# cherubrock-seb/PrMers

Measured on AMD Instinct MI355X. Metric: PRP squaring throughput at p~136M (Marin IBDWT, one exponent per GPU), higher is better.
Workload: dtype u64 (GF(2^64-2^32+1)); 1 GPU; square_mul x<-x^2 mod 2^p-1, p=136279841, n=8388608 words; plan=marin-hip:n=8388608:m1=1024:m2=4096:c=4, parallelism=replicas: one exponent per GPU, no data-path collective

## Files before the change

### prmers_amd/csrc/engine.hip

```cpp
#include "engine.hpp"

#include <algorithm>
#include <cstdlib>
#include <cstring>

#include "host_digits.hpp"

namespace mi355 {

#define HIPCHK(expr)                                                                              \
  do {                                                                                            \
    hipError_t e_ = (expr);                                                                       \
    if (e_ != hipSuccess)                                                                         \
      throw std::runtime_error(std::string("HIP error: ") + hipGetErrorString(e_) + " in " #expr); \
  } while (0)

static ColSweeps col_sweeps(ColKernels k) {
  switch (k) {
    case ColKernels::kRadix8R1: return v2_cols(1);
    case ColKernels::kRadix8R2: return v2_cols(2);
    case ColKernels::kRadix8R4: return v2_cols(4);
    case ColKernels::kRadix4Pairs: return v3_cols(false);
    case ColKernels::kRadix4Planes: return v3_cols(true);
    case ColKernels::kRadix5: return v5_cols(false);
    case ColKernels::kRadix5J1: return v5_cols(true);
    case ColKernels::kSplit: return ColSweeps{};
    default: return ColSweeps{launch_front, launch_back, launch_back_ext, nullptr};
  }
}
static RowsFn row_sweep(RowKernels k) {
  switch (k) {
    case RowKernels::kRadix4Pairs: return v3_rows1024_pairs;
    case RowKernels::kRadix4Planes: return v3_rows1024_planes;
    case RowKernels::kRadix8: return v2_rows4096;
    case RowKernels::kRadix8Wide: return v2_rows8192;
    case RowKernels::kRows2048One: return v2_rows2048_one;
    case RowKernels::kRows2048Two: return v2_rows2048_two;
    default: return launch_middle;
  }
}

template <class T>
static const T* upload(unsigned char*& cursor, unsigned char* base, const std::vector<T>& v, std::vector<unsigned char>& host) {
  const size_t off = size_t(cursor - base);
  std::memcpy(host.data() + off, v.data(), v.size() * sizeof(T));
  const T* p = reinterpret_cast<const T*>(cursor);
  cursor += (v.size() * sizeof(T) + 255) & ~size_t(255);
  return p;
}

Engine::Engine(uint32_t p, size_t reg_count, int device, bool verbose, const char* spec)
    : pl_(make_plan(p, spec, true)), device_(device), verbose_(verbose), nregs_(reg_count) {
  if (reg_count == 0) throw std::runtime_error("register_count must be > 0");
  int ndev = 0;
  hipError_t e = hipGetDeviceCount(&ndev);
  if (e != hipSuccess || ndev == 0)
    throw std::runtime_error("no HIP device available: the MI355X engine has no CPU fallback");
  if (device < 0 || device >= ndev) throw std::runtime_error("HIP device index out of range");
  HIPCHK(hipSetDevice(device));
  HIPCHK(hipStreamCreateWithFlags(&stream_, hipStreamNonBlocking));

  reg_bytes_ = pl_.n * 8;
  HIPCHK(hipMalloc(reinterpret_cast<void**>(&regs_), (nregs_ + 1) * reg_bytes_));
  HIPCHK(hipMemsetAsync(regs_, 0, (nregs_ + 1) * reg_bytes_, stream_));
  slot_.resize(nregs_ + 1);
  for (size_t r = 0; r <= nregs_; ++r) slot_[r] = regs_ + r * reg_bytes_;
  HIPCHK(hipMalloc(reinterpret_cast<void**>(&cbuf_), (nregs_ + 4) * pl_.runs() * 8));
  HIPCHK(hipMemsetAsync(cbuf_, 0, (nregs_ + 4) * pl_.runs() * 8, stream_));
  cb_.resize(nregs_);
  for (size_t r = 0; r < nregs_; ++r) cb_[r] = cbuf_ + r * pl_.runs();
  for (size_t r = nregs_; r < nregs_ + 4; ++r) cb_spare_.push_back(cbuf_ + r * pl_.runs());
  kind_.assign(nregs_, kDigits);
  pending_carry_.assign(nregs_, 0);

  auto padded = [](size_t bytes) { return (bytes + 255) & ~size_t(255); };
  std::vector<uint64_t> tah(pl_.TA.size()), tai2(pl_.TAi.size());
  for (size_t i = 0; i < tah.size(); ++i) { tah[i] = gf::half(pl_.TA[i]); tai2[i] = gf::dbl(pl_.TAi[i]); }
  const size_t total = padded(pl_.SA.size() * 4) + padded(pl_.SB.size() * 4) + padded(pl_.TA.size() * 8) * 4 +
                       padded(pl_.TB.size() * 8) * 2 + padded(pl_.TWlo.size() * 8) + padded(pl_.TWhi.size() * 8) +
                       padded(pl_.UT1.size() * 8) + padded(pl_.UT2.size() * 8) + padded(pl_.S2r.size() * 8) * 2 +
                       padded(pl_.S1r.size() * 8) * 2 + 1024;
  HIPCHK(hipMalloc(&tables_, total));
  std::vector<unsigned char> host(total, 0);
  unsigned char* base = static_cast<unsigned char*>(tables_);
  unsigned char* cur = base;
  dp_.SA = upload(cur, base, pl_.SA, host);
  dp_.SB = upload(cur, base, pl_.SB, host);
  dp_.TA = upload(cur, base, pl_.TA, host);
  dp_.TAi = upload(cur, base, pl_.TAi, host);
  dp_.TAh = upload(cur, base, tah, host);
  dp_.TAi2 = upload(cur, base, tai2, host);
  dp_.TB = upload(cur, base, pl_.TB, host);
  dp_.TBi = upload(cur, base, pl_.TBi, host);
  dp_.TWlo = upload(cur, base, pl_.TWlo, host);
  dp_.TWhi = upload(cur, base, pl_.TWhi, host);
  dp_.UT1 = upload(cur, base, pl_.UT1, host);
  dp_.UT2 = upload(cur, base, pl_.UT2, host);
  dp_.S2r = pl_.S2r.empty() ? nullptr : upload(cur, base, pl_.S2r, host);
  dp_.S2ri = pl_.S2ri.empty() ? nullptr : upload(cur, base, pl_.S2ri, host);
  dp_.S1r = pl_.S1r.empty() ? nullptr : upload(cur, base, pl_.S1r, host);
  dp_.S1ri = pl_.S1ri.empty() ? nullptr : upload(cur, base, pl_.S1ri, host);
  HIPCHK(hipMemcpy(tables_, host.data(), total, hipMemcpyHostToDevice));

  dp_.n = uint32_t(pl_.n); dp_.m = uint32_t(pl_.m);
  dp_.M1 = pl_.M1; dp_.M2 = pl_.M2; dp_.L1 = pl_.L1; dp_.logL1 = pl_.logL1; dp_.logM2 = pl_.logM2;
  dp_.r5 = pl_.r5; dp_.C = pl_.C; dp_.logC = 0; while ((1u << dp_.logC) < pl_.C) ++dp_.logC; dp_.q = pl_.q; dp_.t = pl_.t; dp_.twh = pl_.twh;
  dp_.I4 = pl_.I4; dp_.I4inv = pl_.I4inv;
  dp_.DI = nullptr;
  dp_.F0f = dp_.F0i = dp_.FBf = dp_.FBi = nullptr;
  if (!pl_.DI.empty()) {
    HIPCHK(hipMalloc(reinterpret_cast<void**>(&di_), pl_.DI.size() * 4));
    HIPCHK(hipMemcpy(di_, pl_.DI.data(), pl_.DI.size() * 4, hipMemcpyHostToDevice));
    dp_.DI = di_;
  }
  for (int i = 0; i < 4; ++i) dp_.W5c[i] = pl_.W5c[i];
  { const char* tn = std::getenv("MI355_TUNE"); dp_.tune = tn ? uint32_t(std::atoi(tn)) : 0u; }
  {
    hipDeviceProp_t prop;
    HIPCHK(hipGetDeviceProperties(&prop, device_));
    const uint32_t slots = 2u * uint32_t(prop.multiProcessorCount);
    auto from = [&](size_t grid) { return grid > slots ? uint32_t(grid - size_t(slots) * 50 / 100) : ~0u; };
    dp_.boost_rows = from(pl_.M2 == 2048 ? pl_.M1 / 2 : pl_.M1);
    dp_.boost_tiles = from(pl_.tiles());
  }
  HIPCHK(configure_kernels(pl_.lds_front, pl_.lds_mid));
  if (pl_.split5) {
    HIPCHK(configure_split(dp_));
    HIPCHK(hipMalloc(reinterpret_cast<void**>(&split_), reg_bytes_));
  }
  kc_ = choose_kernels(pl_, std::getenv("MI355_KERNELS"));
  cols_ = col_sweeps(kc_.cols);
  rows_ = row_sweep(kc_.rows);
  dp_.lab_u = 1; dp_.lab_v = pl_.r5; dp_.lab_red = 0;
  if (kc_.cols == ColKernels::kRadix5 || kc_.cols == ColKernels::kRadix5J1) {
    v5_pfa(kc_.cols == ColKernels::kRadix5J1, &dp_.lab_u, &dp_.lab_v);
  } else if (kc_.cols == ColKernels::kGeneric && pl_.r5 == 5 && pl_.L1 > 1) {
    uint32_t u = 1; while ((pl_.L1 * u) % 5 != 1) ++u;
    dp_.lab_u = pl_.L1 * u;
    dp_.lab_red = pl_.M1;
  }
  {
    const uint64_t max_label = dp_.lab_red ? uint64_t(pl_.M1) - 1 : uint64_t(dp_.lab_u) * (pl_.r5 - 1) + uint64_t(dp_.lab_v) * (pl_.L1 - 1);
    if (max_label + uint64_t(pl_.M1) * (pl_.M2 - 1) >= (uint64_t(pl_.TWhi.size()) << pl_.twh))
      throw std::runtime_error("internal: column frequency labels beyond the root table");
  }
  if (kc_.resident_cols() || kc_.rows != RowKernels::kGeneric) HIPCHK(v2_configure());
  if (kc_.resident_cols()) {
    const size_t nt = pl_.tiles() * threads_per_tile(kc_.cols);
    HIPCHK(hipMalloc(reinterpret_cast<void**>(&f0_), (2 * nt + 2 * size_t(pl_.M2)) * 8));
    HIPCHK(cols_.build_fourstep(dp_, f0_, f0_ + nt, f0_ + 2 * nt, f0_ + 2 * nt + pl_.M2, stream_));
    HIPCHK(hipStreamSynchronize(stream_));
    dp_.F0f = f0_; dp_.F0i = f0_ + nt; dp_.FBf = f0_ + 2 * nt; dp_.FBi = f0_ + 2 * nt + pl_.M2;
  }

  width_ = host_digits::digit_widths(p, pl_.n);
  cg_ = CanonGeom::tile_major(dp_, p);
  { const char* hc = std::getenv("MI355_HOST_CARRY"); host_carry_ = hc && hc[0] == '1'; }
  HIPCHK(hipStreamSynchronize(stream_));
  if (verbose_) std::fprintf(stderr, "[mi355] p=%u %s regs=%zu device=%d\n", p, pl_.describe().c_str(), nregs_, device_);
}

Engine::~Engine() {
  (void)hipSetDevice(device_);
  if (stream_) (void)hipStreamSynchronize(stream_);
  if (regs_) (void)hipFree(regs_);
  if (cbuf_) (void)hipFree(cbuf_);
  if (tables_) (void)hipFree(tables_);
  if (di_) (void)hipFree(di_);
  if (f0_) (void)hipFree(f0_);
  if (split_) (void)hipFree(split_);
  if (canon_) (void)hipFree(canon_);
  if (stream_) (void)hipStreamDestroy(stream_);
}

void Engine::sync() {
  HIPCHK(hipSetDevice(device_));
  HIPCHK(hipStreamSynchronize(stream_));
}

void Engine::normalize(size_t r) {
  if (kind_[r] != kDigits) return;
  if (pending_carry_[r]) {
    HIPCHK(launch_carry_fix(dp_, digits(r), cbuf(r), stream_));
    pending_carry_[r] = 0;
  }
}

void Engine::carry_fix_now(size_t r, int excess) {
  HIPCHK(launch_carry_fix(dp_, digits(r), cbuf(r), stream_));
  pending_carry_[r] = 0;
  if (pl_.C >= 2) return;
  if (excess < 0) excess = ilog2(pl_.n) + 1 + 4 - 2;
  const int w = int(pl_.q);
  while (excess > w - 2) {
    HIPCHK(canon_relax(dp_, pl_.p, digits(r), reinterpret_cast<uint32_t*>(work()), stream_));
    swap_with_work(r);
    excess -= w;
  }
}

void Engine::run_front(size_t r) {
  if (kc_.cols == ColKernels::kSplit) HIPCHK(launch_front_split(dp_, digits(r), split_, work(), stream_));
  else HIPCHK(cols_.front(dp_, digits(r), pending_carry_[r] ? cbuf(r) : nullptr, work(), stream_));
}

void Engine::run_middle(const uint64_t* in, const uint64_t* y, uint64_t* out, int mode, const uint64_t* y2, uint64_t* img) {
  HIPCHK(rows_(dp_, in, y, y2, img, out, mode, stream_));
}

void Engine::run_back(size_t r, uint32_t a, hipEvent_t* ev) {
  if (kc_.cols == ColKernels::kSplit) HIPCHK(launch_back_split(dp_, work(), split_, digits(r), cbuf(r), a, stream_));
  else HIPCHK(cols_.back(dp_, work(), digits(r), cbuf(r), a, stream_));
  if (ev) HIPCHK(hipEventRecord(ev[0], stream_));
  if (pl_.C >= 2) pending_carry_[r] = 1;
  else carry_fix_now(r);
  if (ev) HIPCHK(hipEventRecord(ev[1], stream_));
}


void Engine::write_values(size_t dst, const std::vector<uint32_t>& natural) {
  HIPCHK(hipSetDevice(device_));
  HIPCHK(hipStreamSynchronize(stream_));
  uint32_t* nat = reinterpret_cast<uint32_t*>(work());
  HIPCHK(hipMemcpy(nat, natural.data(), pl_.n * 4, hipMemcpyHostToDevice));
  HIPCHK(canon_scatter(dp_, pl_.p, nat, digits(dst), stream_));
  HIPCHK(hipStreamSynchronize(stream_));
  kind_[dst] = kDigits;
  pending_carry_[dst] = 0;
}

uint32_t* Engine::canon_digits(size_t r, int slot) {
  need_residue(r, "get");
  HIPCHK(hipSetDevice(device_));
  const size_t sw = canon_scratch_bytes<uint32_t>(cg_) / 4;
  if (!canon_) {
    HIPCHK(hipMalloc(reinterpret_cast<void**>(&canon_), (sw + 2 * pl_.n) * 4));
    HIPCHK(hipMemsetAsync(canon_flags<uint32_t>(cg_, canon_), 0, 16 * 4, stream_));
  }
  normalize(r);
  uint32_t* out = canon_ + sw + size_t(slot) * pl_.n;
  HIPCHK(canon_launch(cg_, digits(r), out, canon_, stream_));
  return out;
}

bool Engine::canon_flags_ok(uint32_t (&flags)[4]) {
  uint32_t* df = canon_flags<uint32_t>(cg_, canon_);
  HIPCHK(hipMemcpyAsync(flags, df, 16, hipMemcpyDeviceToHost, stream_));
  HIPCHK(hipMemsetAsync(df, 0, 16 * 4, stream_));
  HIPCHK(hipStreamSynchronize(stream_));
  return flags[1] == 0;
}

void Engine::read_values(size_t src, std::vector<uint64_t>& v) {
  if (host_carry_) { read_values_host(src, v); return; }
  uint32_t* d = canon_digits(src, 0);
  uint32_t flags[4];
  stage_.resize(pl_.n);
  HIPCHK(hipMemcpyAsync(stage_.data(), d, pl_.n * 4, hipMemcpyDeviceToHost, stream_));
  if (!canon_flags_ok(flags)) { read_values_host(src, v); return; }
  v.resize(pl_.n);
  if (flags[0]) {
    for (size_t k = 0; k < pl_.n; ++k) v[k] = host_digits::ones(width_[k]);
  } else {
    for (size_t k = 0; k < pl_.n; ++k) v[k] = stage_[k];
  }
}

void Engine::read_values_host(size_t src, std::vector<uint64_t>& v) {
  need_residue(src, "get");
  stage_.resize(pl_.n);
  HIPCHK(hipSetDevice(device_));
  normalize(src);
  HIPCHK(hipStreamSynchronize(stream_));
  HIPCHK(hipMemcpy(stage_.data(), digits(src), pl_.n * 4, hipMemcpyDeviceToHost));
  v.resize(pl_.n);
  const size_t M2 = pl_.M2, C = pl_.C, M1 = pl_.M1;
  for (size_t i = 0; i < pl_.m; ++i) {
    const size_t i1 = i / M2, i2 = i % M2, T = i2 / C, c = i2 % C;
    const size_t s = ((T * M1 + i1) * C + c) * 2;
    v[2 * i] = stage_[s];
    v[2 * i + 1] = stage_[s + 1];
  }
  host_digits::strong_carry(v.data(), width_);
}

void Engine::set_u32(size_t dst, uint32_t value) {
  need_register(dst, "set");
  HIPCHK(hipSetDevice(device_));
  HIPCHK(hipMemsetAsync(digits(dst), 0, pl_.n * 4, stream_));
  if (value) HIPCHK(canon_set_small(dp_, pl_.p, digits(dst), value, stream_));
  kind_[dst] = kDigits;
  pending_carry_[dst] = 0;
}

void Engine::set_digits(size_t dst, const uint64_t* d, size_t count) {
  need_register(dst, "set_digits");
  if (count != pl_.n) throw std::runtime_error("set_digits: count must equal the transform size");
  std::vector<uint32_t> nat(pl_.n);
  for (size_t k = 0; k < pl_.n; ++k) nat[k] = uint32_t(d[k]);
  write_values(dst, nat);
}

void Engine::get_digits(size_t src, uint64_t* d, size_t count) {
  if (count != pl_.n) throw std::runtime_error("get_digits: count must equal the transform size");
  std::vector<uint64_t> v;
  read_values(src, v);
  for (size_t k = 0; k < pl_.n; ++k) d[k] = uint32_t(v[k]) | (uint64_t(width_[k]) << 32);
}

uint64_t Engine::res64(size_t src) {
  std::vector<uint64_t> v;
  size_t have = pl_.n;
  if (host_carry_) {
    read_values_host(src, v);
  } else {
    uint32_t* d = canon_digits(src, 0);
    have = std::min<size_t>(pl_.n, 16);
    uint32_t head[16], flags[4];
    HIPCHK(hipMemcpyAsync(head, d, have * 4, hipMemcpyDeviceToHost, stream_));
    if (!canon_flags_ok(flags)) { read_values_host(src, v); have = pl_.n; }
    else { v.resize(have); for (size_t k = 0; k < have; ++k) v[k] = flags[0] ? host_digits::ones(width_[k]) : head[k]; }
  }
  return host_digits::res64_of_head(v.data(), width_, have);
}

void Engine::get_words(size_t src, uint32_t* w, size_t count) {
  if (count != word_count()) throw std::runtime_error("get_words: count must equal word_count()");
  if (!host_carry_) {
    uint32_t* d = canon_digits(src, 0);
    uint32_t* dw = canon_;
    HIPCHK(canon_pack_words(cg_, d, dw, stream_));
    HIPCHK(hipMemcpyAsync(w, dw, count * 4, hipMemcpyDeviceToHost, stream_));
    uint32_t flags[4];
    if (canon_flags_ok(flags)) return;
  }
  std::vector<uint64_t> v;
  read_values_host(src, v);
  host_digits::pack_words(v.data(), width_, w, count);
}

void Engine::set_words(size_t dst, const uint32_t* w, size_t count) {
  need_register(dst, "set_words");
  if (count != word_count()) throw std::runtime_error("set_words: count must equal word_count()");
  std::vector<uint32_t> src;
  if (host_carry_ || ((pl_.p % 32) && (w[count - 1] >> (pl_.p % 32)))) {
    src.assign(w, w + count);
    host_digits::fold_words_mod_mp(src.data(), count, pl_.p);
    w = src.data();
  }
  if (!host_carry_) {
    HIPCHK(hipSetDevice(device_));
    uint32_t* dw = reinterpret_cast<uint32_t*>(work());
    HIPCHK(hipMemcpyAsync(dw, w, count * 4, hipMemcpyHostToDevice, stream_));
    HIPCHK(canon_unpack_words(cg_, dw, digits(dst), stream_));
    HIPCHK(hipStreamSynchronize(stream_));
    kind_[dst] = kDigits;
    pending_carry_[dst] = 0;
    return;
  }
  std::vector<uint64_t> v(pl_.n);
  host_digits::unpack_words(w, count, width_, v.data());
  write_values(dst, std::vector<uint32_t>(v.begin(), v.end()));
}

bool Engine::equal(size_t lhs, size_t rhs) {
  if (!host_carry_) {
    uint32_t* a = canon_digits(lhs, 0);
    uint32_t* b = canon_digits(rhs, 1);
    HIPCHK(canon_compare(a, b, uint32_t(pl_.n), canon_flags<uint32_t>(cg_, canon_) + 2, stream_));
    uint32_t flags[4];
    if (canon_flags_ok(flags)) return flags[2] == 0;
  }
  return equal_words(lhs, rhs);
}


void Engine::copy(size_t dst, size_t src) {
  need_register(dst, "copy"); need_register(src, "copy");
  if (dst == src) return;
  HIPCHK(hipSetDevice(device_));
  const size_t bytes = (kind_[src] == kDigits) ? pl_.n * 4 : reg_bytes_;
  HIPCHK(hipMemcpyAsync(slot_[dst], slot_[src], bytes, hipMemcpyDeviceToDevice, stream_));
  if (kind_[src] == kDigits && pending_carry_[src])
    HIPCHK(hipMemcpyAsync(cbuf(dst), cbuf(src), pl_.runs() * 8, hipMemcpyDeviceToDevice, stream_));
  pending_carry_[dst] = (kind_[src] == kDigits) ? pending_carry_[src] : 0;
  kind_[dst] = kind_[src];
}

void Engine::square_chain(size_t r, uint32_t a, hipEvent_t* ev) {
  if (a > pl_.a_fast) { square_chain(r, 1, ev); scale(r, a); return; }
  if (ev) HIPCHK(hipEventRecord(ev[0], stream_));
  run_front(r);
  if (ev) HIPCHK(hipEventRecord(ev[1], stream_));
  run_middle(work(), nullptr, work(), 0);
  if (ev) HIPCHK(hipEventRecord(ev[2], stream_));
  run_back(r, a, ev ? ev + 3 : nullptr);
}

void Engine::square_mul(size_t r, uint32_t a) {
  need_residue(r, "square_mul"); need_factor(a, "square_mul");
  HIPCHK(hipSetDevice(device_));
  square_chain(r, a, nullptr);
}

void Engine::square_mul_n(size_t r, uint32_t a, size_t count, uint32_t sub) {
  need_residue(r, "square_mul_n"); need_factor(a, "square_mul_n");
  if (count == 0) return;
  HIPCHK(hipSetDevice(device_));
  for (size_t i = 0; i < count; ++i) { square_chain(r, a, nullptr); if (sub) sub_u32(r, sub); }
}

void Engine::set_multiplicand(size_t dst, size_t src) {
  need_residue(src, "set_multiplicand"); need_register(dst, "set_multiplicand");
  HIPCHK(hipSetDevice(device_));
  run_front(src);
  run_middle(work(), nullptr, image(dst), 2);
  kind_[dst] = kImage;
  pending_carry_[dst] = 0;
}

void Engine::mul(size_t dst, size_t src, uint32_t a) {
  need_residue(dst, "mul"); need_image(src, "mul"); need_factor(a, "mul");
  HIPCHK(hipSetDevice(device_));
  run_front(dst);
  run_middle(work(), image(src), work(), 1);
  run_back(dst, a > pl_.a_fast ? 1u : a);
  if (a > pl_.a_fast) scale(dst, a);
}

void Engine::scale(size_t r, uint32_t a) {
  need_residue(r, "scale");
  uint64_t* fresh = take_spare_cbuf();
  HIPCHK(launch_scale(dp_, digits(r), pending_carry_[r] ? cbuf(r) : nullptr, digits(r), fresh, a, stream_));
  adopt_cbuf(r, fresh);
  pending_carry_[r] = 1;
  if (pl_.C < 2) carry_fix_now(r, 34 - int(pl_.q));
}

uint64_t* Engine::take_spare_cbuf() {
  if (cb_spare_.empty()) throw std::runtime_error("internal: no spare carry buffer");
  uint64_t* b = cb_spare_.back();
  cb_spare_.pop_back();
  return b;
}
void Engine::adopt_cbuf(size_t r, uint64_t* fresh) {
  cb_spare_.push_back(cb_[r]);
  cb_[r] = fresh;
}

void Engine::addsub(long s1, long s2, long d1, long d2, size_t a, size_t b) {
  HIPCHK(hipSetDevice(device_));
  need_residue(a, "addsub"); need_residue(b, "addsub");
  const long outs[4] = {s1, s2, d1, d2};
  for (int i = 0; i < 4; ++i)
    if (outs[i] >= 0) { need_register(size_t(outs[i]), "addsub"); for (int j = 0; j < i; ++j) if (outs[j] == outs[i]) throw std::runtime_error("addsub: output registers must differ"); }
  LinArgs la;
  la.a = digits(a); la.ca = pending_carry_[a] ? cbuf(a) : nullptr;
  la.b = digits(b); la.cb = pending_carry_[b] ? cbuf(b) : nullptr;
  uint64_t* fresh[4] = {nullptr, nullptr, nullptr, nullptr};
  for (int i = 0; i < 4; ++i) if (outs[i] >= 0) fresh[i] = take_spare_cbuf();
  if (s1 >= 0) { la.s1 = digits(size_t(s1)); la.cs1 = fresh[0]; }
  if (s2 >= 0) { la.s2 = digits(size_t(s2)); la.cs2 = fresh[1]; }
  if (d1 >= 0) { la.d1 = digits(size_t(d1)); la.cd1 = fresh[2]; }
  if (d2 >= 0) { la.d2 = digits(size_t(d2)); la.cd2 = fresh[3]; }
  if ((s2 >= 0 && s1 < 0) || (d2 >= 0 && d1 < 0)) throw std::runtime_error("internal: copy output without a primary output");
  HIPCHK(launch_linear(dp_, la, stream_));
  for (int i = 0; i < 4; ++i)
    if (outs[i] >= 0) {
      const size_t r = size_t(outs[i]);
      adopt_cbuf(r, fresh[i]);
      kind_[r] = kDigits; pending_carry_[r] = 1;
      if (pl_.C < 2) carry_fix_now(r);
    }
}

void Engine::add(size_t dst, size_t src) { addsub(long(dst), -1, -1, -1, dst, src); }
void Engine::sub_reg(size_t dst, size_t src) { addsub(-1, -1, long(dst), -1, dst, src); }

void Engine::back_ext(size_t dst, uint32_t a, long copy_to, long add_src) {
  BackExt x;
  if (copy_to >= 0 && size_t(copy_to) != dst) { x.digits2 = digits(size_t(copy_to)); x.cbuf2 = cbuf(size_t(copy_to)); }
  if (add_src >= 0) { x.add_digits = digits(size_t(add_src)); x.add_cbuf = pending_carry_[size_t(add_src)] ? cbuf(size_t(add_src)) : nullptr; }
  uint64_t* fresh = take_spare_cbuf();
  HIPCHK(cols_.back_ext(dp_, work(), digits(dst), fresh, a, x, stream_));
  adopt_cbuf(dst, fresh);
  const size_t outs[2] = {dst, x.digits2 ? size_t(copy_to) : dst};
  for (int i = 0; i < (x.digits2 ? 2 : 1); ++i) {
    const size_t r = outs[i];
    kind_[r] = kDigits; pending_carry_[r] = 1;
    if (pl_.C < 2) carry_fix_now(r);
  }
}

void Engine::square_mul_copy(size_t src, size_t dst_copy, uint32_t a) {
  need_residue(src, "square_mul_copy"); need_register(dst_copy, "square_mul_copy"); need_factor(a, "square_mul_copy");
  HIPCHK(hipSetDevice(device_));
  if (dst_copy == src || !kc_.fused_back() || a > pl_.a_fast) { RegisterMachine::square_mul_copy(src, dst_copy, a); return; }
  run_front(src);
  run_middle(work(), nullptr, work(), 0);
  back_ext(src, a, long(dst_copy), -1);
}

void Engine::mul_copy(size_t dst, size_t src, size_t dst_copy, uint32_t a) {
  need_residue(dst, "mul_copy"); need_image(src, "mul_copy"); need_register(dst_copy, "mul_copy"); need_factor(a, "mul_copy");
  if (dst_copy == src) throw std::runtime_error("mul_copy: the multiplicand must differ from the outputs");
  HIPCHK(hipSetDevice(device_));
  if (dst_copy == dst || !kc_.fused_back() || a > pl_.a_fast) { RegisterMachine::mul_copy(dst, src, dst_copy, a); return; }
  run_front(dst);
  run_middle(work(), image(src), work(), 1);
  back_ext(dst, a, long(dst_copy), -1);
}

void Engine::mul_add(size_t dst, size_t mul_src, size_t add_src, uint32_t a) {
  need_residue(dst, "mul_add"); need_image(mul_src, "mul_add"); need_residue(add_src, "mul_add"); need_factor(a, "mul_add");
  HIPCHK(hipSetDevice(device_));
  if (!kc_.fused_back() || a > pl_.a_fast) {
    if (add_src == dst)
      throw std::runtime_error(!kc_.fused_back() ? "mul_add: add_src == dst needs the fused sweep, which this transform size does not have"
                                          : "mul_add: add_src == dst needs the fused sweep, which takes factors up to the plan's fused bound only (mi355_engine.h)");
    RegisterMachine::mul_add(dst, mul_src, add_src, a); return;
  }
  run_front(dst);
  run_middle(work(), image(mul_src), work(), 1);
  back_ext(dst, a, -1, long(add_src));
}

void Engine::mul_sum(size_t dst, size_t src_a, size_t src_b, size_t tmp) {
  if (!pl_.sum_fast) { RegisterMachine::mul_sum(dst, src_a, src_b, tmp); return; }
  check_mul_sum(dst, src_a, src_b, tmp);
  HIPCHK(hipSetDevice(device_));
  run_front(dst);
  run_middle(work(), image(src_a), work(), 3, image(src_b));
  run_back(dst, 1);
}

void Engine::square_mul_prepare(size_t src, size_t img_out, uint32_t a) {
  check_square_mul_prepare(src, img_out, a);
  HIPCHK(hipSetDevice(device_));
  run_front(src);
  run_middle(work(), nullptr, work(), 4, nullptr, image(img_out));
  kind_[img_out] = kImage;
  pending_carry_[img_out] = 0;
  run_back(src, a > pl_.a_fast ? 1u : a);
  if (a > pl_.a_fast) scale(src, a);
}

void Engine::square_mul_bits(size_t r, uint32_t factor, const uint8_t* bits, size_t nbits) {
  if (!check_square_mul_bits(r, factor, bits, nbits)) return;
  HIPCHK(hipSetDevice(device_));
  for (size_t i = 0; i < nbits; ++i) square_chain(r, bit_of(bits, i) ? factor : 1u, nullptr);
}

void Engine::sub_u32(size_t r, uint32_t v) {
  need_residue(r, "sub");
  if (v == 0) return;
  HIPCHK(hipSetDevice(device_));
  HIPCHK(launch_sub_small(dp_, digits(r), v, stream_));
}


void Engine::get_data(size_t src, void* data, size_t size) {
  need_register(src, "get_data");
  if (size != register_data_size()) throw std::runtime_error("get_data: size mismatch");
  HIPCHK(hipSetDevice(device_));
  normalize(src);
  HIPCHK(hipStreamSynchronize(stream_));
  HIPCHK(hipMemcpy(data, slot_[src], reg_bytes_, hipMemcpyDeviceToHost));
  const uint64_t tag = kind_[src];
  std::memcpy(static_cast<unsigned char*>(data) + reg_bytes_, &tag, 8);
}

void Engine::set_data(size_t dst, const void* data, size_t size) {
  need_register(dst, "set_data");
  if (size != register_data_size()) throw std::runtime_error("set_data: size mismatch");
  uint64_t tag = 0;
  std::memcpy(&tag, static_cast<const unsigned char*>(data) + reg_bytes_, 8);
  if (tag > 1) throw std::runtime_error("set_data: not an image written by this engine");
  HIPCHK(hipSetDevice(device_));
  HIPCHK(hipStreamSynchronize(stream_));
  HIPCHK(hipMemcpy(slot_[dst], data, reg_bytes_, hipMemcpyHostToDevice));
  kind_[dst] = uint8_t(tag);
  pending_carry_[dst] = 0;
}


namespace {
struct EventPool {
  std::vector<hipEvent_t> evs;
  hipEvent_t make() {
    hipEvent_t e = nullptr;
    HIPCHK(hipEventCreate(&e));
    evs.push_back(e);
    return e;
  }
  ~EventPool() { for (hipEvent_t e : evs) (void)hipEventDestroy(e); }
};
}

const char* Engine::stage_name(size_t k) {
  static const char* names[kKernels] = {"k_front", "k_middle", "k_back", "k_carry_fix", "k_sub_small", "event_overhead"};
  return k < kKernels ? names[k] : "";
}

void Engine::time_square_mul(size_t r, uint32_t a, uint32_t sub, size_t iters, double* total_ms, double* kernel_ms, size_t kcount) {
  need_residue(r, "time_square_mul");
  if (a == 0 || iters == 0) throw std::runtime_error("time_square_mul: factor and iters must be >= 1");
  HIPCHK(hipSetDevice(device_));
  EventPool pool;
  const hipEvent_t e0 = pool.make(), e1 = pool.make();
  HIPCHK(hipStreamSynchronize(stream_));
  HIPCHK(hipEventRecord(e0, stream_));
  square_mul_n(r, a, iters, sub);
  HIPCHK(hipEventRecord(e1, stream_));
  HIPCHK(hipEventSynchronize(e1));
  float ms = 0;
  HIPCHK(hipEventElapsedTime(&ms, e0, e1));
  if (total_ms) *total_ms = ms;

  if (kernel_ms && kcount) {
    for (size_t k = 0; k < kcount; ++k) kernel_ms[k] = 0;
    const size_t reps = std::min<size_t>(iters, 64);
    const size_t per = 6;
    std::vector<hipEvent_t> ev(reps * per);
    for (auto& x : ev) x = pool.make();
    double overhead = 0;
    {
      constexpr size_t kBatch = 64, kSkip = 8;
      std::vector<hipEvent_t> oe(kBatch);
      for (auto& x : oe) x = pool.make();
      for (size_t i = 0; i < kBatch; ++i) HIPCHK(hipEventRecord(oe[i], stream_));
      HIPCHK(hipStreamSynchronize(stream_));
      float t = 0;
      HIPCHK(hipEventElapsedTime(&t, oe[kSkip], oe[kBatch - 1]));
      overhead = double(t) / double(kBatch - 1 - kSkip);
    }
    for (size_t i = 0; i < reps; ++i) {
      square_chain(r, a, &ev[i * per]);
// ... 71 lines not shown
```

### prmers_amd/csrc/engine.hpp

```cpp
#pragma once
#include <hip/hip_runtime.h>

#include <algorithm>
#include <cstdint>
#include <stdexcept>
#include <string>
#include <vector>

#include "canon.hpp"
#include "kernels.hpp"
#include "plan.hpp"
#include "register_machine.hpp"

namespace mi355 {

class Engine final : public RegisterMachine {
 public:
  Engine(uint32_t p, size_t reg_count, int device, bool verbose, const char* spec);
  ~Engine() override;
  Engine(const Engine&) = delete;
  Engine& operator=(const Engine&) = delete;

  uint32_t exponent() const override { return pl_.p; }
  std::string describe() const override { return pl_.describe(); }
  size_t size() const override { return pl_.n; }
  size_t reg_count() const override { return nregs_; }

  void sync() override;
  void set_u32(size_t dst, uint32_t v) override;
  void set_digits(size_t dst, const uint64_t* d, size_t count) override;
  void get_digits(size_t src, uint64_t* d, size_t count) override;
  void set_words(size_t dst, const uint32_t* w, size_t count) override;
  void get_words(size_t src, uint32_t* w, size_t count) override;
  uint64_t res64(size_t src) override;
  void copy(size_t dst, size_t src) override;
  void set_multiplicand(size_t dst, size_t src) override;
  void square_mul(size_t r, uint32_t a) override;
  void mul(size_t dst, size_t src, uint32_t a) override;
  void add(size_t dst, size_t src) override;
  void sub_reg(size_t dst, size_t src) override;
  void sub_u32(size_t r, uint32_t v) override;
  bool equal(size_t lhs, size_t rhs) override;
  void addsub(long sum, long sum_copy, long diff, long diff_copy, size_t a, size_t b) override;
  void mul_add(size_t dst, size_t mul_src, size_t add_src, uint32_t a) override;
  void square_mul_copy(size_t src, size_t dst_copy, uint32_t a) override;
  void mul_copy(size_t dst, size_t src, size_t dst_copy, uint32_t a) override;
  void square_mul_n(size_t r, uint32_t a, size_t count, uint32_t sub) override;
  void square_mul_bits(size_t r, uint32_t factor, const uint8_t* bits, size_t nbits) override;
  void mul_sum(size_t dst, size_t src_a, size_t src_b, size_t tmp) override;
  bool mul_sum_is_fused() const override { return pl_.sum_fast; }
  void square_mul_prepare(size_t src, size_t img_out, uint32_t a) override;
  bool square_mul_prepare_is_fused() const override { return true; }

  size_t register_data_size() const override { return reg_bytes_ + 8; }
  void get_data(size_t src, void* data, size_t size) override;
  void set_data(size_t dst, const void* data, size_t size) override;

  static constexpr size_t kKernels = 6;
  static const char* stage_name(size_t k);
  size_t kernel_count() const override { return kKernels; }
  const char* kernel_name(size_t k) const override { return stage_name(k); }
  void time_square_mul(size_t r, uint32_t a, uint32_t sub, size_t iters, double* total_ms, double* kernel_ms, size_t kcount) override;
  size_t algorithmic_bytes() const override { return 48 * pl_.n; }
#if defined(MI355_PROBE)
  void probe(int kind, int grid_mult, int extra_lds, int boost_pct, size_t iters, double* avg_ms, uint64_t* tl, size_t tl_words);
#endif

 private:
  enum Kind : uint8_t { kDigits = 0, kImage = 1 };
  bool holds_image(size_t r) const override { return kind_[r] == kImage; }
  uint32_t* digits(size_t r) { return reinterpret_cast<uint32_t*>(slot_[r]); }
  uint64_t* image(size_t r) { return reinterpret_cast<uint64_t*>(slot_[r]); }
  uint64_t* work() { return reinterpret_cast<uint64_t*>(slot_[nregs_]); }
  void swap_with_work(size_t r) { std::swap(slot_[r], slot_[nregs_]); }
  void read_values(size_t src, std::vector<uint64_t>& v);
  void read_values_host(size_t src, std::vector<uint64_t>& v);
  uint32_t* canon_digits(size_t r, int slot);
  bool canon_flags_ok(uint32_t (&flags)[4]);
  void write_values(size_t dst, const std::vector<uint32_t>& natural);
  void square_chain(size_t r, uint32_t a, hipEvent_t* ev);
  uint64_t* cbuf(size_t r) { return cb_[r]; }
  uint64_t* take_spare_cbuf();
  void adopt_cbuf(size_t r, uint64_t* fresh);
  void back_ext(size_t dst, uint32_t a, long copy_to, long add_src);
  void normalize(size_t r);
  void carry_fix_now(size_t r, int excess = -1);
  void scale(size_t r, uint32_t a);
  void run_front(size_t r);
  void run_middle(const uint64_t* in, const uint64_t* y, uint64_t* out, int mode, const uint64_t* y2 = nullptr, uint64_t* img = nullptr);
  void run_back(size_t r, uint32_t a, hipEvent_t* ev = nullptr);

  Plan pl_;
  DevPlan dp_{};
  CanonGeom cg_{};
  int device_ = 0;
  bool verbose_ = false;
  hipStream_t stream_ = nullptr;
  size_t nregs_ = 0, reg_bytes_ = 0;
  unsigned char* regs_ = nullptr;
  std::vector<unsigned char*> slot_;
  uint64_t* cbuf_ = nullptr;
  std::vector<uint64_t*> cb_, cb_spare_;
  void* tables_ = nullptr;
  uint64_t* split_ = nullptr;
  uint64_t* f0_ = nullptr;
  uint32_t* di_ = nullptr;
  std::vector<uint8_t> kind_;
  std::vector<uint8_t> pending_carry_;
  KernelChoice kc_;
  ColSweeps cols_{};
  RowsFn rows_ = nullptr;
  std::vector<uint8_t> width_;
  std::vector<uint32_t> stage_;
  uint32_t* canon_ = nullptr;
  bool host_carry_ = false;
};

}
```

### prmers_amd/csrc/gfdft.hpp

```cpp
#pragma once
#include "gf.hpp"

namespace gf {

constexpr unsigned LOG2_W64 = 39;
constexpr unsigned shift64(unsigned e) { return (LOG2_W64 * e) % 192; }

template <bool INV, int LAZY = 0>
GF_HD void dft8(uint64_t (&x)[8]) {
  constexpr bool LZ_A0 = (LAZY >= 2), LZ_E0 = (LAZY >= 1);
  const uint64_t a0 = LZ_A0 ? add_lazy(x[0], x[4]) : add(x[0], x[4]);
  const uint64_t a1 = add(x[1], x[5]), a2 = add(x[2], x[6]), a3 = add(x[3], x[7]);
  uint64_t b0 = sub(x[0], x[4]), b1, b2, b3;
  if (!INV) {
    b1 = mul_pow2(sub(x[5], x[1]), 24);
    b2 = mul_pow2(sub(x[2], x[6]), 48);
    b3 = mul_pow2(sub(x[7], x[3]), 72);
  } else {
    b1 = mul_pow2(sub(x[1], x[5]), 72);
    b2 = mul_pow2(sub(x[6], x[2]), 48);
    b3 = mul_pow2(sub(x[3], x[7]), 24);
  }
  const uint64_t c0 = LZ_A0 ? add_lazy(a0, a2) : add(a0, a2);
  const uint64_t c1 = add(a1, a3), d0 = sub(a0, a2);
  const uint64_t d1 = mul_pow2(INV ? sub(a3, a1) : sub(a1, a3), 48);
  const uint64_t e0 = LZ_E0 ? add_lazy(b0, b2) : add(b0, b2);
  const uint64_t e1 = add(b1, b3), f0 = sub(b0, b2);
  const uint64_t f1 = mul_pow2(INV ? sub(b3, b1) : sub(b1, b3), 48);
  x[0] = (LAZY >= 2) ? add_lazy(c0, c1) : add(c0, c1); x[4] = sub(c0, c1);
  x[2] = (LAZY >= 1) ? add_lazy(d0, d1) : add(d0, d1); x[6] = sub(d0, d1);
  x[1] = (LAZY >= 1) ? add_lazy(e0, e1) : add(e0, e1); x[5] = sub(e0, e1);
  x[3] = (LAZY >= 1) ? add_lazy(f0, f1) : add(f0, f1); x[7] = sub(f0, f1);
}

}
```

### prmers_amd/csrc/kernels.hip

```cpp
#include <hip/hip_runtime.h>
#include <stdint.h>
#include <stdlib.h>

#include "gf.hpp"
#include "kernels.hpp"

namespace mi355 {

struct alignas(16) P2 { uint64_t a, b; };

__device__ __forceinline__ P2 p2_add(P2 x, P2 y) { return {gf::add(x.a, y.a), gf::add(x.b, y.b)}; }
__device__ __forceinline__ P2 p2_sub(P2 x, P2 y) { return {gf::sub(x.a, y.a), gf::sub(x.b, y.b)}; }
__device__ __forceinline__ P2 p2_mul(P2 x, uint64_t w) { return {gf::mul(x.a, w), gf::mul(x.b, w)}; }
__device__ __forceinline__ P2 p2_shift48(P2 x) { return {gf::mul_pow2(x.a, 48), gf::mul_pow2(x.b, 48)}; }

__device__ __forceinline__ uint64_t tw_lookup(const DevPlan& pl, uint64_t e) {
  const uint64_t lo = pl.TWlo[e & ((1u << pl.twh) - 1)], hi = pl.TWhi[e >> pl.twh];
  return gf::mul(lo, hi);
}

__device__ __forceinline__ uint32_t freq1(const DevPlan& pl, uint32_t pos) {
  const uint32_t blk = pos >> pl.logL1, q = pos & (pl.L1 - 1);
  const uint32_t rq = pl.logL1 ? (__brev(q) >> (32 - pl.logL1)) : 0u;
  return col_label(pl, blk, rq);
}

__device__ __forceinline__ void digit_info(const DevPlan& pl, uint32_t sa, uint32_t sb, uint32_t& width, bool& wrap) {
  uint64_t s = uint64_t(sa) + sb;
  wrap = (sa > 0) && (sb > 0) && (s <= pl.n);
  if (s >= pl.n) s -= pl.n;
  width = pl.q + ((s + pl.t > 0) ? 1u : 0u) + ((s + pl.t > pl.n) ? 1u : 0u) - ((s > 0) ? 1u : 0u);
}

template <bool INVERSE>
__device__ __forceinline__ void lds_pow2_dft_planes(P2* X, uint32_t L, uint32_t logL, uint32_t nblocks, uint32_t ncols, uint32_t logcols,
                                                    const uint64_t* __restrict__ root, uint32_t rootN, uint32_t rstep, uint32_t tid, uint32_t nthr) {
  uint64_t* Xw = reinterpret_cast<uint64_t*>(X);
  const uint32_t n4 = logL / 2, has2 = logL & 1;
  const uint32_t npass = n4 + has2;
  for (uint32_t ps = 0; ps < npass; ++ps) {
    const uint32_t pf = INVERSE ? (npass - 1 - ps) : ps;
    if (pf < n4) {
      const uint32_t loglen = logL - 2 * pf, len = 1u << loglen, q = len >> 2;
      const uint32_t per = L >> 2;
      const uint32_t total = per * nblocks * ncols * 2;
      const uint32_t tstep = (L >> loglen) * rstep;
      for (uint32_t idx2 = tid; idx2 < total; idx2 += nthr) {
        const uint32_t plane = idx2 & 1, idx = idx2 >> 1;
        const uint32_t col = idx & (ncols - 1), bi = idx >> logcols;
        const uint32_t blk = bi >> (logL - 2), bj = bi & (per - 1);
        const uint32_t sub = bj >> (loglen - 2), t = bj & (q - 1);
        const uint32_t e0 = 2 * ((blk * L + sub * len + t) * ncols + col) + plane, es = 2 * q * ncols;
        const uint32_t r1 = t * tstep;
        const uint64_t x0 = Xw[e0], x1 = Xw[e0 + es], x2 = Xw[e0 + 2 * es], x3 = Xw[e0 + 3 * es];
        if (!INVERSE) {
          const uint64_t w1 = root[r1], w2 = root[2 * r1], w3 = root[3 * r1];
          const uint64_t a = gf::add(x0, x2), b = gf::add(x1, x3), c = gf::sub(x0, x2), d = gf::mul_pow2(gf::sub(x1, x3), 48);
          Xw[e0] = gf::add(a, b);
          Xw[e0 + es] = gf::mul(gf::sub(a, b), w2);
          Xw[e0 + 2 * es] = gf::mul(gf::add(c, d), w1);
          Xw[e0 + 3 * es] = gf::mul(gf::sub(c, d), w3);
        } else {
          const uint64_t w1 = root[r1 ? rootN - r1 : 0], w2 = root[r1 ? rootN - 2 * r1 : 0], w3 = root[r1 ? rootN - 3 * r1 : 0];
          const uint64_t y1 = gf::mul(x1, w2);
          const uint64_t A = gf::add(x0, y1), B = gf::sub(x0, y1);
          const uint64_t y2 = gf::mul(x2, w1), y3 = gf::mul(x3, w3);
          const uint64_t Cc = gf::add(y2, y3), D = gf::mul_pow2(gf::sub(y3, y2), 48);
          Xw[e0] = gf::add(A, Cc);
          Xw[e0 + 2 * es] = gf::sub(A, Cc);
          Xw[e0 + es] = gf::add(B, D);
          Xw[e0 + 3 * es] = gf::sub(B, D);
        }
      }
    } else {
      const uint32_t per = L >> 1, total = per * nblocks * ncols * 2;
      for (uint32_t idx2 = tid; idx2 < total; idx2 += nthr) {
        const uint32_t plane = idx2 & 1, idx = idx2 >> 1;
        const uint32_t col = idx & (ncols - 1), bi = idx >> logcols;
        const uint32_t blk = bi >> (logL - 1), bj = bi & (per - 1);
        const uint32_t e0 = 2 * ((blk * L + 2 * bj) * ncols + col) + plane;
        const uint64_t u = Xw[e0], v = Xw[e0 + 2 * ncols];
        Xw[e0] = gf::add(u, v);
        Xw[e0 + 2 * ncols] = gf::sub(u, v);
      }
    }
    __syncthreads();
  }
}

template <bool INVERSE>
__device__ __forceinline__ void lds_pow2_dft(P2* X, uint32_t L, uint32_t logL, uint32_t nblocks, uint32_t ncols, uint32_t logcols,
                                             const uint64_t* __restrict__ root, uint32_t rootN, uint32_t rstep,
                                             uint64_t I4, uint32_t tid, uint32_t nthr) {
  if (nthr * 2 >= (L >> 2) * nblocks * ncols * 2 && nthr > (L >> 2) * nblocks * ncols) {
    lds_pow2_dft_planes<INVERSE>(X, L, logL, nblocks, ncols, logcols, root, rootN, rstep, tid, nthr);
    return;
  }
  const uint32_t n4 = logL / 2, has2 = logL & 1;
  const uint32_t npass = n4 + has2;
  for (uint32_t ps = 0; ps < npass; ++ps) {
    const uint32_t pf = INVERSE ? (npass - 1 - ps) : ps;
    if (pf < n4) {
      const uint32_t loglen = logL - 2 * pf, len = 1u << loglen, q = len >> 2;
      const uint32_t per = L >> 2;
      const uint32_t total = per * nblocks * ncols;
      const uint32_t tstep = (L >> loglen) * rstep;
      for (uint32_t idx = tid; idx < total; idx += nthr) {
        const uint32_t col = idx & (ncols - 1), bi = idx >> logcols;
        const uint32_t blk = bi >> (logL - 2), bj = bi & (per - 1);
        const uint32_t sub = bj >> (loglen - 2), t = bj & (q - 1);
        const uint32_t e0 = (blk * L + sub * len + t) * ncols + col, es = q * ncols;
        const uint32_t r1 = t * tstep;
        P2 x0 = X[e0], x1 = X[e0 + es], x2 = X[e0 + 2 * es], x3 = X[e0 + 3 * es];
        if (!INVERSE) {
          const uint64_t w1 = root[r1], w2 = root[2 * r1], w3 = root[3 * r1];
          const P2 a = p2_add(x0, x2), b = p2_add(x1, x3), c = p2_sub(x0, x2), d = p2_shift48(p2_sub(x1, x3));
          X[e0] = p2_add(a, b);
          X[e0 + es] = p2_mul(p2_sub(a, b), w2);
          X[e0 + 2 * es] = p2_mul(p2_add(c, d), w1);
          X[e0 + 3 * es] = p2_mul(p2_sub(c, d), w3);
        } else {
          const uint64_t w1 = root[r1 ? rootN - r1 : 0], w2 = root[r1 ? rootN - 2 * r1 : 0], w3 = root[r1 ? rootN - 3 * r1 : 0];
          const P2 y1 = p2_mul(x1, w2);
          const P2 A = p2_add(x0, y1), B = p2_sub(x0, y1);
          const P2 y2 = p2_mul(x2, w1), y3 = p2_mul(x3, w3);
          const P2 Cc = p2_add(y2, y3), D = p2_shift48(p2_sub(y3, y2));
          X[e0] = p2_add(A, Cc);
          X[e0 + 2 * es] = p2_sub(A, Cc);
          X[e0 + es] = p2_add(B, D);
          X[e0 + 3 * es] = p2_sub(B, D);
        }
      }
    } else {
      const uint32_t per = L >> 1, total = per * nblocks * ncols;
      for (uint32_t idx = tid; idx < total; idx += nthr) {
        const uint32_t col = idx & (ncols - 1), bi = idx >> logcols;
        const uint32_t blk = bi >> (logL - 1), bj = bi & (per - 1);
        const uint32_t e0 = (blk * L + 2 * bj) * ncols + col;
        const P2 u = X[e0], v = X[e0 + ncols];
        X[e0] = p2_add(u, v);
        X[e0 + ncols] = p2_sub(u, v);
      }
    }
    __syncthreads();
  }
}

template <bool INVERSE>
__device__ __forceinline__ void dft5(P2 (&x)[5], const uint64_t (&c5)[4]) {
  const P2 t1 = p2_add(x[1], x[4]), t2 = p2_add(x[2], x[3]), t3 = p2_sub(x[1], x[4]), t4 = p2_sub(x[2], x[3]);
  const P2 t5 = p2_add(t1, t2);
  const P2 A = p2_add(x[0], P2{gf::mul_pow2(t5.a, 94), gf::mul_pow2(t5.b, 94)});
  const P2 m2 = p2_mul(p2_sub(t1, t2), c5[0]);
  const P2 B1 = p2_add(A, m2), B2 = p2_sub(A, m2);
  const P2 m3 = p2_mul(p2_add(t3, t4), c5[1]), m4 = p2_mul(t4, c5[2]), m5 = p2_mul(t3, c5[3]);
  const P2 Pp = p2_add(m3, m4), Q = p2_sub(m5, m3);
  x[0] = p2_add(x[0], t5);
  if (!INVERSE) { x[1] = p2_add(B1, Pp); x[4] = p2_sub(B1, Pp); x[2] = p2_add(B2, Q); x[3] = p2_sub(B2, Q); }
  else          { x[1] = p2_sub(B1, Pp); x[4] = p2_add(B1, Pp); x[2] = p2_sub(B2, Q); x[3] = p2_add(B2, Q); }
}

template <bool INVERSE>
__device__ __forceinline__ void lds_radix5(const DevPlan& pl, P2* X, uint32_t ncols, uint32_t tid, uint32_t nthr) {
  const uint32_t L1 = pl.L1, total = L1 * ncols;
  const bool pfa = pl.lab_u != 1;
  for (uint32_t idx = tid; idx < total; idx += nthr) {
    const uint32_t col = idx & (ncols - 1), t = idx >> pl.logC;
    const uint32_t t5 = 5 * t, rho = pfa ? (t5 & (L1 - 1)) : t, w0 = pfa ? (t5 >> pl.logL1) : 0u;
    P2 x[5];
    if (!INVERSE) {
#pragma unroll
      for (uint32_t r = 0; r < 5; ++r) { const uint32_t b = r + w0; x[r] = X[(L1 * (b >= 5 ? b - 5 : b) + rho) * ncols + col]; }
      dft5<false>(x, pl.W5c);
      if (!pfa) {
#pragma unroll
        for (int k = 1; k < 5; ++k) x[k] = p2_mul(x[k], pl.UT1[t * k]);
      }
#pragma unroll
      for (int r = 0; r < 5; ++r) X[(L1 * r + rho) * ncols + col] = x[r];
    } else {
#pragma unroll
      for (int r = 0; r < 5; ++r) x[r] = X[(L1 * r + rho) * ncols + col];
      if (!pfa) {
#pragma unroll
        for (int k = 1; k < 5; ++k) x[k] = p2_mul(x[k], pl.UT1[(t * k) ? pl.M1 - t * k : 0]);
      }
      dft5<true>(x, pl.W5c);
#pragma unroll
      for (uint32_t r = 0; r < 5; ++r) { const uint32_t b = r + w0; X[(L1 * (b >= 5 ? b - 5 : b) + rho) * ncols + col] = x[r]; }
    }
  }
  __syncthreads();
}

extern __shared__ __attribute__((aligned(16))) unsigned char smem_raw[];

__device__ __forceinline__ uint64_t carry_in_of(const DevPlan& pl, const uint64_t* cbuf, uint32_t T, uint32_t i1) {
  const uint32_t NT = pl.M2 / pl.C;
  if (T > 0) return *(cbuf + size_t(T - 1) * pl.M1 + i1);
  return *(cbuf + size_t(NT - 1) * pl.M1 + (i1 ? i1 - 1 : pl.M1 - 1));
}

__device__ __forceinline__ void front_body(const DevPlan& pl, const uint32_t* digits, const uint64_t* cbuf_in, uint64_t* Wout, uint32_t T,
                                           P2* X, uint32_t tid, uint32_t nthr) {
  const uint32_t C = pl.C, M1 = pl.M1, tile = M1 * C;
  const uint2* dg = reinterpret_cast<const uint2*>(digits) + size_t(T) * tile;

  for (uint32_t e = tid; e < tile; e += nthr) {
    const uint32_t i1 = e >> pl.logC, c = e & (C - 1), i2 = T * C + c;
    uint2 d = dg[e];
    const uint32_t sa = pl.SA[i1];
    if (cbuf_in && c < 2) {
      uint64_t cin = carry_in_of(pl, cbuf_in, T, i1);
      if (cin) {
        const uint2* run = dg + i1 * C;
        const uint2 p0 = run[0], p1 = run[1];
        uint32_t dd[4] = {p0.x, p0.y, p1.x, p1.y};
#pragma unroll
        for (int k = 0; k < 3; ++k) {
          uint32_t width; bool wr;
          digit_info(pl, sa, pl.SB[2 * (T * C) + k], width, wr);
          const uint64_t v = uint64_t(dd[k]) + cin;
          dd[k] = uint32_t(v & ((uint64_t(1) << width) - 1));
          cin = v >> width;
        }
        dd[3] += uint32_t(cin);
        d = c ? make_uint2(dd[2], dd[3]) : make_uint2(dd[0], dd[1]);
      }
    }
    uint32_t w0, w1; bool wr0, wr1;
    const uint32_t sb = pl.SB[2 * i2];
    digit_info(pl, sa, sb, w0, wr0);
    digit_info(pl, pl.SA[M1 + i1], sb, w1, wr1);
    const uint64_t a0 = gf::mul_u32(pl.TAh[i1], d.x << (wr0 ? 0 : 1));
    const uint64_t a1 = gf::mul_u32(pl.TAh[M1 + i1], d.y << (wr1 ? 0 : 1));
    X[e] = {a0, a1};
  }
  __syncthreads();

  const bool one = tile <= nthr;
  uint64_t pre_lo = 0, pre_hi = 0, pre_tb = 0;
  if (one && tid < tile) {
    const uint32_t pos = tid >> pl.logC, i2 = T * C + (tid & (C - 1));
    const uint64_t ex = uint64_t(i2) * freq1(pl, pos);
    pre_lo = pl.TWlo[ex & ((1u << pl.twh) - 1)]; pre_hi = pl.TWhi[ex >> pl.twh]; pre_tb = pl.TB[2 * i2];
  }
  if (pl.r5 == 5) lds_radix5<false>(pl, X, C, tid, nthr);
  if (pl.logL1) lds_pow2_dft<false>(X, pl.L1, pl.logL1, pl.r5, C, pl.logC, pl.UT1, M1, pl.r5, pl.I4, tid, nthr);

  P2* W = reinterpret_cast<P2*>(Wout);
  for (uint32_t e = tid; e < tile; e += nthr) {
    const uint32_t pos = e >> pl.logC, c = e & (C - 1), i2 = T * C + c;
    const uint32_t k1 = freq1(pl, pos);
    const uint32_t ex = i2 * k1;
    const uint64_t tw = one ? gf::mul(pre_lo, pre_hi) : tw_lookup(pl, ex);
    const P2 x = X[e];
    const uint64_t twb = gf::mul(tw, one ? pre_tb : pl.TB[2 * i2]);
    P2* out = W + size_t(pos) * pl.M2 + i2;
    *out = {gf::mul(x.a, twb), gf::mul(x.b, twb)};
  }
}
__global__ void __launch_bounds__(1024) k_front(DevPlan pl, const uint32_t* __restrict__ digits, const uint64_t* __restrict__ cbuf_in,
                                                uint64_t* __restrict__ Wout) {
  if (blockIdx.x >= pl.boost_tiles) __builtin_amdgcn_s_setprio(3);
  front_body(pl, digits, cbuf_in, Wout, blockIdx.x, reinterpret_cast<P2*>(smem_raw), threadIdx.x, blockDim.x);
}

template <bool KEEP = false>
__device__ __forceinline__ void middle_body(const DevPlan& pl, const uint64_t* Win, const uint64_t* Yimg, const uint64_t* Yimg2, uint64_t* Wout, int mode, uint32_t sub, uint32_t row,
                                            P2* X, uint32_t tid, uint32_t nthr, uint64_t* Wimg = nullptr) {
  const uint32_t M2 = pl.M2;
  const P2* in = reinterpret_cast<const P2*>(Win) + size_t(row) * M2;
  P2* out = reinterpret_cast<P2*>(Wout) + size_t(row) * M2;

  for (uint32_t e = tid; e < M2; e += nthr) X[e] = in[e];
  __syncthreads();
  if (sub != 0 && tid == 0) X[0].a = gf::sub(X[0].a, uint64_t(sub));
  __syncthreads();
  const uint32_t k1 = freq1(pl, row);
  const bool one = M2 <= nthr;
  uint64_t pre_lo = 0, pre_hi = 0;
  if (one && tid < M2 && mode != 2) {
    const uint64_t ex = rho_exponent(pl, k1, __brev(tid) >> (32 - pl.logM2));
    pre_lo = pl.TWlo[ex & ((1u << pl.twh) - 1)]; pre_hi = pl.TWhi[ex >> pl.twh];
  }
  lds_pow2_dft<false>(X, M2, pl.logM2, 1, 1, 0, pl.UT2, M2, 1, pl.I4, tid, nthr);
  if (mode == 2) {
    for (uint32_t e = tid; e < M2; e += nthr) out[e] = X[e];
    return;
  }
  if constexpr (KEEP) {
    P2* img = reinterpret_cast<P2*>(Wimg) + size_t(row) * M2;
    for (uint32_t e = tid; e < M2; e += nthr) img[e] = X[e];
  }
  const P2* Y = reinterpret_cast<const P2*>(Yimg) + size_t(row) * M2;
  for (uint32_t e = tid; e < M2; e += nthr) {
    const uint32_t k2 = __brev(e) >> (32 - pl.logM2);
    const uint64_t rho = one ? gf::mul(pre_lo, pre_hi) : tw_lookup(pl, rho_exponent(pl, k1, k2));
    const P2 u = X[e];
    P2 r;
    if (mode == 0) {
      r.a = gf::add(gf::sqr(u.a), gf::mul(gf::sqr(u.b), rho));
      r.b = gf::mul(u.b, gf::dbl(u.a));
    } else {
      P2 y = Y[e];
      if (mode == 3) {
        const P2 z = reinterpret_cast<const P2*>(Yimg2)[size_t(row) * M2 + e];
        y = {gf::add_lazy_any(y.a, z.a), gf::add_lazy_any(y.b, z.b)};
      }
      r.a = gf::add(gf::mul(u.a, y.a), gf::mul(gf::mul(u.b, y.b), rho));
      r.b = gf::add(gf::mul(u.a, y.b), gf::mul(u.b, y.a));
    }
    X[e] = r;
  }
  __syncthreads();
  lds_pow2_dft<true>(X, M2, pl.logM2, 1, 1, 0, pl.UT2, M2, 1, pl.I4inv, tid, nthr);
  for (uint32_t e = tid; e < M2; e += nthr) out[e] = X[e];
}
__global__ void __launch_bounds__(1024) k_middle(DevPlan pl, const uint64_t* __restrict__ Win, const uint64_t* __restrict__ Yimg,
                                                const uint64_t* __restrict__ Yimg2, uint64_t* __restrict__ Wout, int mode, uint32_t sub) {
  middle_body(pl, Win, Yimg, Yimg2, Wout, mode, sub, blockIdx.x, reinterpret_cast<P2*>(smem_raw), threadIdx.x, blockDim.x);
}
__global__ void __launch_bounds__(1024) k_middle_keep(DevPlan pl, const uint64_t* __restrict__ Win, uint64_t* __restrict__ Wimg, uint64_t* __restrict__ Wout, uint32_t sub) {
  middle_body<true>(pl, Win, nullptr, nullptr, Wout, 0, sub, blockIdx.x, reinterpret_cast<P2*>(smem_raw), threadIdx.x, blockDim.x, Wimg);
}

__device__ __forceinline__ void run_carry_in(const DevPlan& pl, uint32_t sa, uint32_t T, uint64_t cin, uint32_t (&dd)[4]) {
#pragma unroll
  for (int k = 0; k < 3; ++k) {
    uint32_t width; bool wr;
    digit_info(pl, sa, pl.SB[2 * (T * pl.C) + k], width, wr);
    const uint64_t v = uint64_t(dd[k]) + cin;
    dd[k] = uint32_t(v & ((uint64_t(1) << width) - 1));
    cin = v >> width;
  }
  dd[3] += uint32_t(cin);
}

__device__ __forceinline__ uint32_t xcd_tile(const DevPlan& pl, uint32_t b, uint32_t groups) {
  return (!(pl.tune & 1) && groups % 8 == 0) ? (b & 7) * (groups >> 3) + (b >> 3) : b;
}
template <bool EXT>
__device__ __forceinline__ void back_body(const DevPlan& pl, const uint64_t* Win, uint32_t* digits, uint64_t* cbuf, uint32_t a, const BackExt& ext, uint32_t T,
                                          P2* X, uint32_t tid, uint32_t nthr) {
  const uint32_t C = pl.C, M1 = pl.M1, tile = M1 * C;
  const P2* W = reinterpret_cast<const P2*>(Win);

  for (uint32_t e = tid; e < tile; e += nthr) {
    const uint32_t pos = e >> pl.logC, c = e & (C - 1), i2 = T * C + c;
    const uint32_t k1 = freq1(pl, pos);
    const uint32_t ex = i2 * k1;
    const uint64_t tw = tw_lookup(pl, ex ? pl.m - ex : 0);
    const P2 x = *(W + size_t(pos) * pl.M2 + i2);
    const uint64_t twb = gf::mul(tw, pl.TBi[2 * i2]);
    X[e] = {gf::mul(x.a, twb), gf::mul(x.b, twb)};
  }
  __syncthreads();

  if (pl.logL1) lds_pow2_dft<true>(X, pl.L1, pl.logL1, pl.r5, C, pl.logC, pl.UT1, M1, pl.r5, pl.I4inv, tid, nthr);
  if (pl.r5 == 5) lds_radix5<true>(pl, X, C, tid, nthr);

  uint2* dg = reinterpret_cast<uint2*>(digits) + size_t(T) * tile;
  for (uint32_t i1 = tid; i1 < M1; i1 += nthr) {
    const uint32_t sa[2] = {pl.SA[i1], pl.SA[M1 + i1]};
    const uint64_t tai[2] = {pl.TAi[i1], pl.TAi[M1 + i1]};
    const uint64_t tai2[2] = {pl.TAi2[i1], pl.TAi2[M1 + i1]};
    uint64_t carry = 0;
    uint32_t addh[4] = {0, 0, 0, 0};
    const uint2* ad = nullptr;
    if (EXT && ext.add_digits) {
      ad = reinterpret_cast<const uint2*>(ext.add_digits) + size_t(T) * tile + size_t(i1) * C;
      if (ext.add_cbuf) {
        const uint2 p0 = ad[0], p1 = ad[1];
        addh[0] = p0.x; addh[1] = p0.y; addh[2] = p1.x; addh[3] = p1.y;
        run_carry_in(pl, pl.SA[i1], T, carry_in_of(pl, ext.add_cbuf, T, i1), addh);
      }
    }
    for (uint32_t c = 0; c < C; ++c) {
      const uint32_t i2 = T * C + c;
      const P2 x = X[i1 * C + c];
      const uint32_t sb = pl.SB[2 * i2];
      uint32_t out[2];
      uint32_t av[2] = {0, 0};
      if (EXT && ad) {
        if (ext.add_cbuf && c < 2) { av[0] = addh[2 * c]; av[1] = addh[2 * c + 1]; }
        else { const uint2 q = ad[c]; av[0] = q.x; av[1] = q.y; }
      }
#pragma unroll
      for (int b = 0; b < 2; ++b) {
        uint32_t width; bool wrap;
        digit_info(pl, sa[b], sb, width, wrap);
        const uint64_t u = gf::mul(b ? x.b : x.a, wrap ? tai2[b] : tai[b]);
        const uint64_t mask = (uint64_t(1) << width) - 1;
        if (a == 1) {
          const uint64_t r = u + carry + (EXT ? av[b] : 0u);
          out[b] = uint32_t(r & mask);
          carry = r >> width;
        } else {
          const uint64_t dlo = u & mask, chi = u >> width;
          const uint64_t r = dlo * a + carry + (EXT ? av[b] : 0u);
          out[b] = uint32_t(r & mask);
          carry = (r >> width) + chi * a;
        }
      }
      *(dg + i1 * C + c) = make_uint2(out[0], out[1]);
      if (EXT && ext.digits2) reinterpret_cast<uint2*>(ext.digits2)[size_t(T) * tile + size_t(i1) * C + c] = make_uint2(out[0], out[1]);
    }
    *(cbuf + size_t(T) * M1 + i1) = carry;
    if (EXT && ext.digits2) ext.cbuf2[size_t(T) * M1 + i1] = carry;
  }
}
template <bool EXT>
__global__ void __launch_bounds__(1024) k_back(DevPlan pl, const uint64_t* __restrict__ Win, uint32_t* __restrict__ digits,
                                              uint64_t* __restrict__ cbuf, uint32_t a, BackExt ext) {
  if (blockIdx.x >= pl.boost_tiles) __builtin_amdgcn_s_setprio(3);
  back_body<EXT>(pl, Win, digits, cbuf, a, ext, xcd_tile(pl, blockIdx.x, gridDim.x), reinterpret_cast<P2*>(smem_raw), threadIdx.x, blockDim.x);
}

__global__ void __launch_bounds__(256) k_front_split_a(DevPlan pl, const uint32_t* __restrict__ digits, uint64_t* __restrict__ Uout) {
  const size_t e = size_t(blockIdx.x) * 256 + threadIdx.x;
  const uint32_t t = uint32_t(e & (pl.L1 - 1)), i2 = uint32_t(e >> pl.logL1), M1 = pl.M1;
  if (i2 >= pl.M2) return;
  const uint2* dg = reinterpret_cast<const uint2*>(digits) + size_t(i2) * M1;
  const uint32_t sb = pl.SB[2 * i2];
  P2 x[5];
#pragma unroll
  for (int r = 0; r < 5; ++r) {
    const uint32_t i1 = pl.L1 * r + t;
    const uint2 d = dg[i1];
    uint32_t w0, w1; bool wr0, wr1;
    digit_info(pl, pl.SA[i1], sb, w0, wr0);
    digit_info(pl, pl.SA[M1 + i1], sb, w1, wr1);
    x[r] = {gf::mul_u32(pl.TAh[i1], d.x << (wr0 ? 0 : 1)), gf::mul_u32(pl.TAh[M1 + i1], d.y << (wr1 ? 0 : 1))};
  }
  dft5<false>(x, pl.W5c);
#pragma unroll
  for (int k = 1; k < 5; ++k) x[k] = p2_mul(x[k], pl.UT1[t * k]);
  P2* U = reinterpret_cast<P2*>(Uout);
#pragma unroll
  for (int k0 = 0; k0 < 5; ++k0) U[(size_t(k0) * pl.M2 + i2) * pl.L1 + t] = x[k0];
}
__global__ void __launch_bounds__(1024) k_front_split_b(DevPlan pl, const uint64_t* __restrict__ Uin, uint64_t* __restrict__ Wout, uint32_t logCb) {
  P2* X = reinterpret_cast<P2*>(smem_raw);
  const uint32_t tid = threadIdx.x, nthr = blockDim.x, Cb = 1u << logCb, per = pl.M2 >> logCb;
  const uint32_t k0 = blockIdx.x / per, T = blockIdx.x - k0 * per, tile = pl.L1 << logCb;
  const P2* U = reinterpret_cast<const P2*>(Uin);
  for (uint32_t e = tid; e < tile; e += nthr) {
    const uint32_t c = e >> pl.logL1, pp = e & (pl.L1 - 1);
    X[(pp << logCb) + c] = U[(size_t(k0) * pl.M2 + (T << logCb) + c) * pl.L1 + pp];
  }
  __syncthreads();
  if (pl.logL1) lds_pow2_dft<false>(X, pl.L1, pl.logL1, 1, Cb, logCb, pl.UT1, pl.M1, pl.r5, pl.I4, tid, nthr);
  P2* W = reinterpret_cast<P2*>(Wout);
  for (uint32_t e = tid; e < tile; e += nthr) {
    const uint32_t pp = e >> logCb, c = e & (Cb - 1), i2 = (T << logCb) + c, pos = k0 * pl.L1 + pp;
    const uint64_t ex = uint64_t(i2) * freq1(pl, pos);
// ... 271 lines not shown
```

### prmers_amd/csrc/kernels.hpp

```cpp
#pragma once
#include <hip/hip_runtime.h>
#include <stdint.h>

namespace mi355 {

struct DevPlan {
  uint32_t n, m, M1, M2, L1, logL1, logM2, r5, C, logC, q, t, twh;
  const uint32_t *SA, *SB;
  const uint64_t *TA, *TAi, *TB, *TBi;
  const uint64_t *TAh, *TAi2;
  const uint64_t *TWlo, *TWhi, *UT1, *UT2;
  const uint64_t *S2r, *S2ri, *S1r, *S1ri;
  uint64_t I4, I4inv;
  uint64_t W5c[4];
  const uint64_t *F0f, *F0i, *FBf, *FBi;
  const uint32_t* DI;
  uint32_t boost_rows, boost_tiles;
  uint32_t lab_u, lab_v;
  uint32_t lab_red;
#if defined(MI355_PROBE)
  uint64_t* probe;
  uint32_t probe_mod;
#endif
  uint32_t tune;
};

#if defined(__HIPCC__)
__device__ __forceinline__ uint32_t col_label(const DevPlan& pl, uint32_t blk, uint32_t rq) {
  uint32_t l = pl.lab_u * blk + pl.lab_v * rq;
  if (pl.lab_red) {
#pragma unroll
    for (int i = 0; i < 4; ++i) l = (l >= pl.lab_red) ? l - pl.lab_red : l;
  }
  return l;
}
__device__ __forceinline__ uint64_t rho_exponent(const DevPlan& pl, uint32_t label, uint64_t k) { return uint64_t(label) + uint64_t(pl.M1) * k; }
#endif

struct BackExt {
  uint32_t* digits2 = nullptr; uint64_t* cbuf2 = nullptr;
  const uint32_t* add_digits = nullptr; const uint64_t* add_cbuf = nullptr;
  bool any() const { return digits2 || add_digits; }
};
struct LinArgs {
  const uint32_t* a = nullptr; const uint64_t* ca = nullptr; const uint32_t* b = nullptr; const uint64_t* cb = nullptr;
  uint32_t* s1 = nullptr; uint64_t* cs1 = nullptr; uint32_t* s2 = nullptr; uint64_t* cs2 = nullptr;
  uint32_t* d1 = nullptr; uint64_t* cd1 = nullptr; uint32_t* d2 = nullptr; uint64_t* cd2 = nullptr;
};
hipError_t launch_linear(const DevPlan& pl, const LinArgs& la, hipStream_t s);
hipError_t launch_scale(const DevPlan& pl, const uint32_t* in, const uint64_t* cin, uint32_t* out, uint64_t* cout, uint32_t a, hipStream_t s);
hipError_t launch_carry_fix(const DevPlan& pl, uint32_t* digits, const uint64_t* cbuf, hipStream_t s);
hipError_t launch_sub_small(const DevPlan& pl, uint32_t* digits, uint32_t a, hipStream_t s);

typedef hipError_t (*FrontFn)(const DevPlan& pl, const uint32_t* digits, const uint64_t* cbuf_in, uint64_t* W, hipStream_t s);
typedef hipError_t (*BackFn)(const DevPlan& pl, const uint64_t* W, uint32_t* digits, uint64_t* cbuf, uint32_t a, hipStream_t s);
typedef hipError_t (*BackExtFn)(const DevPlan& pl, const uint64_t* W, uint32_t* digits, uint64_t* cbuf, uint32_t a, const BackExt& x, hipStream_t s);
typedef hipError_t (*FourStepFn)(const DevPlan& pl, uint64_t* f0f, uint64_t* f0i, uint64_t* fbf, uint64_t* fbi, hipStream_t s);
typedef hipError_t (*RowsFn)(const DevPlan& pl, const uint64_t* Win, const uint64_t* Y, const uint64_t* Y2, uint64_t* Wimg, uint64_t* Wout, int mode, hipStream_t s);
struct ColSweeps { FrontFn front; BackFn back; BackExtFn back_ext; FourStepFn build_fourstep; };

hipError_t configure_kernels(size_t lds_front, size_t lds_mid);
hipError_t launch_front(const DevPlan& pl, const uint32_t* digits, const uint64_t* cbuf_in, uint64_t* W, hipStream_t s);
hipError_t launch_middle(const DevPlan& pl, const uint64_t* Win, const uint64_t* Y, const uint64_t* Y2, uint64_t* Wimg, uint64_t* Wout, int mode, hipStream_t s);
hipError_t launch_back(const DevPlan& pl, const uint64_t* W, uint32_t* digits, uint64_t* cbuf, uint32_t a, hipStream_t s);
hipError_t launch_back_ext(const DevPlan& pl, const uint64_t* W, uint32_t* digits, uint64_t* cbuf, uint32_t a, const BackExt& x, hipStream_t s);
hipError_t configure_split(const DevPlan& pl);
hipError_t launch_front_split(const DevPlan& pl, const uint32_t* digits, uint64_t* U, uint64_t* W, hipStream_t s);
hipError_t launch_back_split(const DevPlan& pl, const uint64_t* W, uint64_t* U, uint32_t* digits, uint64_t* cbuf, uint32_t a, hipStream_t s);

hipError_t v2_configure();
ColSweeps v2_cols(uint32_t R);
ColSweeps v3_cols(bool planes);
ColSweeps v5_cols(bool j1);
void v5_pfa(bool j1, uint32_t* u, uint32_t* v);
hipError_t v2_rows4096(const DevPlan& pl, const uint64_t* Win, const uint64_t* Y, const uint64_t* Y2, uint64_t* Wimg, uint64_t* Wout, int mode, hipStream_t s);
hipError_t v2_rows8192(const DevPlan& pl, const uint64_t* Win, const uint64_t* Y, const uint64_t* Y2, uint64_t* Wimg, uint64_t* Wout, int mode, hipStream_t s);
hipError_t v2_rows2048_one(const DevPlan& pl, const uint64_t* Win, const uint64_t* Y, const uint64_t* Y2, uint64_t* Wimg, uint64_t* Wout, int mode, hipStream_t s);
hipError_t v2_rows2048_two(const DevPlan& pl, const uint64_t* Win, const uint64_t* Y, const uint64_t* Y2, uint64_t* Wimg, uint64_t* Wout, int mode, hipStream_t s);
hipError_t v3_rows1024_pairs(const DevPlan& pl, const uint64_t* Win, const uint64_t* Y, const uint64_t* Y2, uint64_t* Wimg, uint64_t* Wout, int mode, hipStream_t s);
hipError_t v3_rows1024_planes(const DevPlan& pl, const uint64_t* Win, const uint64_t* Y, const uint64_t* Y2, uint64_t* Wimg, uint64_t* Wout, int mode, hipStream_t s);
#if defined(MI355_PROBE)
hipError_t v2_probe_launch(const DevPlan& pl, int kind, int grid_mult, int extra_lds, const uint32_t* digits, uint64_t* cbuf, uint64_t* W, uint32_t* dout, hipStream_t s);
hipError_t v5_probe_launch(const DevPlan& pl, int kind, int grid_mult, int extra_lds, const uint32_t* digits, uint64_t* cbuf, uint64_t* W, uint32_t* dout, hipStream_t s);
#endif

}
```

### prmers_amd/csrc/kernels_v2.hip

```cpp
#include "kernels_v2_common.hpp"

namespace mi355 {
namespace v2 {
template <int RL, int W, bool INV>
__device__ __forceinline__ void seam_rows_const(P2 (&x)[8]) {
#pragma unroll
  for (int k = 1; k < 8; ++k) {
    constexpr int R1 = 8 >> RL;
    if ((k & (R1 - 1)) == 0) continue;
    const unsigned f = ((1u << RL) * gf::LOG2_W64 * unsigned(k & (R1 - 1)) * unsigned(W)) % 192u;
    const unsigned sh = INV ? (192u - f) % 192u : f;
    x[k] = {gf::mul_pow2(x[k].a, sh), gf::mul_pow2(x[k].b, sh)};
  }
}
template <int RL, bool INV>
__device__ __forceinline__ void seam_rows(P2 (&x)[8], uint32_t wave) {
  switch (wave) {
    case 0: break;
    case 1: seam_rows_const<RL, 1, INV>(x); break;
    case 2: seam_rows_const<RL, 2, INV>(x); break;
    case 3: seam_rows_const<RL, 3, INV>(x); break;
    case 4: seam_rows_const<RL, 4, INV>(x); break;
    case 5: seam_rows_const<RL, 5, INV>(x); break;
    case 6: seam_rows_const<RL, 6, INV>(x); break;
    default: seam_rows_const<RL, 7, INV>(x); break;
  }
}
template <int RL, bool INV>
__device__ __forceinline__ void dft_rows_first(P2 (&x)[8]) {
  static_assert(RL == 1, "two rows to a tile");
  dft4<INV>(x[0].a, x[1].a, x[2].a, x[3].a); dft4<INV>(x[0].b, x[1].b, x[2].b, x[3].b);
  dft4<INV>(x[4].a, x[5].a, x[6].a, x[7].a); dft4<INV>(x[4].b, x[5].b, x[6].b, x[7].b);
}

template <int mode, int H, int RL = 0>
__global__ void __launch_bounds__(512 * H, 4) k2_rows4096(DevPlan pl, const uint64_t* __restrict__ Win, const uint64_t* __restrict__ Yimg,
                                                          const uint64_t* __restrict__ Yimg2, uint64_t* __restrict__ Wimg, uint64_t* __restrict__ Wout, uint32_t sub) {
  static_assert(RL == 0 || (RL == 1 && H == 1), "two rows to a tile only with one tile per work-group");
  constexpr bool HALF = (RL > 0);
  constexpr int HH = H;
  constexpr int R1 = 8 >> RL;
  const uint32_t h = (H == 2) ? __builtin_amdgcn_readfirstlane(threadIdx.x >> 9) : 0u;
  if (H == 1) boost_if_late(pl.boost_rows);
  P2* X = reinterpret_cast<P2*>(smem_v2) + h * kLdsSlots;
  const uint32_t t = threadIdx.x & 511, lane = t & 63, wave = __builtin_amdgcn_readfirstlane((threadIdx.x >> 6) & 7);
  const uint32_t tile = PROBE_BLOCK(pl);
  const uint32_t row = HALF ? (tile << RL) + (lane >> (6 - RL)) : tile;
  PROBE_BEGIN(pl)
  const P2* in = reinterpret_cast<const P2*>(Win) + size_t(tile) * (4096 * HH);
  P2* out = reinterpret_cast<P2*>(Wout) + size_t(tile) * (4096 * HH) + h * 4096;
  P2 x[8];
  const uint32_t kb = ((lane >> 3) & uint32_t(R1 - 1)) + R1 * (lane & 7) + 8 * R1 * wave;
  const uint32_t blk = row / pl.L1, qq = row - blk * pl.L1;
  const uint32_t k1row = col_label(pl, blk, pl.logL1 ? (__brev(qq) >> (32 - pl.logL1)) : 0u);
  const uint64_t erho = rho_exponent(pl, k1row, HH * kb + h);
  const uint64_t rho_lo = pl.TWlo[erho & ((1u << pl.twh) - 1)], rho_hi = pl.TWhi[erho >> pl.twh];

  if (H == 1) {
#pragma unroll
    for (int j = 0; j < 8; ++j) x[j] = w_load(&in[512 * j + t]);
    if (sub != 0 && t == 0) {
#pragma unroll
      for (int r = 0; r < (1 << RL); ++r) x[R1 * r].a = gf::sub(x[R1 * r].a, uint64_t(sub));
    }
  } else {
#pragma unroll
    for (int j = 0; j < 8; ++j) {
      P2 lo = in[512 * j + t];
      const P2 hi = in[4096 + 512 * j + t];
      if (j == 0 && sub != 0 && t == 0) lo.a = gf::sub(lo.a, uint64_t(sub));
      if (h == 0) x[j] = {gf::add(lo.a, hi.a), gf::add(lo.b, hi.b)};
      else x[j] = p2_mul(P2{gf::sub(lo.a, hi.a), gf::sub(lo.b, hi.b)}, pl.UT2[512 * j + t]);
    }
  }
  if constexpr (HALF) { dft_rows_first<RL, false>(x); seam_rows<RL, false>(x, wave); }
  else {
    dft8p<false, 1>(x);
    seam64<false, true>(x, wave);
  }
  uint64_t sw[8];
  {
    const uint32_t k1 = t & 7, b = t >> 3;
    const uint64_t* __restrict__ tw = pl.S2r + b * 64 + k1 * 8;
#pragma unroll
    for (int k2 = 0; k2 < 8; ++k2) sw[k2] = tw[k2];
  }
  EXCH_THREAD_MAJOR_TO_STRIDED(X, x, t)
  dft8p<false, 2>(x);
#pragma unroll
  for (int k2 = 0; k2 < 8; ++k2) x[k2] = p2_mul(x[k2], sw[k2]);
  EXCH_THREAD_MAJOR_TO_STRIDED(X, x, t)
  dft8p<false, 1>(x);
  seam64<false, true>(x, wave);
  lds_barrier();
#pragma unroll
  for (int k = 0; k < 8; ++k) X[phys(wave * 512 + k * 64 + lane)] = x[k];
  lds_barrier();
#pragma unroll
  for (int j = 0; j < 8; ++j) x[j] = X[phys(j * 512 + t)];
  dft8p<false, 2>(x);

  if (mode == 2) {
#pragma unroll
    for (int j = 0; j < 8; ++j) out[512 * j + t] = x[j];
    return;
  }
  if (mode == 4) {
    P2* img = reinterpret_cast<P2*>(Wimg) + size_t(tile) * (4096 * HH) + h * 4096;
#pragma unroll
    for (int j = 0; j < 8; ++j) img[512 * j + t] = x[j];
  }

  PROBE_MID(pl)
  {
    const uint64_t rho0 = gf::mul(rho_lo, rho_hi);
    const P2* Y = reinterpret_cast<const P2*>(Yimg) + size_t(tile) * (4096 * HH) + h * 4096;
#pragma unroll
    for (int k4 = 0; k4 < 8; ++k4) {
      const unsigned sh = 24u * (k4 & 3);
      const bool neg = (k4 == 1) || (k4 == 3) || (k4 == 4) || (k4 == 6);
      const P2 u = x[k4];
      P2 r;
      if (mode == 0 || mode == 4) {
        const uint64_t q = gf::mul_pow2(gf::mul(gf::sqr(u.b), rho0), sh);
        const uint64_t s0 = gf::sqr(u.a);
        r.a = neg ? gf::sub(s0, q) : gf::add(s0, q);
        r.b = gf::dbl(gf::mul(u.b, u.a));
      } else {
        P2 y = Y[512 * k4 + t];
        if (mode == 3) {
          const P2 z = (reinterpret_cast<const P2*>(Yimg2) + size_t(tile) * (4096 * HH) + h * 4096)[512 * k4 + t];
          y = {gf::add_lazy_any(y.a, z.a), gf::add_lazy_any(y.b, z.b)};
        }
        const uint64_t q = gf::mul_pow2(gf::mul(gf::mul(u.b, y.b), rho0), sh);
        const uint64_t s0 = gf::mul(u.a, y.a);
        r.a = neg ? gf::sub(s0, q) : gf::add(s0, q);
        r.b = gf::add(gf::mul(u.a, y.b), gf::mul(u.b, y.a));
      }
      x[k4] = r;
    }
  }

  dft8p<true>(x);
  lds_barrier();
#pragma unroll
  for (int j = 0; j < 8; ++j) X[phys(j * 512 + t)] = x[j];
  lds_barrier();
#pragma unroll
  for (int k = 0; k < 8; ++k) x[k] = X[phys(wave * 512 + k * 64 + lane)];
  seam64<true>(x, wave);
  dft8p<true, 2>(x);
  {
    const uint32_t k1 = t & 7, b = t >> 3;
    const uint64_t* __restrict__ tw = pl.S2ri + b * 64 + k1 * 8;
#pragma unroll
    for (int k2 = 0; k2 < 8; ++k2) sw[k2] = tw[k2];
  }
  EXCH_STRIDED_TO_THREAD_MAJOR(X, x, t)
  if (H == 1) __builtin_amdgcn_s_setprio(0);
#pragma unroll
  for (int k2 = 0; k2 < 8; ++k2) x[k2] = p2_mul(x[k2], sw[k2]);
  dft8p<true>(x);
  EXCH_STRIDED_TO_THREAD_MAJOR(X, x, t)
  if constexpr (HALF) { seam_rows<RL, true>(x, wave); dft_rows_first<RL, true>(x); }
  else {
    seam64<true>(x, wave);
    if (H == 1) dft8p<true, 2>(x);
    else dft8p<true>(x);
  }
  if (H == 2) {
    if (h == 1) {
#pragma unroll
      for (int j = 0; j < 8; ++j) { const uint32_t i = 512 * j + t; x[j] = p2_mul(x[j], pl.UT2[i ? 8192 - i : 0]); }
    }
    __syncthreads();
#pragma unroll
    for (int j = 0; j < 8; ++j) X[phys(j * 512 + t)] = x[j];
    __syncthreads();
    const P2* Xo = reinterpret_cast<const P2*>(smem_v2) + (1 - h) * kLdsSlots;
#pragma unroll
    for (int j = 0; j < 8; ++j) {
      const P2 o = Xo[phys(j * 512 + t)];
      x[j] = (h == 0) ? P2{gf::add(x[j].a, o.a), gf::add(x[j].b, o.b)} : P2{gf::sub(o.a, x[j].a), gf::sub(o.b, x[j].b)};
    }
  }
#pragma unroll
  for (int j = 0; j < 8; ++j) w_store(&out[512 * j + t], x[j]);
  PROBE_END(pl)
}

__device__ __forceinline__ uint32_t phys8(uint32_t i) { return i ^ ((i >> 3) & 31u); }
__device__ __forceinline__ uint64_t swap32(uint64_t v, uint32_t partner_byte) {
  const uint32_t lo = uint32_t(__builtin_amdgcn_ds_bpermute(int(partner_byte), int(uint32_t(v))));
  const uint32_t hi = uint32_t(__builtin_amdgcn_ds_bpermute(int(partner_byte), int(uint32_t(v >> 32))));
  return (uint64_t(hi) << 32) | lo;
}
template <int W, bool INV>
__device__ __forceinline__ void seam64w_const(uint64_t (&x)[8]) {
#pragma unroll
  for (int k = 1; k < 8; ++k) {
    const unsigned f = (gf::LOG2_W64 * unsigned(k) * unsigned(W)) % 192u;
    x[k] = gf::mul_pow2(x[k], INV ? (192u - f) % 192u : f);
  }
}
template <bool INV, bool FOLD0 = false>
__device__ __forceinline__ void seam64w(uint64_t (&x)[8], uint32_t wave) {
  switch (wave) {
    case 0:
      if (FOLD0) { x[1] = gf::fold(x[1]); x[2] = gf::fold(x[2]); x[3] = gf::fold(x[3]); x[5] = gf::fold(x[5]); }
      break;
    case 1: seam64w_const<1, INV>(x); break;
    case 2: seam64w_const<2, INV>(x); break;
    case 3: seam64w_const<3, INV>(x); break;
    case 4: seam64w_const<4, INV>(x); break;
    case 5: seam64w_const<5, INV>(x); break;
    case 6: seam64w_const<6, INV>(x); break;
    default: seam64w_const<7, INV>(x); break;
  }
}
template <int W, bool INV>
__device__ __forceinline__ void seam32w_const(uint64_t (&x)[8]) {
#pragma unroll
  for (int k = 1; k < 8; ++k) {
    if ((k & 3) == 0) continue;
    const unsigned f = (2u * gf::LOG2_W64 * unsigned(k & 3) * unsigned(W)) % 192u;
    x[k] = gf::mul_pow2(x[k], INV ? (192u - f) % 192u : f);
  }
}
template <bool INV>
__device__ __forceinline__ void seam32w(uint64_t (&x)[8], uint32_t wave) {
  switch (wave) {
    case 0: break;
    case 1: seam32w_const<1, INV>(x); break;
    case 2: seam32w_const<2, INV>(x); break;
    case 3: seam32w_const<3, INV>(x); break;
    case 4: seam32w_const<4, INV>(x); break;
    case 5: seam32w_const<5, INV>(x); break;
    case 6: seam32w_const<6, INV>(x); break;
    default: seam32w_const<7, INV>(x); break;
  }
}
#define EXCHW_THREAD_MAJOR_TO_STRIDED(X, x, t)                      \
  lds_barrier();                                                    \
  _Pragma("unroll") for (int r_ = 0; r_ < 8; ++r_) X[phys8((t) * 8 + r_)] = x[r_]; \
  lds_barrier();                                                    \
  _Pragma("unroll") for (int j_ = 0; j_ < 8; ++j_) x[j_] = X[phys8(j_ * 512 + (t))];
#define EXCHW_STRIDED_TO_THREAD_MAJOR(X, x, t)                      \
  lds_barrier();                                                    \
  _Pragma("unroll") for (int j_ = 0; j_ < 8; ++j_) X[phys8(j_ * 512 + (t))] = x[j_]; \
  lds_barrier();                                                    \
  _Pragma("unroll") for (int r_ = 0; r_ < 8; ++r_) x[r_] = X[phys8((t) * 8 + r_)];

constexpr uint32_t kLdsBytesPlanes = 4096 * 8;

template <int mode>
__global__ void __launch_bounds__(512, 4) k2_rows2048_planes(DevPlan pl, const uint64_t* __restrict__ Win, const uint64_t* __restrict__ Yimg,
                                                             const uint64_t* __restrict__ Yimg2, uint64_t* __restrict__ Wimg, uint64_t* __restrict__ Wout, uint32_t sub) {
  uint64_t* X = reinterpret_cast<uint64_t*>(smem_v2);
  const uint32_t t = threadIdx.x, lane = t & 63, wave = __builtin_amdgcn_readfirstlane(threadIdx.x >> 6);
  const uint32_t row = blockIdx.x;
  const P2* in = reinterpret_cast<const P2*>(Win) + size_t(row) * 2048;
  P2* out = reinterpret_cast<P2*>(Wout) + size_t(row) * 2048;
  uint64_t x[8];
  const uint32_t pln = lane >> 5, partner = ((lane ^ 32u) << 2);
  const uint32_t kb = ((lane >> 3) & 3u) + 4 * (lane & 7) + 32 * wave;
  const uint32_t blk = row / pl.L1, qq = row - blk * pl.L1;
  const uint32_t k1row = col_label(pl, blk, pl.logL1 ? (__brev(qq) >> (32 - pl.logL1)) : 0u);
  const uint64_t erho = rho_exponent(pl, k1row, kb);
  const uint64_t rho_lo = pl.TWlo[erho & ((1u << pl.twh) - 1)], rho_hi = pl.TWhi[erho >> pl.twh];

#pragma unroll
  for (int d = 0; d < 4; ++d) { const P2 v = in[512 * d + t]; x[d] = v.a; x[4 + d] = v.b; }
  if (sub != 0 && t == 0) x[0] = gf::sub(x[0], uint64_t(sub));
  dft4<false>(x[0], x[1], x[2], x[3]); dft4<false>(x[4], x[5], x[6], x[7]);
  seam32w<false>(x, wave);
  uint64_t sw[8];
  {
    const uint32_t k1 = t & 7, b = t >> 3;
    const uint64_t* __restrict__ tw = pl.S2r + b * 64 + k1 * 8;
#pragma unroll
    for (int k2 = 0; k2 < 8; ++k2) sw[k2] = tw[k2];
  }
  EXCHW_THREAD_MAJOR_TO_STRIDED(X, x, t)
  gf::dft8<false, 2>(x);
#pragma unroll
  for (int k2 = 0; k2 < 8; ++k2) x[k2] = gf::mul(x[k2], sw[k2]);
  EXCHW_THREAD_MAJOR_TO_STRIDED(X, x, t)
  gf::dft8<false, 1>(x);
  seam64w<false, true>(x, wave);
  lds_barrier();
#pragma unroll
  for (int k = 0; k < 8; ++k) X[phys8(wave * 512 + k * 64 + lane)] = x[k];
  lds_barrier();
#pragma unroll
  for (int j = 0; j < 8; ++j) x[j] = X[phys8(j * 512 + t)];
  gf::dft8<false, 2>(x);

  if (mode == 2) {
    uint64_t* img = Wout + size_t(row) * 4096;
#pragma unroll
    for (int j = 0; j < 8; ++j) img[512 * j + t] = x[j];
    return;
  }
  if (mode == 4) {
    uint64_t* img = Wimg + size_t(row) * 4096;
#pragma unroll
    for (int j = 0; j < 8; ++j) img[512 * j + t] = x[j];
  }

  {
    const uint64_t rho0 = gf::mul(rho_lo, rho_hi);
    const uint64_t* Y = Yimg + size_t(row) * 4096;
#pragma unroll
    for (int k4 = 0; k4 < 8; ++k4) {
      const unsigned sh = 24u * (k4 & 3);
      const bool neg = (k4 == 1) || (k4 == 3) || (k4 == 4) || (k4 == 6);
      const uint64_t w = x[k4];
      uint64_t keep, send;
      if (mode == 0 || mode == 4) {
        const uint64_t o = swap32(w, partner);
        keep = gf::sqr(w);
        send = gf::mul(pln ? keep : w, pln ? rho0 : o);
        if (pln) send = gf::mul_pow2(send, sh);
      } else {
        uint64_t y = Y[512 * k4 + t], yo = Y[512 * k4 + (t ^ 32u)];
        if (mode == 3) {
          const uint64_t* Z = Yimg2 + size_t(row) * 4096;
          y = gf::add_lazy_any(y, Z[512 * k4 + t]); yo = gf::add_lazy_any(yo, Z[512 * k4 + (t ^ 32u)]);
        }
        keep = gf::mul(w, y);
        send = gf::mul(w, yo);
        if (pln) { const uint64_t q = gf::mul_pow2(gf::mul(keep, rho0), sh); keep = send; send = q; }
      }
      const uint64_t recv = swap32(send, partner);
      if (mode == 0 || mode == 4) x[k4] = pln ? gf::dbl(recv) : (neg ? gf::sub(keep, recv) : gf::add(keep, recv));
      else x[k4] = pln ? gf::add(keep, recv) : (neg ? gf::sub(keep, recv) : gf::add(keep, recv));
    }
  }

  gf::dft8<true>(x);
  lds_barrier();
#pragma unroll
  for (int j = 0; j < 8; ++j) X[phys8(j * 512 + t)] = x[j];
  lds_barrier();
#pragma unroll
  for (int k = 0; k < 8; ++k) x[k] = X[phys8(wave * 512 + k * 64 + lane)];
  seam64w<true>(x, wave);
  gf::dft8<true, 2>(x);
  {
    const uint32_t k1 = t & 7, b = t >> 3;
    const uint64_t* __restrict__ tw = pl.S2ri + b * 64 + k1 * 8;
#pragma unroll
    for (int k2 = 0; k2 < 8; ++k2) sw[k2] = tw[k2];
  }
  EXCHW_STRIDED_TO_THREAD_MAJOR(X, x, t)
#pragma unroll
  for (int k2 = 0; k2 < 8; ++k2) x[k2] = gf::mul(x[k2], sw[k2]);
  gf::dft8<true>(x);
  EXCHW_STRIDED_TO_THREAD_MAJOR(X, x, t)
  seam32w<true>(x, wave);
  dft4<true>(x[0], x[1], x[2], x[3]); dft4<true>(x[4], x[5], x[6], x[7]);
#pragma unroll
  for (int d = 0; d < 4; ++d) out[512 * d + t] = P2{x[d], x[4 + d]};
}


template <int R> struct ColShape {
  static constexpr int C = 8 / R;
  static constexpr int LC = (C == 8) ? 3 : (C == 4) ? 2 : 1;
  static constexpr int LR = 3 - LC;
  static constexpr int M1 = 512 * R, LM = 9 + LR, ND = 2 * C;
};

template <int R, int W>
__device__ __forceinline__ void stage_r_fwd_const(P2 (&x)[8]) {
  constexpr int C = 8 / R;
  if (R == 2) {
#pragma unroll
    for (int c = 0; c < C; ++c) {
      const P2 u = x[c], v = x[C + c];
      x[c] = {gf::add(u.a, v.a), gf::add(u.b, v.b)};
      x[C + c] = {gf::sub(u.a, v.a), gf::sub(u.b, v.b)};
    }
  } else if (R == 4) {
#pragma unroll
    for (int c = 0; c < C; ++c) {
      dft4<false>(x[c].a, x[C + c].a, x[2 * C + c].a, x[3 * C + c].a);
      dft4<false>(x[c].b, x[C + c].b, x[2 * C + c].b, x[3 * C + c].b);
    }
  }
#pragma unroll
  for (int k1 = 1; k1 < R; ++k1) {
    const unsigned s = ((8u / unsigned(R)) * gf::LOG2_W64 * unsigned(k1) * unsigned(W)) % 192u;
#pragma unroll
    for (int c = 0; c < C; ++c) x[k1 * C + c] = {gf::mul_pow2(x[k1 * C + c].a, s), gf::mul_pow2(x[k1 * C + c].b, s)};
  }
}
template <int R, int W>
__device__ __forceinline__ void stage_r_inv_const(P2 (&x)[8]) {
  constexpr int C = 8 / R;
  if (R == 2) {
    const unsigned f = (192u - (4u * gf::LOG2_W64 * unsigned(W)) % 192u) % 192u;
    const bool neg = f >= 96u;
    const unsigned s = neg ? f - 96u : f;
#pragma unroll
    for (int c = 0; c < C; ++c) {
      const P2 u = x[c];
      const P2 v = {gf::mul_pow2(x[C + c].a, s), gf::mul_pow2(x[C + c].b, s)};
      const P2 sum = {gf::add(u.a, v.a), gf::add(u.b, v.b)}, dif = {gf::sub(u.a, v.a), gf::sub(u.b, v.b)};
      x[c] = neg ? dif : sum;
      x[C + c] = neg ? sum : dif;
    }
  } else if (R == 4) {
#pragma unroll
    for (int k1 = 1; k1 < R; ++k1) {
      const unsigned s = (192u - ((8u / unsigned(R)) * gf::LOG2_W64 * unsigned(k1) * unsigned(W)) % 192u) % 192u;
#pragma unroll
      for (int c = 0; c < C; ++c) x[k1 * C + c] = {gf::mul_pow2(x[k1 * C + c].a, s), gf::mul_pow2(x[k1 * C + c].b, s)};
    }
#pragma unroll
    for (int c = 0; c < C; ++c) {
      dft4<true>(x[c].a, x[C + c].a, x[2 * C + c].a, x[3 * C + c].a);
      dft4<true>(x[c].b, x[C + c].b, x[2 * C + c].b, x[3 * C + c].b);
    }
  }
}

template <int R>
__device__ __forceinline__ void front_tile(const DevPlan& pl, P2* X, uint32_t T, uint32_t t, uint32_t lane, uint32_t wave,
                                           const uint32_t (&dg)[R][16 / R], uint32_t di, uint32_t sub, uint64_t* __restrict__ Wout) {
  using S = ColShape<R>;
  constexpr int C = S::C, LC = S::LC;
  P2 x[8];
  const uint32_t nowrap = ~di;
#pragma unroll
  for (int d1 = 0; d1 < R; ++d1) {
    const uint32_t i1 = 512 * d1 + t;
    const uint64_t tah = pl.TAh[i1], tah1 = pl.TAh[S::M1 + i1];
#pragma unroll
    for (int c = 0; c < C; ++c) {
      const int idx = d1 * S::ND + 2 * c;
      const uint64_t a0 = gf::mul_u32(tah, dg[d1][2 * c] << ((nowrap >> (2 * idx + 1)) & 1u));
      const uint64_t a1 = gf::mul_u32(tah1, dg[d1][2 * c + 1] << ((nowrap >> (2 * idx + 3)) & 1u));
      x[C * d1 + c] = {a0, a1};
    }
    if (sub != 0 && T == 0 && i1 == 0) x[0].a = gf::sub(x[0].a, uint64_t(sub));
  }
#define MI355_CALL(W) stage_r_fwd_const<R, W>(x)
  MI355_SWITCH8(wave, MI355_CALL)
#undef MI355_CALL
  uint64_t sw[8];
  {
    const uint32_t k1 = (t & 7) >> LC, b = t >> 3;
    const uint64_t* __restrict__ tw = pl.S1r + b * (8 * R) + k1 * 8;
#pragma unroll
    for (int k2 = 0; k2 < 8; ++k2) sw[k2] = tw[k2];
  }
  EXCH_THREAD_MAJOR_TO_STRIDED(X, x, t)
  dft8p<false, 2>(x);
#pragma unroll
  for (int k2 = 0; k2 < 8; ++k2) x[k2] = p2_mul(x[k2], sw[k2]);
  const uint32_t fc = t & (C - 1), fkb = ((t >> (3 + LC)) & (R - 1)) + R * ((t >> LC) & 7) + 8 * R * (t >> 6), fi2 = C * T + fc;
  const uint64_t fca0 = pl.F0f[size_t(T) * 512 + t], fB = pl.FBf[fi2];
  EXCH_THREAD_MAJOR_TO_STRIDED(X, x, t)
  dft8p<false, 1>(x);
  seam64<false, true>(x, wave);
  {
    const uint32_t off = ((lane >> (3 + LC)) << (3 + LC)) | ((lane & 7) << LC) | ((lane >> 3) & (C - 1));
    lds_barrier();
#pragma unroll
    for (int k = 0; k < 8; ++k) X[phys(wave * 512 + k * 64 + off)] = x[k];
    lds_barrier();
#pragma unroll
    for (int j = 0; j < 8; ++j) x[j] = X[phys(j * 512 + t)];
  }
  dft8p<false, 2>(x);
  {
    const uint32_t kb = fkb, i2 = fi2;
    const uint64_t B = fB;
    uint64_t ca = fca0;
    const uint32_t row0 = __brev(kb) >> (32 - S::LM);
    P2* W = reinterpret_cast<P2*>(Wout);
#pragma unroll
    for (int j = 0; j < 8; ++j) {
      const uint32_t rj = ((j & 1) << 2) | (j & 2) | (j >> 2);
      w_store(&W[size_t(row0 + rj) * pl.M2 + i2], P2{gf::mul(x[j].a, ca), gf::mul(x[j].b, ca)});
      if (j < 7) ca = gf::mul(ca, B);
    }
// ... 293 lines not shown
```

### prmers_amd/csrc/kernels_v2_common.hpp

```cpp
#pragma once
#include <hip/hip_runtime.h>
#include <stdint.h>

#include "gfdft.hpp"
#include "kernels.hpp"

namespace mi355 {
namespace v2 {

struct alignas(16) P2 { uint64_t a, b; };

__device__ __forceinline__ uint32_t phys(uint32_t i) { return i ^ ((i >> 3) & 15u); }
constexpr uint32_t kLdsSlots = 4096;
constexpr uint32_t kLdsBytes = kLdsSlots * 16;

__device__ __forceinline__ void w_store(P2* p, P2 v) { *p = v; }
__device__ __forceinline__ P2 w_load(const P2* p) { return *p; }

__device__ __forceinline__ P2 p2_mul(P2 x, uint64_t w) { return {gf::mul(x.a, w), gf::mul(x.b, w)}; }

template <bool INV, int LAZY = 0>
__device__ __forceinline__ void dft8p(P2 (&x)[8]) {
  uint64_t u[8], v[8];
#pragma unroll
  for (int j = 0; j < 8; ++j) { u[j] = x[j].a; v[j] = x[j].b; }
  gf::dft8<INV, LAZY>(u);
  gf::dft8<INV, LAZY>(v);
#pragma unroll
  for (int j = 0; j < 8; ++j) x[j] = {u[j], v[j]};
}

template <int W, bool INV>
__device__ __forceinline__ void seam64_const(P2 (&x)[8]) {
#pragma unroll
  for (int k = 1; k < 8; ++k) {
    const unsigned f = (gf::LOG2_W64 * unsigned(k) * unsigned(W)) % 192u;
    const unsigned s = INV ? (192u - f) % 192u : f;
    x[k] = {gf::mul_pow2(x[k].a, s), gf::mul_pow2(x[k].b, s)};
  }
}
template <bool INV, bool FOLD0 = false>
__device__ __forceinline__ void seam64(P2 (&x)[8], uint32_t wave) {
  switch (wave) {
    case 0:
      if (FOLD0) {
#pragma unroll
        for (int k = 1; k < 4; ++k) x[k] = {gf::fold(x[k].a), gf::fold(x[k].b)};
        x[5] = {gf::fold(x[5].a), gf::fold(x[5].b)};
      }
      break;
    case 1: seam64_const<1, INV>(x); break;
    case 2: seam64_const<2, INV>(x); break;
    case 3: seam64_const<3, INV>(x); break;
    case 4: seam64_const<4, INV>(x); break;
    case 5: seam64_const<5, INV>(x); break;
    case 6: seam64_const<6, INV>(x); break;
    default: seam64_const<7, INV>(x); break;
  }
}

#define MI355_SWITCH8(w, CALL) \
  switch (w) {                 \
    case 0: CALL(0); break;    \
    case 1: CALL(1); break;    \
    case 2: CALL(2); break;    \
    case 3: CALL(3); break;    \
    case 4: CALL(4); break;    \
    case 5: CALL(5); break;    \
    case 6: CALL(6); break;    \
    default: CALL(7); break;   \
  }

__device__ __forceinline__ uint64_t tw_lookup(const DevPlan& pl, uint64_t e) {
  const uint64_t lo = pl.TWlo[e & ((1u << pl.twh) - 1)], hi = pl.TWhi[e >> pl.twh];
  return gf::mul(lo, hi);
}

extern __shared__ __attribute__((aligned(16))) unsigned char smem_v2[];

__device__ __forceinline__ uint32_t tile_of_block(const DevPlan& pl, uint32_t b, uint32_t nblocks) {
  if (!(pl.tune & 1) && (nblocks % 8 == 0)) return (b & 7) * (nblocks >> 3) + (b >> 3);
  return b;
}
__device__ __forceinline__ void boost_if_late(uint32_t boost_from) {
  if (blockIdx.x >= boost_from) __builtin_amdgcn_s_setprio(3);
}

__device__ __forceinline__ void lds_barrier() {
  asm volatile("s_waitcnt lgkmcnt(0)\n\ts_barrier" ::: "memory");
}

#if defined(MI355_PROBE)
#define PROBE_BEGIN(pl)                                                                             \
  uint64_t pb_r0_ = 0, pb_c0_ = 0, pb_rm_ = 0;                                                      \
  if (pl.probe) { pb_r0_ = __builtin_amdgcn_s_memrealtime(); pb_c0_ = __builtin_amdgcn_s_memtime(); }
#define PROBE_MID(pl) if (pl.probe) pb_rm_ = __builtin_amdgcn_s_memrealtime();
#define PROBE_END(pl)                                                                               \
  if (pl.probe && threadIdx.x == 0) {                                                               \
    uint64_t* o_ = pl.probe + size_t(blockIdx.x) * 8;                                               \
    o_[0] = pb_r0_; o_[1] = __builtin_amdgcn_s_memrealtime(); o_[2] = pb_c0_; o_[3] = __builtin_amdgcn_s_memtime(); \
    o_[4] = __builtin_amdgcn_s_getreg((31 << 11) | 4); o_[5] = __builtin_amdgcn_s_getreg((31 << 11) | 20); o_[6] = pb_rm_; \
  }
#define PROBE_BLOCK(pl) (pl.probe_mod ? blockIdx.x % pl.probe_mod : blockIdx.x)
#define PROBE_GRID(pl) (pl.probe_mod ? pl.probe_mod : gridDim.x)
#else
#define PROBE_BEGIN(pl)
#define PROBE_MID(pl)
#define PROBE_END(pl)
#define PROBE_BLOCK(pl) blockIdx.x
#define PROBE_GRID(pl) gridDim.x
#endif

#define EXCH_THREAD_MAJOR_TO_STRIDED(X, x, t)                      \
  lds_barrier();                                                   \
  _Pragma("unroll") for (int r_ = 0; r_ < 8; ++r_) X[phys((t) * 8 + r_)] = x[r_]; \
  lds_barrier();                                                   \
  _Pragma("unroll") for (int j_ = 0; j_ < 8; ++j_) x[j_] = X[phys(j_ * 512 + (t))];

#define EXCH_STRIDED_TO_THREAD_MAJOR(X, x, t)                      \
  lds_barrier();                                                   \
  _Pragma("unroll") for (int j_ = 0; j_ < 8; ++j_) X[phys(j_ * 512 + (t))] = x[j_]; \
  lds_barrier();                                                   \
  _Pragma("unroll") for (int r_ = 0; r_ < 8; ++r_) x[r_] = X[phys((t) * 8 + r_)];

__device__ __forceinline__ uint64_t carry_in_of(const DevPlan& pl, const uint64_t* cbuf, uint32_t T, uint32_t i1) {
  const uint32_t NT = pl.M2 / pl.C;
  if (T > 0) return cbuf[size_t(T - 1) * pl.M1 + i1];
  return cbuf[size_t(NT - 1) * pl.M1 + (i1 ? i1 - 1 : pl.M1 - 1)];
}

template <bool INV>
__device__ __forceinline__ void dft4(uint64_t& x0, uint64_t& x1, uint64_t& x2, uint64_t& x3) {
  const uint64_t a0 = gf::add(x0, x2), a1 = gf::add(x1, x3), b0 = gf::sub(x0, x2);
  const uint64_t b1 = gf::mul_pow2(INV ? gf::sub(x3, x1) : gf::sub(x1, x3), 48);
  x0 = gf::add(a0, a1); x2 = gf::sub(a0, a1); x1 = gf::add(b0, b1); x3 = gf::sub(b0, b1);
}

template <int ND>
__device__ __forceinline__ void apply_carry_in(const DevPlan& pl, uint32_t di, int run, uint64_t cin, uint32_t (&d)[ND]) {
#pragma unroll
  for (int k = 0; k < 3; ++k) {
    const uint32_t width = pl.q + ((di >> (2 * (run * ND + k))) & 1u);
    const uint64_t v = uint64_t(d[k]) + cin;
    d[k] = __builtin_amdgcn_ubfe(uint32_t(v), 0u, width);
    cin = v >> width;
  }
  d[3] += uint32_t(cin);
}

}

hipError_t v5_configure();

}
```

### prmers_amd/csrc/kernels_v3.hip

```cpp
#include "kernels_v2_common.hpp"

namespace mi355 {
namespace v3 {
using v2::P2;
using v2::lds_barrier;

constexpr uint32_t kThreads = 256;
constexpr uint32_t kLdsBytes = 1024 * 16;

__device__ __forceinline__ uint32_t m0(uint32_t i) { return i; }
__device__ __forceinline__ uint32_t m2(uint32_t i) { return i ^ ((i >> 2) & 15u); }
__device__ __forceinline__ uint32_t m3(uint32_t i) { return i ^ ((i >> 3) & 15u); }

struct Pairs {
  using E = P2;
  static constexpr uint32_t kBlock = kThreads, pln = 0;
  const uint32_t t = threadIdx.x;
  template <class I> __device__ __forceinline__ I at(I i) const { return i; }
  __device__ __forceinline__ P2 halves(const uint64_t* __restrict__ tab) const { return {tab[t], tab[256 + t]}; }
  static __device__ __forceinline__ uint32_t edge(uint32_t i) { return m3(i); }
};
struct Planes {
  using E = uint64_t;
  static constexpr uint32_t kBlock = 2 * kThreads;
  const uint32_t t = threadIdx.x >> 1, pln = threadIdx.x & 1u;
  template <class I> __device__ __forceinline__ I at(I i) const { return 2 * i + pln; }
  __device__ __forceinline__ uint64_t halves(const uint64_t* __restrict__ tab) const { return tab[256 * pln + t]; }
  static __device__ __forceinline__ uint32_t edge(uint32_t i) { return m2(i); }
};
__device__ __forceinline__ uint64_t swap_planes(uint64_t v) {
  const uint32_t lo = uint32_t(__builtin_amdgcn_update_dpp(0, int(uint32_t(v)), 0xB1, 0xF, 0xF, false));
  const uint32_t hi = uint32_t(__builtin_amdgcn_update_dpp(0, int(uint32_t(v >> 32)), 0xB1, 0xF, 0xF, false));
  return (uint64_t(hi) << 32) | lo;
}

template <bool INV>
__device__ __forceinline__ void dft4(P2 (&x)[4]) {
  v2::dft4<INV>(x[0].a, x[1].a, x[2].a, x[3].a);
  v2::dft4<INV>(x[0].b, x[1].b, x[2].b, x[3].b);
}
template <bool INV>
__device__ __forceinline__ void dft4(uint64_t (&x)[4]) { v2::dft4<INV>(x[0], x[1], x[2], x[3]); }
__device__ __forceinline__ P2 mulw(P2 x, uint64_t w) { return v2::p2_mul(x, w); }
__device__ __forceinline__ uint64_t mulw(uint64_t x, uint64_t w) { return gf::mul(x, w); }
template <class E>
__device__ __forceinline__ void twiddle3(E (&x)[4], const uint64_t (&w)[3]) {
#pragma unroll
  for (int k = 1; k < 4; ++k) x[k] = mulw(x[k], w[k - 1]);
}

__device__ __forceinline__ uint32_t hi2(uint32_t t) { return t >> 6; }
__device__ __forceinline__ uint32_t d2nd(uint32_t t) { return (t >> 4) & 3u; }
__device__ __forceinline__ uint32_t d3rd(uint32_t t) { return (t >> 2) & 3u; }
__device__ __forceinline__ uint32_t idx_a(uint32_t t, uint32_t j) { return 256u * j + t; }
__device__ __forceinline__ uint32_t idx_b(uint32_t t, uint32_t j) { return 256u * hi2(t) + 64u * j + (t & 63u); }
__device__ __forceinline__ uint32_t idx_c(uint32_t t, uint32_t j) { return 256u * hi2(t) + 64u * d2nd(t) + 16u * j + (t & 15u); }
__device__ __forceinline__ uint32_t idx_d(uint32_t t, uint32_t j) { return (t & ~3u) * 4u + 4u * j + (t & 3u); }
__device__ __forceinline__ uint32_t idx_e(uint32_t t, uint32_t j) { return 4u * t + j; }

using Idx = uint32_t (*)(uint32_t, uint32_t);
using Map = uint32_t (*)(uint32_t);
template <Idx WI, Idx RI, Map MAP, class Form>
__device__ __forceinline__ void exchange(const Form& f, typename Form::E (&x)[4]) {
  typename Form::E* X = reinterpret_cast<typename Form::E*>(v2::smem_v2);
  lds_barrier();
#pragma unroll
  for (int k = 0; k < 4; ++k) X[f.at(MAP(WI(f.t, k)))] = x[k];
  lds_barrier();
#pragma unroll
  for (int j = 0; j < 4; ++j) x[j] = X[f.at(MAP(RI(f.t, j)))];
}

template <class Form, int NS>
__device__ __forceinline__ void forward3(const Form& f, typename Form::E (&x)[4], const uint64_t (&w)[NS][3]) {
  dft4<false>(x); twiddle3(x, w[0]); exchange<idx_a, idx_b, m0>(f, x);
  dft4<false>(x); twiddle3(x, w[1]); exchange<idx_b, idx_c, m0>(f, x);
  dft4<false>(x); twiddle3(x, w[2]); exchange<idx_c, idx_d, m2>(f, x);
}
template <class Form, int NS>
__device__ __forceinline__ void inverse3(const Form& f, typename Form::E (&x)[4], const uint64_t (&v)[NS][3]) {
  exchange<idx_d, idx_c, m2>(f, x); twiddle3(x, v[2]); dft4<true>(x);
  exchange<idx_c, idx_b, m0>(f, x); twiddle3(x, v[1]); dft4<true>(x);
  exchange<idx_b, idx_a, m0>(f, x); twiddle3(x, v[0]); dft4<true>(x);
}

struct RowWords { uint64_t w[4][3], v[4][3]; };
template <bool INVERSE_TOO>
__device__ __forceinline__ void rows_prefetch(const uint64_t* __restrict__ UT, uint32_t t, RowWords& tw) {
#pragma unroll
  for (uint32_t k = 1; k < 4; ++k) {
    const uint32_t e[4] = {k * t, 4 * k * (t & 63u), 16 * k * (t & 15u), 64 * k * (t & 3u)};
#pragma unroll
    for (int s = 0; s < 4; ++s) tw.w[s][k - 1] = UT[e[s]];
    if (INVERSE_TOO) {
#pragma unroll
      for (int s = 0; s < 4; ++s) tw.v[s][k - 1] = UT[(1024 - e[s]) & 1023];
    }
  }
}
template <class Form>
__device__ __forceinline__ void rows_forward(const Form& f, typename Form::E (&x)[4], const RowWords& tw) {
  forward3(f, x, tw.w);
  dft4<false>(x); twiddle3(x, tw.w[3]); exchange<idx_d, idx_e, m2>(f, x);
  dft4<false>(x);
}
template <class Form>
__device__ __forceinline__ void rows_inverse(const Form& f, typename Form::E (&x)[4], const RowWords& tw) {
  dft4<true>(x);
  exchange<idx_e, idx_d, m2>(f, x); twiddle3(x, tw.v[3]); dft4<true>(x);
  inverse3(f, x, tw.v);
}

template <int mode>
__device__ __forceinline__ void pointwise(const Pairs& f, P2 (&x)[4], uint64_t rho0, const uint64_t* __restrict__ Y, const uint64_t* __restrict__ Y2, size_t base) {
#pragma unroll
  for (int k5 = 0; k5 < 4; ++k5) {
    const P2 u = x[k5];
    P2 r;
    uint64_t q, s0;
    if (mode == 0) {
      q = gf::mul(gf::sqr(u.b), rho0);
      s0 = gf::sqr(u.a);
      r.b = gf::dbl(gf::mul(u.b, u.a));
    } else {
      P2 y = reinterpret_cast<const P2*>(Y + base)[256 * k5 + f.t];
      if (mode == 3) {
        const P2 z = reinterpret_cast<const P2*>(Y2 + base)[256 * k5 + f.t];
        y = {gf::add_lazy_any(y.a, z.a), gf::add_lazy_any(y.b, z.b)};
      }
      q = gf::mul(gf::mul(u.b, y.b), rho0);
      s0 = gf::mul(u.a, y.a);
      r.b = gf::add(gf::mul(u.a, y.b), gf::mul(u.b, y.a));
    }
    if (k5 & 1) q = gf::mul_pow2(q, 48);
    r.a = (k5 & 2) ? gf::sub(s0, q) : gf::add(s0, q);
    x[k5] = r;
  }
}
template <int mode>
__device__ __forceinline__ void pointwise(const Planes& f, uint64_t (&x)[4], uint64_t rho0, const uint64_t* __restrict__ Y, const uint64_t* __restrict__ Y2, size_t base) {
#pragma unroll
  for (int k5 = 0; k5 < 4; ++k5) {
    const uint64_t u = x[k5], uo = swap_planes(u);
    uint64_t m1, cross;
    if (mode == 0) {
      m1 = gf::sqr(u);
      cross = gf::dbl(gf::mul(u, uo));
    } else {
      uint64_t y = (Y + base)[f.at(256 * k5 + f.t)];
      if (mode == 3) y = gf::add_lazy_any(y, (Y2 + base)[f.at(256 * k5 + f.t)]);
      const uint64_t yo = swap_planes(y);
      m1 = gf::mul(u, y);
      const uint64_t mx = gf::mul(u, yo);
      cross = gf::add(mx, swap_planes(mx));
    }
    uint64_t q = swap_planes(gf::mul(m1, rho0));
    if (k5 & 1) q = gf::mul_pow2(q, 48);
    const uint64_t ra = (k5 & 2) ? gf::sub(m1, q) : gf::add(m1, q);
    x[k5] = f.pln ? cross : ra;
  }
}

template <class Form, int mode>
__global__ void __launch_bounds__(Form::kBlock) k2_rows1024(DevPlan pl, const uint64_t* __restrict__ Win, const uint64_t* __restrict__ Yimg,
                                                            const uint64_t* __restrict__ Yimg2, uint64_t* __restrict__ Wimg, uint64_t* __restrict__ Wout) {
  using E = typename Form::E;
  const Form f;
  const uint32_t t = f.t, row = blockIdx.x;
  const size_t base = size_t(row) * 2048;
  const E* in = reinterpret_cast<const E*>(Win + base);
  E* out = reinterpret_cast<E*>(Wout + base);
  E x[4];
#pragma unroll
  for (int j = 0; j < 4; ++j) x[j] = in[f.at(256 * j + t)];
  RowWords tw;
  rows_prefetch<mode != 2>(pl.UT2, t, tw);
  const uint32_t kb = hi2(t) + 4 * d2nd(t) + 16 * d3rd(t) + 64 * (t & 3u);
  const uint32_t blk = row / pl.L1, qq = row - blk * pl.L1;
  const uint32_t k1row = col_label(pl, blk, pl.logL1 ? (__brev(qq) >> (32 - pl.logL1)) : 0u);
  const uint64_t erho = rho_exponent(pl, k1row, kb);
  uint64_t rho_lo = 0, rho_hi = 0;
  if (mode != 2) { rho_lo = pl.TWlo[erho & ((1u << pl.twh) - 1)]; rho_hi = pl.TWhi[erho >> pl.twh]; }

  rows_forward(f, x, tw);
  if (mode == 4) {
    E* img = reinterpret_cast<E*>(Wimg + base);
#pragma unroll
    for (int j = 0; j < 4; ++j) img[f.at(256 * j + t)] = x[j];
  }
  if (mode != 2) {
    pointwise<(mode == 4 ? 0 : mode)>(f, x, gf::mul(rho_lo, rho_hi), Yimg, Yimg2, base);
    rows_inverse(f, x, tw);
  }
#pragma unroll
  for (int j = 0; j < 4; ++j) out[f.at(256 * j + t)] = x[j];
}

__device__ __forceinline__ uint32_t rev2(uint32_t k) { return ((k & 1u) << 1) | (k >> 1); }

template <bool INV>
__device__ __forceinline__ void cols_prefetch(const uint64_t* __restrict__ UT, uint32_t t, uint64_t (&w)[3][3]) {
#pragma unroll
  for (uint32_t k = 1; k < 4; ++k) {
    const uint32_t e[3] = {k * (t >> 2), 4 * k * ((t >> 2) & 15u), 16 * k * ((t >> 2) & 3u)};
#pragma unroll
    for (int s = 0; s < 3; ++s) w[s][k - 1] = UT[INV ? (256 - e[s]) & 255 : e[s]];
  }
}
template <class Form>
__device__ __forceinline__ void cols_forward(const Form& f, typename Form::E (&x)[4], const uint64_t (&w)[3][3]) {
  exchange<idx_e, idx_a, Form::edge>(f, x);
  forward3(f, x, w);
  dft4<false>(x);
}
template <class Form>
__device__ __forceinline__ void cols_inverse(const Form& f, typename Form::E (&x)[4], const uint64_t (&v)[3][3]) {
  dft4<true>(x);
  inverse3(f, x, v);
  exchange<idx_a, idx_e, Form::edge>(f, x);
}
__device__ __forceinline__ void load_run(const uint32_t* __restrict__ digits, uint32_t T, uint32_t t, uint32_t (&dg)[8]) {
  const uint4* src = reinterpret_cast<const uint4*>(digits) + (size_t(T) * 256 + t) * 2;
  const uint4 a = src[0], b = src[1];
  dg[0] = a.x; dg[1] = a.y; dg[2] = a.z; dg[3] = a.w; dg[4] = b.x; dg[5] = b.y; dg[6] = b.z; dg[7] = b.w;
}
template <class E>
__device__ __forceinline__ void chain4(E (&x)[4], uint64_t ca, uint64_t ratio) {
#pragma unroll
  for (int j = 0; j < 4; ++j) {
    x[j] = mulw(x[j], ca);
    if (j < 3) ca = gf::mul(ca, ratio);
  }
}

__device__ __forceinline__ void weigh(const Pairs&, P2 tah, uint32_t nowrap, const uint32_t (&dg)[8], P2 (&x)[4]) {
#pragma unroll
  for (int c = 0; c < 4; ++c)
    x[c] = {gf::mul_u32(tah.a, dg[2 * c] << ((nowrap >> (4 * c + 1)) & 1u)), gf::mul_u32(tah.b, dg[2 * c + 1] << ((nowrap >> (4 * c + 3)) & 1u))};
}
__device__ __forceinline__ void weigh(const Planes& f, uint64_t tah, uint32_t nowrap, const uint32_t (&dg)[8], uint64_t (&x)[4]) {
#pragma unroll
  for (int c = 0; c < 4; ++c) {
    const uint32_t d = dg[2 * c] ^ ((dg[2 * c] ^ dg[2 * c + 1]) & (0u - f.pln));
    const uint32_t sh = nowrap >> (4 * c + 1 + 2 * f.pln);
    x[c] = gf::mul_u32(tah, d << (sh & 1u));
  }
}

template <class Form>
__global__ void __launch_bounds__(Form::kBlock) k1_cols256(DevPlan pl, const uint32_t* __restrict__ digits, const uint64_t* __restrict__ cbuf_in,
                                                           uint64_t* __restrict__ Wout) {
  using E = typename Form::E;
  const Form f;
  const uint32_t t = f.t, T = blockIdx.x;
  uint64_t w[3][3];
  cols_prefetch<false>(pl.UT1, t, w);
  const uint32_t c4 = t & 3u, kb = hi2(t) + 4 * d2nd(t) + 16 * d3rd(t), i2 = 4 * T + c4;
  const uint64_t fca0 = pl.F0f[size_t(T) * kThreads + t], fB = pl.FBf[i2];
  const uint32_t di = pl.DI[size_t(T) * kThreads + t];
  const E tah = f.halves(pl.TAh);
  uint32_t dg[8];
  load_run(digits, T, t, dg);
  asm volatile("" ::: "memory");
  if (cbuf_in) v2::apply_carry_in<8>(pl, di, 0, v2::carry_in_of(pl, cbuf_in, T, t), dg);
  E x[4];
  weigh(f, tah, ~di, dg, x);
  cols_forward(f, x, w);
  chain4(x, fca0, fB);
  const uint32_t row0 = __brev(kb) >> 24;
  E* W = reinterpret_cast<E*>(Wout);
#pragma unroll
  for (int j = 0; j < 4; ++j) W[f.at(size_t(row0 + rev2(j)) * pl.M2 + i2)] = x[j];
}

__device__ __forceinline__ void unweigh(const Pairs&, uint32_t di, P2 tai, P2 tai2, const P2 (&x)[4], uint64_t (&u)[8]) {
#pragma unroll
  for (int k = 0; k < 8; ++k) {
    const bool wrap = ((di >> (2 * k)) & 2u) != 0;
    u[k] = (k & 1) ? gf::mul(x[k >> 1].b, wrap ? tai2.b : tai.b) : gf::mul(x[k >> 1].a, wrap ? tai2.a : tai.a);
  }
}
__device__ __forceinline__ void unweigh(const Planes& f, uint32_t di, uint64_t tai, uint64_t tai2, const uint64_t (&x)[4], uint64_t (&u)[8]) {
  uint64_t own[4], oth[4];
#pragma unroll
  for (int c = 0; c < 4; ++c) {
    const bool wrap = ((di >> (2 * (2 * c + int(f.pln)))) & 2u) != 0;
    own[c] = gf::mul(x[c], wrap ? tai2 : tai);
  }
#pragma unroll
  for (int c = 0; c < 4; ++c) oth[c] = swap_planes(own[c]);
#pragma unroll
  for (int k = 0; k < 8; ++k) u[k] = ((k & 1) == int(f.pln)) ? own[k >> 1] : oth[k >> 1];
}
__device__ __forceinline__ uint32_t adc_mul(uint64_t u, uint32_t a, uint32_t addend, uint32_t width, uint64_t& carry) {
  if (a == 1) {
    const uint64_t r = u + carry + addend;
    carry = r >> width;
    return __builtin_amdgcn_ubfe(uint32_t(r), 0u, width);
  }
  const uint64_t mask = (uint64_t(1) << width) - 1;
  const uint64_t dlo = u & mask, chi = u >> width;
  const uint64_t r = dlo * a + carry + addend;
  carry = (r >> width) + chi * a;
  return uint32_t(r & mask);
}
__device__ __forceinline__ void store_run(const Pairs&, uint32_t* __restrict__ digits, uint64_t* __restrict__ cbuf, size_t run, const uint32_t (&dg)[8], uint64_t carry) {
  uint4* dst = reinterpret_cast<uint4*>(digits) + run * 2;
  dst[0] = make_uint4(dg[0], dg[1], dg[2], dg[3]); dst[1] = make_uint4(dg[4], dg[5], dg[6], dg[7]);
  cbuf[run] = carry;
}
__device__ __forceinline__ void store_run(const Planes& f, uint32_t* __restrict__ digits, uint64_t* __restrict__ cbuf, size_t run, const uint32_t (&dg)[8], uint64_t carry) {
  uint4* dst = reinterpret_cast<uint4*>(digits) + run * 2;
  dst[f.pln] = f.pln ? make_uint4(dg[4], dg[5], dg[6], dg[7]) : make_uint4(dg[0], dg[1], dg[2], dg[3]);
  if (!f.pln) cbuf[run] = carry;
}

template <class Form, bool EXT>
__global__ void __launch_bounds__(Form::kBlock) k3_cols256(DevPlan pl, const uint64_t* __restrict__ Win, uint32_t* __restrict__ digits, uint64_t* __restrict__ cbuf,
                                                           uint32_t a, BackExt ext) {
  using E = typename Form::E;
  const Form f;
  const uint32_t t = f.t, T = v2::tile_of_block(pl, blockIdx.x, gridDim.x);
  uint64_t v[3][3];
  cols_prefetch<true>(pl.UT1, t, v);
  const uint32_t c4 = t & 3u, kb = hi2(t) + 4 * d2nd(t) + 16 * d3rd(t), i2 = 4 * T + c4;
  const uint32_t di = pl.DI[size_t(T) * kThreads + t];
  const E tai = f.halves(pl.TAi);
  const uint64_t ca = pl.F0i[size_t(T) * kThreads + t], B = pl.FBi[i2];
  const uint32_t row0 = __brev(kb) >> 24;
  const E* W = reinterpret_cast<const E*>(Win);
  E x[4];
#pragma unroll
  for (int j = 0; j < 4; ++j) x[j] = W[f.at(size_t(row0 + rev2(j)) * pl.M2 + i2)];
  uint32_t ad[8] = {0, 0, 0, 0, 0, 0, 0, 0};
  if (EXT && ext.add_digits) {
// ... 72 lines not shown
```

### prmers_amd/csrc/plan.hpp

```cpp
#pragma once
#include <algorithm>
#include <cstddef>
#include <cstdint>
#include <cstdio>
#include <cstdlib>
#include <cstring>
#include <stdexcept>
#include <string>
#include <vector>

#include "gf.hpp"

namespace mi355 {

inline size_t transform_size(uint32_t exponent) {
  uint32_t w = 0, log2_n = 1, log2_n5 = 2;
  do { ++log2_n; w = exponent >> log2_n; } while ((w + 1) * 2 + log2_n >= 64);
  do { ++log2_n5; w = exponent / (5u << log2_n5); } while ((w + 1) * 2 + (log2_n5 + 2.4) >= 64);
  const size_t invalid = size_t(-1);
  const size_t n2 = (log2_n <= 26) ? (size_t(1) << log2_n) : invalid;
  const size_t n5 = (log2_n5 <= 26) ? (size_t(5) << log2_n5) : invalid;
  return n2 < n5 ? n2 : n5;
}

inline int ilog2(size_t v) { int r = -1; while (v) { v >>= 1; ++r; } return r; }

inline uint32_t bitrev(uint32_t i, int bits) {
  uint32_t r = 0;
  for (int k = 0; k < bits; ++k) { r = (r << 1) | (i & 1); i >>= 1; }
  return r;
}

struct Plan {
  uint32_t p = 0;
  size_t n = 0, m = 0;
  uint32_t r5 = 1;
  uint32_t M1 = 1, M2 = 1;
  uint32_t L1 = 1, logL1 = 0, logM2 = 0;
  uint32_t C = 1;
  bool split5 = false;
  uint32_t q = 0, t = 0;
  uint32_t twh = 0;
  uint32_t a_fast = 1;
  bool sum_fast = false;
  size_t lds_front = 0, lds_mid = 0;

  std::vector<uint32_t> SA, SB;
  std::vector<uint64_t> TA, TAi, TB, TBi;
  std::vector<uint64_t> TWlo, TWhi;
  std::vector<uint64_t> UT1, UT2;
  std::vector<uint64_t> S2r, S2ri, S1r, S1ri;
  std::vector<uint32_t> DI;
  uint64_t I4 = 0, I4inv = 0;
  uint64_t W5[5] = {1, 0, 0, 0, 0}, W5i[5] = {1, 0, 0, 0, 0};
  uint64_t W5c[4] = {0, 0, 0, 0};

  size_t tiles() const { return M2 / C; }
  size_t runs() const { return tiles() * M1; }

  uint32_t width_of_s(uint64_t s) const {
    return q + ((s + t > 0) ? 1u : 0u) + ((s + t > n) ? 1u : 0u) - ((s > 0) ? 1u : 0u);
  }
  uint32_t width(size_t j) const { return width_of_s((uint64_t(p) * j) % n); }

  size_t pos(size_t j) const {
    const size_t i = j >> 1, b = j & 1;
    const size_t i1 = i / M2, i2 = i % M2;
    const size_t T = i2 / C, c = i2 % C;
    return ((T * M1 + i1) * C + c) * 2 + b;
  }

  std::string describe() const {
    char buf[160];
    std::snprintf(buf, sizeof buf, "marin-hip:n=%zu:m1=%u:m2=%u:c=%u%s", n, M1, M2, C, split5 ? ":split5" : "");
    return buf;
  }
};

inline bool carry_chain_ok(uint32_t q, size_t n, uint32_t C, uint64_t a, unsigned mult) {
  typedef unsigned __int128 u128;
  const u128 field = (u128(1) << 64) - (u128(1) << 32) + 1, lim = u128(1) << 64;
  const u128 D = (u128(1) << (q + 1)) - 1;
  const size_t runs = n / (2 * size_t(C));
  u128 E = D;
  for (int it = 0; it < 64; ++it) {
    const u128 U = u128(mult) * ((C >= 2) ? u128(n - runs) * D * D + u128(runs) * E * E : u128(n) * D * D);
    if (U >= field) return false;
    const u128 chi = U >> q;
    u128 c = 0;
    for (int k = 0; k < 4096; ++k) {
      const u128 r = D * a + c + (u128(1) << 32);
      if (r >= lim) return false;
      const u128 c2 = (r >> q) + chi * a;
      if (c2 >= lim) return false;
      if (c2 == c) break;
      c = c2;
    }
    if (C < 2) return true;
    const u128 E2 = D + (c >> (3 * q)) + 3;
    if (E2 >= (u128(1) << 31)) return false;
    if (E2 <= E) return true;
    E = E2;
  }
  return false;
}
inline bool fused_factor_ok(uint32_t q, size_t n, uint32_t C, uint64_t a) { return carry_chain_ok(q, n, C, a, 1); }

inline bool sum_product_ok(uint32_t q, size_t n, uint32_t C) { return carry_chain_ok(q, n, C, 1, 4); }

enum class ColKernels : uint8_t {
  kGeneric,
  kSplit,
  kRadix8R1, kRadix8R2, kRadix8R4,
  kRadix4Pairs, kRadix4Planes,
  kRadix5, kRadix5J1,
};
enum class RowKernels : uint8_t {
  kGeneric,
  kRadix4Pairs, kRadix4Planes,
  kRadix8,
  kRadix8Wide,
  kRows2048One, kRows2048Two,
};

struct KernelChoice {
  ColKernels cols = ColKernels::kGeneric;
  RowKernels rows = RowKernels::kGeneric;
  bool resident_cols() const { return cols != ColKernels::kGeneric && cols != ColKernels::kSplit; }
  bool fused_back() const { return cols != ColKernels::kSplit; }
};

inline KernelChoice served_kernels(uint32_t r5, uint32_t M1, uint32_t M2, uint32_t C, bool split5) {
  KernelChoice k;
  if (split5) k.cols = ColKernels::kSplit;
  else if (r5 == 5 && ((M1 == 1280 && C == 4) || (M1 == 2560 && C == 2)) && M2 >= 8)
    k.cols = M1 == 2560 ? ColKernels::kRadix5J1 : ColKernels::kRadix5;
  else if (r5 == 1 && M1 == 256 && C == 4 && M2 >= 8)
    k.cols = M2 / 4 <= 512 ? ColKernels::kRadix4Planes : ColKernels::kRadix4Pairs;
  else if (r5 == 1 && (M1 == 512 || M1 == 1024 || M1 == 2048) && M1 * C == 4096 && M2 >= 2 * C)
    k.cols = M1 == 512 ? ColKernels::kRadix8R1 : M1 == 1024 ? ColKernels::kRadix8R2 : ColKernels::kRadix8R4;
  if (M2 == 1024) k.rows = M1 < 512 ? RowKernels::kRadix4Planes : RowKernels::kRadix4Pairs;
  else if (M2 == 4096) k.rows = RowKernels::kRadix8;
  else if (M2 == 8192) k.rows = RowKernels::kRadix8Wide;
  else if (M2 == 2048 && (M1 < 512 || M1 == 1280)) k.rows = RowKernels::kRows2048One;
  else if (M2 == 2048 && M1 % 2 == 0 && M1 >= 512) k.rows = RowKernels::kRows2048Two;
  return k;
}

inline uint32_t threads_per_tile(ColKernels c) {
  switch (c) {
    case ColKernels::kRadix8R1: case ColKernels::kRadix8R2: case ColKernels::kRadix8R4: return 512;
    case ColKernels::kRadix4Pairs: case ColKernels::kRadix4Planes: return 256;
    case ColKernels::kRadix5: case ColKernels::kRadix5J1: return 640;
    default: return 0;
  }
}

inline uint32_t fused_factor_limit(uint32_t q, size_t n, uint32_t C) {
  uint64_t lo = 1, hi = 0xffffffffu;
  if (!fused_factor_ok(q, n, C, 1)) return 1;
  while (lo < hi) {
    const uint64_t mid = (lo + hi + 1) / 2;
    if (fused_factor_ok(q, n, C, mid)) lo = mid; else hi = mid - 1;
  }
  return uint32_t(C >= 2 ? lo : std::min<uint64_t>(lo, 15));
}

inline Plan make_plan(uint32_t p, const char* spec = nullptr, bool build_tables = true) {
  if (p < 3) throw std::runtime_error("exponent must be >= 3");
  Plan pl;
  pl.p = p;
  pl.n = transform_size(p);
  if (pl.n == size_t(-1)) throw std::runtime_error("exponent too large for the Goldilocks IBDWT");
  pl.m = pl.n / 2;
  pl.r5 = (pl.m % 5 == 0) ? 5 : 1;
  const int k = ilog2(pl.m / pl.r5);

  long want_m2 = -1, want_c = -1;
  bool want_split = false;
  if (spec && *spec) {
    std::string s(spec);
    for (size_t i = 0; i < s.size();) {
      size_t e = s.find_first_of(",:; ", i);
      if (e == std::string::npos) e = s.size();
      const std::string tok = s.substr(i, e - i);
      if (tok.rfind("m2=", 0) == 0) want_m2 = std::atol(tok.c_str() + 3);
      else if (tok.rfind("c=", 0) == 0) want_c = std::atol(tok.c_str() + 2);
      else if (tok == "split5") want_split = true;
      else if (!tok.empty() && tok != "marin-hip" && tok.rfind("n=", 0) != 0 && tok.rfind("m1=", 0) != 0)
        throw std::runtime_error("unknown plan token '" + tok + "'");
      i = e + 1;
    }
  }

  int b = (k + 3) / 2;
  const int bmin = k - (pl.r5 == 5 ? 8 : 10);
  if (b < bmin) b = bmin;
  if (b > 12) b = 12;
  if (b > k) b = k;
  if (b < 1) b = 1;
  if (want_m2 > 0) {
    b = ilog2(size_t(want_m2));
    if ((long(1) << b) != want_m2 || b > k || b < 1 || b > 13) throw std::runtime_error("bad m2 in plan spec");
  } else {
    while ((pl.m >> b) > (pl.r5 == 5 ? 2560u : 2048u) && b < 13 && b < k) ++b;
    if (pl.r5 == 5 && (pl.m >> b) > 10240 && b < k) b = std::min(13, k);
  }
  pl.logM2 = uint32_t(b);
  pl.M2 = 1u << b;
  pl.M1 = uint32_t(pl.m / pl.M2);
  pl.L1 = pl.M1 / pl.r5;
  pl.logL1 = uint32_t(ilog2(pl.L1));
  if (want_split && pl.r5 != 5) throw std::runtime_error("split5 needs a 5 * 2^k transform");
  pl.split5 = want_split || size_t(pl.M1) * 16 > 160 * 1024;
  if (pl.split5 && (pl.r5 != 5 || size_t(pl.L1) * 16 > 128 * 1024)) throw std::runtime_error("transform size not supported (columns beyond the split sweeps)");

  uint32_t C = 1;
  while (C * 2 <= pl.M2 && size_t(pl.M1) * (C * 2) <= 4096 && C < 16) C *= 2;
  while (C < 4 && C * 2 <= pl.M2 && size_t(pl.M1) * (C * 2) <= 8192 && !(pl.r5 == 1 && pl.M1 == 2048)) C *= 2;
  while (C > 4 && pl.M2 / C < 256) C /= 2;
  if (C == 1 && pl.M2 >= 2 && size_t(pl.M1) * 2 * 16 <= 160 * 1024 && pl.n >= (size_t(1) << 19)) C = 2;
  if (pl.split5) C = 1;
  if (pl.r5 == 1 && pl.M1 == 256 && pl.M2 >= 8 && C > 4 && !pl.split5) C = 4;
  if (want_c > 0 && !pl.split5) {
    C = uint32_t(want_c);
    if ((C & (C - 1)) != 0 || C > pl.M2 || size_t(pl.M1) * C > 10240) throw std::runtime_error("bad c in plan spec");
  }
  pl.C = C;
  pl.lds_front = pl.split5 ? 0 : size_t(pl.M1) * pl.C * 16;
  pl.lds_mid = size_t(pl.M2) * 16;
  pl.q = uint32_t(p / pl.n);
  pl.t = uint32_t(p % pl.n);
  pl.a_fast = fused_factor_limit(pl.q, pl.n, pl.C);
  pl.sum_fast = sum_product_ok(pl.q, pl.n, pl.C);
  if (!build_tables) return pl;

  const size_t n = pl.n, m = pl.m;
  const uint64_t r = gf::root_of_two(n);
  const uint64_t om = gf::root_of_unity(m);
  const uint64_t inv_m = gf::inv(uint64_t(m) % gf::P);

  pl.SA.resize(2 * size_t(pl.M1)); pl.TA.resize(2 * size_t(pl.M1)); pl.TAi.resize(2 * size_t(pl.M1));
  for (uint32_t i1 = 0; i1 < 2 * pl.M1; ++i1) {
    const uint64_t s0 = (uint64_t(2) * pl.M2 % n * (uint64_t(p) % n) % n * (i1 % pl.M1)) % n;
    const uint64_t s = (i1 < pl.M1) ? s0 : (s0 + pl.t) % n;
    pl.SA[i1] = uint32_t(s);
    pl.TA[i1] = gf::pow(r, (n - s) % n);
    pl.TAi[i1] = gf::mul(gf::inv(pl.TA[i1]), inv_m);
  }
  pl.SB.resize(2 * size_t(pl.M2)); pl.TB.resize(2 * size_t(pl.M2)); pl.TBi.resize(2 * size_t(pl.M2));
  for (uint32_t x = 0; x < 2 * pl.M2; ++x) {
    const uint64_t s = (uint64_t(p) * x) % n;
    pl.SB[x] = uint32_t(s);
    pl.TB[x] = gf::pow(r, (n - s) % n);
    pl.TBi[x] = gf::inv(pl.TB[x]);
  }
  pl.twh = uint32_t((ilog2(m) + 2) / 2);
  const size_t lo_n = size_t(1) << pl.twh, hi_n = ((m + (size_t(1) << 20)) >> pl.twh) + 2;
  pl.TWlo.resize(lo_n); pl.TWhi.resize(hi_n);
  pl.TWlo[0] = 1; for (size_t i = 1; i < lo_n; ++i) pl.TWlo[i] = gf::mul(pl.TWlo[i - 1], om);
  const uint64_t step = gf::mul(pl.TWlo[lo_n - 1], om);
  pl.TWhi[0] = 1; for (size_t i = 1; i < hi_n; ++i) pl.TWhi[i] = gf::mul(pl.TWhi[i - 1], step);
  const uint64_t om1 = gf::pow(om, pl.M2), om2 = gf::pow(om, pl.M1);
  pl.UT1.resize(pl.M1); pl.UT1[0] = 1; for (uint32_t i = 1; i < pl.M1; ++i) pl.UT1[i] = gf::mul(pl.UT1[i - 1], om1);
  pl.UT2.resize(pl.M2); pl.UT2[0] = 1; for (uint32_t i = 1; i < pl.M2; ++i) pl.UT2[i] = gf::mul(pl.UT2[i - 1], om2);
  const KernelChoice kc = served_kernels(pl.r5, pl.M1, pl.M2, pl.C, pl.split5);
  if (kc.rows == RowKernels::kRadix8 || kc.rows == RowKernels::kRadix8Wide) {
    const uint32_t st = pl.M2 / 4096;
    pl.S2r.resize(4096); pl.S2ri.resize(4096);
    for (uint32_t b = 0; b < 64; ++b) for (uint32_t ka = 0; ka < 64; ++ka) {
      const uint32_t e = ka * b;
      const uint32_t idx = b * 64 + (ka & 7) * 8 + (ka >> 3);
      pl.S2r[idx] = pl.UT2[st * e]; pl.S2ri[idx] = pl.UT2[st * ((4096 - e) & 4095)];
    }
  }
  if (kc.rows == RowKernels::kRows2048One || kc.rows == RowKernels::kRows2048Two) {
    pl.S2r.resize(4096); pl.S2ri.resize(4096);
    for (uint32_t b = 0; b < 64; ++b) for (uint32_t k1 = 0; k1 < 8; ++k1) for (uint32_t k2 = 0; k2 < 8; ++k2) {
      const uint32_t e = (((k1 & 3) + 4 * k2) * b) & 2047;
      pl.S2r[b * 64 + k1 * 8 + k2] = pl.UT2[e]; pl.S2ri[b * 64 + k1 * 8 + k2] = pl.UT2[(2048 - e) & 2047];
    }
  }
  const uint32_t tpt = threads_per_tile(kc.cols);
  if (tpt == 512) {
    const uint32_t ka_n = pl.M1 / 64;
    pl.S1r.resize(pl.M1); pl.S1ri.resize(pl.M1);
    for (uint32_t b = 0; b < 64; ++b) for (uint32_t ka = 0; ka < ka_n; ++ka) {
      const uint32_t e = ka * b;
      const uint32_t Rr = pl.M1 / 512, idx = b * ka_n + (ka % Rr) * 8 + (ka / Rr);
      pl.S1r[idx] = pl.UT1[e]; pl.S1ri[idx] = pl.UT1[(pl.M1 - e) & (pl.M1 - 1)];
    }
  }
  if (m % 4 == 0) { pl.I4 = gf::pow(om, m / 4); pl.I4inv = gf::inv(pl.I4); }
  else { pl.I4 = gf::root_of_unity(4); pl.I4inv = gf::inv(pl.I4); }
  if (tpt) {
    const uint32_t NR = pl.M1 / tpt, ND = 2 * pl.C;
    pl.DI.assign(pl.tiles() * tpt, 0u);
    for (size_t T = 0; T < pl.tiles(); ++T)
      for (uint32_t t = 0; t < tpt; ++t) {
        uint32_t w = 0;
        for (uint32_t d1 = 0; d1 < NR; ++d1)
          for (uint32_t k = 0; k < ND; ++k) {
            const uint32_t i1 = tpt * d1 + t, i2 = uint32_t(T) * pl.C + (k >> 1);
            const uint64_t sb = pl.SB[2 * i2 + (k & 1)], s = (uint64_t(pl.SA[i1]) + sb) % n;
            const uint64_t wa = (k & 1) ? pl.SA[pl.M1 + i1] : pl.SA[i1], wb = pl.SB[2 * i2];
            const uint32_t wbit = pl.width_of_s(s) - pl.q, wrap = (wa > 0 && wb > 0 && wa + wb <= n) ? 1u : 0u;
            w |= (wbit | (wrap << 1)) << (2 * (d1 * ND + k));
          }
        pl.DI[T * tpt + t] = w;
      }
  }
  if (pl.I4 != (uint64_t(1) << 48)) throw std::runtime_error("internal: omega_4 is expected to be 2^48");
  if (pl.r5 == 5) {
    const uint64_t w5 = gf::pow(om, m / 5);
    for (int i = 0; i < 5; ++i) { pl.W5[i] = gf::pow(w5, uint64_t(i)); pl.W5i[i] = gf::inv(pl.W5[i]); }
    const uint64_t a = gf::add(pl.W5[1], pl.W5[4]), b = gf::add(pl.W5[2], pl.W5[3]);
    const uint64_t k1 = gf::half(gf::sub(pl.W5[1], pl.W5[4])), k2 = gf::half(gf::sub(pl.W5[2], pl.W5[3]));
    pl.W5c[0] = gf::half(gf::half(gf::sub(a, b))); pl.W5c[1] = k1; pl.W5c[2] = gf::sub(k2, k1); pl.W5c[3] = gf::add(k1, k2);
  }
  return pl;
}

inline KernelChoice choose_kernels(const Plan& pl, const char* mi355_kernels) {
  KernelChoice k = served_kernels(pl.r5, pl.M1, pl.M2, pl.C, pl.split5);
  const std::string sel = mi355_kernels ? mi355_kernels : "v2";
  if (sel != "v2" && sel != "v2rows") k.rows = RowKernels::kGeneric;
  if (sel != "v2" && sel != "v2cols" && k.resident_cols()) k.cols = ColKernels::kGeneric;
  return k;
}

}
```

### prmers_amd/csrc/selftest.hip

```cpp
#include <hip/hip_runtime.h>
#include <stdint.h>

#include <stdexcept>
#include <string>
#include <vector>

#include "kernels_v2_common.hpp"
#include "selftest_cases.hpp"

namespace mi355 {

namespace {
using namespace cases;

template <class Fam>
__global__ void k_selftest_family(const uint64_t* __restrict__ in, uint64_t* __restrict__ out, const uint64_t* __restrict__ aux, int n) {
  const int i = blockIdx.x * blockDim.x + threadIdx.x;
  if (i >= n) return;
  Fam::eval(in + size_t(i) * Fam::IN, out + size_t(i) * Fam::OUT, aux);
}

__global__ void k_selftest_dft4(const uint64_t* __restrict__ in, uint64_t* __restrict__ out, int n) {
  const int i = blockIdx.x * blockDim.x + threadIdx.x;
  if (i >= n) return;
  uint64_t f[4], g[4];
  for (int j = 0; j < 4; ++j) f[j] = g[j] = in[size_t(i) * 4 + j];
  v2::dft4<false>(f[0], f[1], f[2], f[3]); v2::dft4<true>(g[0], g[1], g[2], g[3]);
  for (int j = 0; j < 4; ++j) { out[size_t(i) * 8 + j] = f[j]; out[size_t(i) * 8 + 4 + j] = g[j]; }
}

__global__ void __launch_bounds__(512) k_selftest_chain(const uint64_t* __restrict__ tuples, size_t ntuples, const uint64_t* __restrict__ fac, uint64_t* __restrict__ out) {
  const int g = blockIdx.x * 512 + threadIdx.x;
  const uint32_t wave = __builtin_amdgcn_readfirstlane((threadIdx.x >> 6) & 7);
  const uint64_t* ta = tuples + 8 * GfChain::tuple_of(g, 0, ntuples);
  const uint64_t* tb = tuples + 8 * GfChain::tuple_of(g, 1, ntuples);
  uint64_t* o = out + size_t(g) * GfChain::OUT;
  v2::P2 x[8], y[8];
  uint64_t sw[8];
  for (int k = 0; k < 8; ++k) { x[k] = y[k] = {ta[k], tb[k]}; sw[k] = fac[size_t(g) * 8 + k]; }
  v2::dft8p<false, 1>(x);
  v2::seam64<false, true>(x, wave);
  for (int k = 0; k < 8; ++k) { o[k] = x[k].a; o[8 + k] = x[k].b; }
  v2::dft8p<false, 2>(x);
  for (int k = 0; k < 8; ++k) { x[k] = v2::p2_mul(x[k], sw[k]); o[16 + k] = x[k].a; o[24 + k] = x[k].b; }
  v2::dft8p<true>(y);
  v2::seam64<true>(y, wave);
  v2::dft8p<true, 2>(y);
  for (int k = 0; k < 8; ++k) { y[k] = v2::p2_mul(y[k], sw[k]); o[32 + k] = y[k].a; o[40 + k] = y[k].b; }
}

void chk(hipError_t e, const char* what) { if (e != hipSuccess) throw std::runtime_error(std::string("selftest: ") + what + ": " + hipGetErrorString(e)); }

struct DevWords {
  uint64_t* p = nullptr;
  explicit DevWords(size_t n) { chk(hipMalloc(reinterpret_cast<void**>(&p), (n ? n : 1) * 8), "hipMalloc"); }
  explicit DevWords(const std::vector<uint64_t>& v) : DevWords(v.size()) { if (!v.empty()) chk(hipMemcpy(p, v.data(), v.size() * 8, hipMemcpyHostToDevice), "copy"); }
  ~DevWords() { (void)hipFree(p); }
  DevWords(const DevWords&) = delete;
  DevWords& operator=(const DevWords&) = delete;
  void fetch(std::vector<uint64_t>& v, const char* what) const { chk(hipMemcpy(v.data(), p, v.size() * 8, hipMemcpyDeviceToHost), what); }
};

template <class Fam>
void run_family(const char* name, std::vector<uint64_t>& in, std::vector<uint64_t>& out) {
  std::vector<uint64_t> aux;
  in.clear(); Fam::fill(in); Fam::aux(aux);
  const size_t n = in.size() / Fam::IN;
  out.assign(n * Fam::OUT, 0);
  {
    DevWords din(in), daux(aux), dout(out.size());
    hipLaunchKernelGGL(k_selftest_family<Fam>, dim3(uint32_t((n + 63) / 64)), dim3(64), 0, 0, din.p, dout.p, daux.p, int(n));
    chk(hipGetLastError(), name);
    dout.fetch(out, name);
  }
  if (Fam::kHostEqualsDevice) {
    std::vector<uint64_t> h(Fam::OUT);
    for (size_t i = 0; i < n; ++i) {
      Fam::eval(in.data() + i * Fam::IN, h.data(), aux.data());
      for (int k = 0; k < Fam::OUT; ++k)
        if (h[k] != out[i * Fam::OUT + k])
          throw std::runtime_error(std::string("selftest: ") + name + msg(": device and host evaluation differ, case %zu word %d: %016llx / %016llx", i, k, MI355_X(out[i * Fam::OUT + k]), MI355_X(h[k])));
    }
  }
  const std::string err = Fam::check(in.data(), out.data(), n);
  if (!err.empty()) throw std::runtime_error("selftest: " + err);
}
}

void selftest_primitives(int device) {
  chk(hipSetDevice(device), "hipSetDevice");
  std::vector<uint64_t> in, out, tuples, dft8_out;
  run_family<GfScalar>("gf scalars", in, out);
  run_family<GfLazySum>("gf lazy sum", in, out);
  run_family<GfDft8>("gf dft8", tuples, dft8_out);
  {
    in.clear(); GfDft4::fill(in);
    const size_t n = in.size() / GfDft4::IN;
    out.assign(n * GfDft4::OUT, 0);
    DevWords din(in), dout(out.size());
    hipLaunchKernelGGL(k_selftest_dft4, dim3(uint32_t((n + 63) / 64)), dim3(64), 0, 0, din.p, dout.p, int(n));
    chk(hipGetLastError(), "gf dft4");
    dout.fetch(out, "gf dft4");
    const std::string err = GfDft4::check(in.data(), out.data(), n);
    if (!err.empty()) throw std::runtime_error("selftest: " + err);
  }
  {
    std::vector<uint64_t> fac; GfChain::factors(fac);
    const size_t ntuples = tuples.size() / 8;
    out.assign(size_t(GfChain::kThreads) * GfChain::OUT, 0);
    DevWords dt(tuples), df(fac), dout(out.size());
    hipLaunchKernelGGL(k_selftest_chain, dim3(GfChain::kThreads / 512), dim3(512), 0, 0, dt.p, ntuples, df.p, dout.p);
    chk(hipGetLastError(), "gf chain");
    dout.fetch(out, "gf chain");
    const std::string err = GfChain::check(tuples.data(), ntuples, fac.data(), out.data(), dft8_out.data());
    if (!err.empty()) throw std::runtime_error("selftest: " + err);
  }
  run_family<CrtScalar>("crt scalars", in, out);
  run_family<CrtCmul>("crt cmul", in, out);
  run_family<CrtBfly>("crt bfly", in, out);
  run_family<CrtOdd>("crt dft_odd", in, out);
  run_family<CrtWalk>("crt DigitWalk", in, out);
}

}
```

### prmers_amd/csrc/selftest_cases.hpp

```cpp
#pragma once
#include <stdint.h>

#include <cstdarg>
#include <cstdio>
#include <string>
#include <utility>
#include <vector>

#include "crt_arith.hpp"
#include "gfdft.hpp"

namespace mi355 {

void selftest_primitives(int device);

namespace cases {

typedef unsigned __int128 u128;
constexpr uint64_t P = gf::P;

struct Rng {
  uint64_t s;
  explicit Rng(uint64_t seed) : s(seed) {}
  uint64_t next() { s = s * 6364136223846793005ull + 1442695040888963407ull; return s ^ (s >> 29); }
};

inline std::string msg(const char* fmt, ...) __attribute__((format(printf, 1, 2)));
inline std::string msg(const char* fmt, ...) {
  char buf[400];
  va_list ap; va_start(ap, fmt); std::vsnprintf(buf, sizeof buf, fmt, ap); va_end(ap);
  return buf;
}
#define MI355_X(v) ((unsigned long long)(v))

inline uint64_t gf_mulmod(uint64_t a, uint64_t b) { return uint64_t((u128(a % P) * (b % P)) % P); }
inline const uint64_t* gf_pow2_table() {
  static uint64_t t[192];
  if (!t[0]) { t[0] = 1; for (int s = 1; s < 192; ++s) t[s] = uint64_t((u128(t[s - 1]) * 2) % P); }
  return t;
}

inline unsigned mul_tail_case(uint64_t a, uint64_t b) {
  const uint64_t a0 = uint32_t(a), a1 = a >> 32, b0 = uint32_t(b), b1 = b >> 32;
  const uint64_t t0 = a0 * b0, t1 = a0 * b1 + (t0 >> 32);
  const u128 t2w = u128(a1 * b0) + t1;
  const uint64_t t2 = uint64_t(t2w), c = uint64_t(t2w >> 64);
  const uint64_t t3 = a1 * b1 + (t2 >> 32);
  const uint64_t lo = (t2 << 32) | uint32_t(t0), hh = t3 >> 32, hl = uint32_t(t3);
  const unsigned bw = u128(lo) < u128(hh) + c;
  const uint64_t x = lo - hh - c;
  const u128 rw = u128(x) + u128(hl) * 0xffffffffull;
  return bw | unsigned(rw >> 64) << 1 | unsigned(uint64_t(rw) >= P) << 2 | unsigned(c) << 3;
}

template <unsigned... S>
GF_HD void mul_pow2_const(uint64_t x, uint64_t* o, std::integer_sequence<unsigned, S...>) { ((o[S] = gf::mul_pow2(x, S)), ...); }

struct GfScalar {
  static constexpr int IN = 2, OUT = 7 + 192 + 192;
  static constexpr bool kHostEqualsDevice = false;
  static void aux(std::vector<uint64_t>&) {}
  static void edges(std::vector<uint64_t>& e) {
    e = {0, 1, 2, P - 1, P - 2, P, 0xffffffffull, 0x100000000ull, 0xffffffff00000000ull, 0x8000000000000000ull, 0xfffffffeffffffffull, 0x00000000fffffffeull,
         0x123456789abcdef0ull % P,
         0x100000001ull, 0x00000001ffffffffull, 0xfffffffe00000001ull, 0x0000000100000000ull + 0xfffffffeull, 0xffffffff00000000ull - 1, 0x00000000ffff0001ull,
         0xffff0000ffff0001ull,
         0x200000000ull, 0xc000000000000000ull, 0x7fffffffcull, 0xfffffffdffffffffull,
         P + 1, P + 0xfffffffeull, 0xffffffffffffffffull, 0xffffffff80000000ull, 0xffffffff00000002ull, 0xfffffffffffffffeull};
  }
  static void fill(std::vector<uint64_t>& in) {
    std::vector<uint64_t> e; edges(e);
    for (uint64_t x : e) for (uint64_t y : e) { in.push_back(x); in.push_back(y); }
    Rng r(0x9e3779b97f4a7c15ull);
    for (int i = 0; i < 4096; ++i) { in.push_back(r.next() % P); in.push_back(r.next() % P); }
    for (int i = 0; i < 1024; ++i) { in.push_back(r.next() | (i & 1 ? 0xffffffff00000000ull : 0)); in.push_back(r.next() % P); }
    for (int i = 0; i < 1024; ++i) { in.push_back(r.next() % P); in.push_back(r.next() | (i & 1 ? 0xffffffff00000000ull : 0)); }
  }
  static GF_HDM void eval(const uint64_t* in, uint64_t* o, const uint64_t*) {
    const uint64_t x = in[0], y = in[1];
    o[0] = gf::add(x, y);
    o[1] = gf::sub(x, y);
    o[2] = gf::mul(x, y);
    o[3] = gf::add_lazy(x, y);
    o[4] = gf::fold(x + y);
    o[5] = gf::mul_u32(x, uint32_t(y));
    o[6] = gf::fold(x);
    for (unsigned s = 0; s < 192; ++s) o[7 + s] = gf::mul_pow2(x, s);
    mul_pow2_const(x, o + 7 + 192, std::make_integer_sequence<unsigned, 192>());
  }
  static std::string check(const uint64_t* in, const uint64_t* out, size_t n) {
    const uint64_t* p2 = gf_pow2_table();
    unsigned seen = 0;
    for (size_t i = 0; i < n; ++i) {
      const uint64_t x = in[2 * i], y = in[2 * i + 1], xm = x % P, ym = y % P;
      const uint64_t* o = out + i * OUT;
      const uint64_t sum = uint64_t((u128(xm) + ym) % P), dif = uint64_t((u128(xm) + P - ym) % P);
      const bool one_small = x <= P || y <= P;
#define MI355_FAIL(op, s, got) return msg("gf %s: a=%016llx b=%016llx s=%u got %016llx", op, MI355_X(x), MI355_X(y), unsigned(s), MI355_X(got))
      if (x <= P && y <= P && (o[0] % P != sum || o[0] > P)) MI355_FAIL("add", 0, o[0]);
      if (y <= P && (o[1] % P != dif || (x <= P && o[1] > P))) MI355_FAIL("sub", 0, o[1]);
      if (one_small && o[2] != gf_mulmod(x, y)) MI355_FAIL("mul", 0, o[2]);
      if (one_small && o[3] % P != sum) MI355_FAIL("add_lazy", 0, o[3]);
      if (o[4] != (x + y) % P) MI355_FAIL("fold", 0, o[4]);
      if (o[5] != gf_mulmod(x, uint32_t(y))) MI355_FAIL("mul_u32", 0, o[5]);
      if (o[6] != xm) MI355_FAIL("fold", 1, o[6]);
      for (unsigned k = 0; k < 384; ++k) {
        const unsigned s = k % 192;
        const uint64_t r = o[7 + k];
        if (r % P != gf_mulmod(x, p2[s]) || (s != 0 && r > P)) MI355_FAIL(k < 192 ? "mul_pow2" : "mul_pow2 (constant s)", s, r);
      }
#undef MI355_FAIL
      if (one_small) { const unsigned c = mul_tail_case(x, y); seen |= 1u << (c & 3); if ((c & 7) == 4) seen |= 1u << 4; if ((c & 9) == 9) seen |= 1u << 5; }
    }
    if (seen != 0x3f) return msg("gf mul: the operand list misses a tail case (seen mask %02x)", seen);
    return "";
  }
};

struct GfLazySum {
  static constexpr int IN = 2, OUT = 2;
  static constexpr bool kHostEqualsDevice = false;
  static void aux(std::vector<uint64_t>&) {}
  static void fill(std::vector<uint64_t>& in) {
    std::vector<uint64_t> e; GfScalar::edges(e);
    for (uint64_t x : e) for (uint64_t y : e) { in.push_back(x); in.push_back(y); }
    Rng r(0xa4093822299f31d0ull);
    for (int i = 0; i < 4096; ++i) { in.push_back(r.next()); in.push_back(r.next()); }
    for (int i = 0; i < 4096; ++i) {
      const uint64_t hi = 0xffffffff00000000ull, lo = 0xfffffffe00000000ull;
      in.push_back((r.next() & 0xffffffffull) | (i & 1 ? hi : lo)); in.push_back((r.next() & 0xffffffffull) | (i & 2 ? hi : lo));
    }
  }
  static GF_HDM void eval(const uint64_t* in, uint64_t* o, const uint64_t*) {
    o[0] = gf::add_lazy_any(in[0], in[1]);
    o[1] = gf::mul(o[0], in[0]);
  }
  static std::string check(const uint64_t* in, const uint64_t* out, size_t n) {
    size_t both_lazy = 0, sum_lazy = 0;
    for (size_t i = 0; i < n; ++i) {
      const uint64_t x = in[2 * i], y = in[2 * i + 1];
      const uint64_t sum = uint64_t((u128(x % P) + y % P) % P);
      if (out[2 * i] % P != sum) return msg("gf add_lazy_any: a=%016llx b=%016llx got %016llx", MI355_X(x), MI355_X(y), MI355_X(out[2 * i]));
      if (out[2 * i + 1] != gf_mulmod(sum, x)) return msg("gf mul of a lazy sum: a=%016llx b=%016llx got %016llx", MI355_X(x), MI355_X(y), MI355_X(out[2 * i + 1]));
      both_lazy += (x > P && y > P); sum_lazy += out[2 * i] > P;
    }
    if (!both_lazy || !sum_lazy) return msg("gf add_lazy_any: the operand list misses a lazy case (both operands above P: %zu, sum above P: %zu)", both_lazy, sum_lazy);
    return "";
  }
};

inline const std::vector<uint64_t>& gf_alphabet() {
  static const std::vector<uint64_t> a = {0, 1, P - 1, P - 2, 0xffffffffull, P - 0xffffffffull, P - 0x100000000ull, 0x8000000000000000ull, 0x7fffffff80000001ull, P};
  return a;
}
inline void gf_direct_dft(const uint64_t* x, uint64_t* y, int N, unsigned lw) {
  const uint64_t* p2 = gf_pow2_table();
  for (int k = 0; k < N; ++k) {
    u128 s = 0;
    for (int j = 0; j < N; ++j) s += gf_mulmod(x[j], p2[(lw * unsigned(j * k)) % 192]);
    y[k] = uint64_t(s % P);
  }
}
inline void gf_tuples(std::vector<uint64_t>& in, int N, int sampled9, int sampled10, int random) {
  const std::vector<uint64_t>& a = gf_alphabet();
  for (uint64_t v : a) for (int j = 0; j < N; ++j) in.push_back(v);
  Rng r(0x243f6a8885a308d3ull);
  for (int i = 0; i < sampled9; ++i) for (int j = 0; j < N; ++j) in.push_back(a[r.next() % 9]);
  for (int i = 0; i < sampled10; ++i) for (int j = 0; j < N; ++j) in.push_back(a[r.next() % 10]);
  for (int i = 0; i < random; ++i) for (int j = 0; j < N; ++j) in.push_back(r.next() % P);
}

struct GfDft8 {
  static constexpr int IN = 8, OUT = 48;
  static constexpr bool kHostEqualsDevice = false;
  static void aux(std::vector<uint64_t>&) {}
  static void fill(std::vector<uint64_t>& in) {
    gf_tuples(in, 8, 2048, 1024, 512);
    const std::vector<uint64_t>& a = gf_alphabet();
    const int where[4][4] = {{0, 2, 4, 6}, {1, 3, 5, 7}, {0, 1, 4, 5}, {0, 3, 4, 7}};
    for (const auto& w : where)
      for (int p = 0; p < 9; ++p) for (int q = 0; q < 9; ++q) for (int r = 0; r < 9; ++r) for (int s = 0; s < 9; ++s) {
        uint64_t v[8] = {};
        v[w[0]] = a[p]; v[w[1]] = a[q]; v[w[2]] = a[r]; v[w[3]] = a[s];
        for (int j = 0; j < 8; ++j) in.push_back(v[j]);
      }
  }
  static GF_HDM void eval(const uint64_t* in, uint64_t* o, const uint64_t*) {
    uint64_t x[6][8];
    for (int v = 0; v < 6; ++v) for (int j = 0; j < 8; ++j) x[v][j] = in[j];
    gf::dft8<false, 0>(x[0]); gf::dft8<false, 1>(x[1]); gf::dft8<false, 2>(x[2]);
    gf::dft8<true, 0>(x[3]); gf::dft8<true, 1>(x[4]); gf::dft8<true, 2>(x[5]);
    for (int v = 0; v < 6; ++v) for (int j = 0; j < 8; ++j) o[8 * v + j] = x[v][j];
  }
  static bool may_be_lazy(int lazy, int slot) { return lazy == 2 ? slot != 7 : lazy == 1 ? (slot == 1 || slot == 2 || slot == 3 || slot == 5) : false; }
  static std::string check(const uint64_t* in, const uint64_t* out, size_t n, size_t* counts = nullptr) {
    size_t above[6][8] = {};
    for (size_t i = 0; i < n; ++i) {
      uint64_t want[2][8];
      gf_direct_dft(in + 8 * i, want[0], 8, 120); gf_direct_dft(in + 8 * i, want[1], 8, 72);
      for (int v = 0; v < 6; ++v) for (int k = 0; k < 8; ++k) {
        const uint64_t r = out[i * OUT + 8 * v + k];
        if (r % P != want[v / 3][k] || (!may_be_lazy(v % 3, k) && r > P))
          return msg("gf dft8<%s, %d> slot %d: got %016llx want %016llx, input %016llx %016llx %016llx %016llx %016llx %016llx %016llx %016llx", v / 3 ? "inverse" : "forward",
                     v % 3, k, MI355_X(r), MI355_X(want[v / 3][k]), MI355_X(in[8 * i]), MI355_X(in[8 * i + 1]), MI355_X(in[8 * i + 2]), MI355_X(in[8 * i + 3]),
                     MI355_X(in[8 * i + 4]), MI355_X(in[8 * i + 5]), MI355_X(in[8 * i + 6]), MI355_X(in[8 * i + 7]));
        above[v][k] += r > P;
      }
    }
    if (counts) for (int v = 0; v < 6; ++v) for (int k = 0; k < 8; ++k) counts[8 * v + k] = above[v][k];
    for (int v = 0; v < 6; ++v) for (int k = 0; k < 8; ++k)
      if (may_be_lazy(v % 3, k) && !above[v][k]) return msg("gf dft8<%s, %d>: no case left a value above P in slot %d", v / 3 ? "inverse" : "forward", v % 3, k);
    return "";
  }
};

struct GfDft4 {
  static constexpr int IN = 4, OUT = 8;
  static void fill(std::vector<uint64_t>& in) {
    const std::vector<uint64_t>& a = gf_alphabet();
    for (uint64_t p : a) for (uint64_t q : a) for (uint64_t r : a) for (uint64_t s : a) { in.push_back(p); in.push_back(q); in.push_back(r); in.push_back(s); }
    gf_tuples(in, 4, 0, 0, 512);
  }
  static std::string check(const uint64_t* in, const uint64_t* out, size_t n) {
    for (size_t i = 0; i < n; ++i) {
      uint64_t want[2][4];
      gf_direct_dft(in + 4 * i, want[0], 4, 48); gf_direct_dft(in + 4 * i, want[1], 4, 144);
      for (int k = 0; k < 8; ++k) {
        const uint64_t r = out[i * OUT + k];
        if (r % P != want[k / 4][k % 4] || r > P)
          return msg("gf dft4<%s> slot %d: got %016llx want %016llx, input %016llx %016llx %016llx %016llx", k / 4 ? "inverse" : "forward", k % 4, MI355_X(r),
                     MI355_X(want[k / 4][k % 4]), MI355_X(in[4 * i]), MI355_X(in[4 * i + 1]), MI355_X(in[4 * i + 2]), MI355_X(in[4 * i + 3]));
      }
    }
    return "";
  }
};

struct GfChain {
  static constexpr int OUT = 48, kThreads = 512 * 8;
  static void factors(std::vector<uint64_t>& f) {
    Rng r(0x13198a2e03707344ull);
    const uint64_t e[4] = {0, 1, P - 1, 0xffffffffull};
    for (int i = 0; i < kThreads * 8; ++i) { const uint64_t v = r.next(); f.push_back((v & 0x1f) < 4 ? e[v & 3] : v % P); }
  }
  static GF_HDM size_t tuple_of(int g, int plane, size_t ntuples) { return (size_t(2 * g + plane) * 7) % ntuples; }
  static unsigned seam_shift(int k, int w, bool inv) { const unsigned f = (gf::LOG2_W64 * unsigned(k) * unsigned(w)) % 192u; return inv ? (192u - f) % 192u : f; }
  static std::string check(const uint64_t* tuples, size_t ntuples, const uint64_t* fac, const uint64_t* out, const uint64_t* dft8_out) {
    const uint64_t* p2 = gf_pow2_table();
    size_t folded[8] = {};
    for (int g = 0; g < kThreads; ++g) {
      const int w = (g >> 6) & 7;
      for (int plane = 0; plane < 2; ++plane) {
        const size_t tu = tuple_of(g, plane, ntuples);
        const uint64_t* in = tuples + 8 * tu;
        const uint64_t* o = out + size_t(g) * OUT;
        for (int inv = 0; inv < 2; ++inv) {
          uint64_t a[8], b[8], c[8];
          gf_direct_dft(in, a, 8, inv ? 72 : 120);
          for (int k = 0; k < 8; ++k) b[k] = gf_mulmod(a[k], p2[seam_shift(k, w, inv)]);
          gf_direct_dft(b, c, 8, inv ? 72 : 120);
          for (int k = 0; k < 8; ++k) {
            const uint64_t want = gf_mulmod(c[k], fac[size_t(g) * 8 + k]);
            if (!inv) {
              const uint64_t s1 = o[8 * plane + k];
              if (s1 % P != b[k] || s1 > P)
                return msg("gf chain forward, after seam64 at wave %d, slot %d: got %016llx want %016llx (tuple %zu)", w, k, MI355_X(s1), MI355_X(b[k]), tu);
            }
            const uint64_t r = o[(inv ? 32 : 16) + 8 * plane + k];
            if (r != want) return msg("gf chain %s, after the multiplication, wave %d slot %d: got %016llx want %016llx (tuple %zu)", inv ? "inverse" : "forward", w, k, MI355_X(r), MI355_X(want), tu);
          }
        }
        if (w == 0) for (int k = 0; k < 8; ++k) folded[k] += dft8_out[tu * GfDft8::OUT + 8 * 1 + k] > P;
      }
    }
    for (int k : {1, 2, 3, 5})
      if (!folded[k]) return msg("gf chain: wave 0 (the FOLD0 case of seam64) met no value above P in slot %d", k);
    return "";
  }
};

using crt::F31; using crt::F61; using crt::M31; using crt::M61;

struct Cx { uint64_t re, im; };
inline Cx cx_mul(Cx a, Cx b, uint64_t m) {
  const u128 re = (u128(a.re % m) * (b.re % m) + u128(m - a.im % m) * (b.im % m)) % m, im = (u128(a.re % m) * (b.im % m) + u128(a.im % m) * (b.re % m)) % m;
  return {uint64_t(re), uint64_t(im)};
}
inline Cx cx_add(Cx a, Cx b, uint64_t m) { return {uint64_t((u128(a.re % m) + b.re % m) % m), uint64_t((u128(a.im % m) + b.im % m) % m)}; }
inline Cx cx_conj(Cx a, uint64_t m) { return {a.re % m, (m - a.im % m) % m}; }
inline void cx_direct_dft(const Cx* x, Cx* y, int N, Cx w, uint64_t m) {
  Cx pw[16]; pw[0] = {1, 0};
  for (int e = 1; e < N; ++e) pw[e] = cx_mul(pw[e - 1], w, m);
  for (int k = 0; k < N; ++k) { Cx s{0, 0}; for (int q = 0; q < N; ++q) s = cx_add(s, cx_mul(x[q], pw[(q * k) % N], m), m); y[k] = s; }
}
inline Cx root_of_radix(int R, uint64_t m, bool inv) {
  const uint64_t h = m == M61 ? (1ull << 30) : (1ull << 15);
  const Cx w = R == 8 ? Cx{h, h} : R == 4 ? Cx{0, 1} : Cx{m - 1, 0};
  return inv ? cx_conj(w, m) : w;
}
// ... 284 lines not shown
```

Before: 6304 iter/s.

## Square pointwise pairs with three multiplies using tau = sqrt(-rho) twiddles

Replaces the pointwise squaring of (a + b·X) modulo X^2 - rho, which took four multiplies (a², b², b²·rho, a·b), with a three-multiply form: t = b·tau, ra = (a + t)(a - t), rb = a·b, where tau² = -rho. It adds tau root tables from a 2m-th root of unity, and a second device plan for the squaring back pass whose inverse tables are doubled to absorb the dropped factor of 2 in rb. The squaring modes of the row kernels now look up tau instead of rho, and the per-k4 tau sequence is built with shifts. This cuts multiplies in the middle pass at the cost of more table memory and extra plan state.

```diff
diff --git a/prmers_amd/csrc/engine.hip b/prmers_amd/csrc/engine.hip
--- a/prmers_amd/csrc/engine.hip
+++ b/prmers_amd/csrc/engine.hip
@@ -76,8 +76,10 @@
   auto padded = [](size_t bytes) { return (bytes + 255) & ~size_t(255); };
   std::vector<uint64_t> tah(pl_.TA.size()), tai2(pl_.TAi.size());
   for (size_t i = 0; i < tah.size(); ++i) { tah[i] = gf::half(pl_.TA[i]); tai2[i] = gf::dbl(pl_.TAi[i]); }
-  const size_t total = padded(pl_.SA.size() * 4) + padded(pl_.SB.size() * 4) + padded(pl_.TA.size() * 8) * 4 +
-                       padded(pl_.TB.size() * 8) * 2 + padded(pl_.TWlo.size() * 8) + padded(pl_.TWhi.size() * 8) +
+  std::vector<uint64_t> tai_sq(pl_.TAi), tai2_sq(tai2);
+  for (size_t i = pl_.M1; i < tai_sq.size(); ++i) { tai_sq[i] = gf::dbl(tai_sq[i]); tai2_sq[i] = gf::dbl(tai2_sq[i]); }
+  const size_t total = padded(pl_.SA.size() * 4) + padded(pl_.SB.size() * 4) + padded(pl_.TA.size() * 8) * 6 +
+                       padded(pl_.TB.size() * 8) * 2 + (padded(pl_.TWlo.size() * 8) + padded(pl_.TWhi.size() * 8)) * 2 +
                        padded(pl_.UT1.size() * 8) + padded(pl_.UT2.size() * 8) + padded(pl_.S2r.size() * 8) * 2 +
                        padded(pl_.S1r.size() * 8) * 2 + 1024;
   HIPCHK(hipMalloc(&tables_, total));
@@ -94,6 +96,10 @@
   dp_.TBi = upload(cur, base, pl_.TBi, host);
   dp_.TWlo = upload(cur, base, pl_.TWlo, host);
   dp_.TWhi = upload(cur, base, pl_.TWhi, host);
+  dp_.TAUlo = upload(cur, base, pl_.TAUlo, host);
+  dp_.TAUhi = upload(cur, base, pl_.TAUhi, host);
+  const uint64_t* tai_sq_dev = upload(cur, base, tai_sq, host);
+  const uint64_t* tai2_sq_dev = upload(cur, base, tai2_sq, host);
   dp_.UT1 = upload(cur, base, pl_.UT1, host);
   dp_.UT2 = upload(cur, base, pl_.UT2, host);
   dp_.S2r = pl_.S2r.empty() ? nullptr : upload(cur, base, pl_.S2r, host);
@@ -152,6 +158,9 @@
     HIPCHK(hipStreamSynchronize(stream_));
     dp_.F0f = f0_; dp_.F0i = f0_ + nt; dp_.FBf = f0_ + 2 * nt; dp_.FBi = f0_ + 2 * nt + pl_.M2;
   }
+
+  dp_sq_ = dp_;
+  dp_sq_.TAi = tai_sq_dev; dp_sq_.TAi2 = tai2_sq_dev;
 
   width_ = host_digits::digit_widths(p, pl_.n);
   cg_ = CanonGeom::tile_major(dp_, p);
@@ -206,11 +215,12 @@
 
 void Engine::run_middle(const uint64_t* in, const uint64_t* y, uint64_t* out, int mode, const uint64_t* y2, uint64_t* img) {
   HIPCHK(rows_(dp_, in, y, y2, img, out, mode, stream_));
+  rows_mode_ = mode;
 }
 
 void Engine::run_back(size_t r, uint32_t a, hipEvent_t* ev) {
-  if (kc_.cols == ColKernels::kSplit) HIPCHK(launch_back_split(dp_, work(), split_, digits(r), cbuf(r), a, stream_));
-  else HIPCHK(cols_.back(dp_, work(), digits(r), cbuf(r), a, stream_));
+  if (kc_.cols == ColKernels::kSplit) HIPCHK(launch_back_split(back_plan(), work(), split_, digits(r), cbuf(r), a, stream_));
+  else HIPCHK(cols_.back(back_plan(), work(), digits(r), cbuf(r), a, stream_));
   if (ev) HIPCHK(hipEventRecord(ev[0], stream_));
   if (pl_.C >= 2) pending_carry_[r] = 1;
   else carry_fix_now(r);
@@ -482,7 +492,7 @@
   if (copy_to >= 0 && size_t(copy_to) != dst) { x.digits2 = digits(size_t(copy_to)); x.cbuf2 = cbuf(size_t(copy_to)); }
   if (add_src >= 0) { x.add_digits = digits(size_t(add_src)); x.add_cbuf = pending_carry_[size_t(add_src)] ? cbuf(size_t(add_src)) : nullptr; }
   uint64_t* fresh = take_spare_cbuf();
-  HIPCHK(cols_.back_ext(dp_, work(), digits(dst), fresh, a, x, stream_));
+  HIPCHK(cols_.back_ext(back_plan(), work(), digits(dst), fresh, a, x, stream_));
   adopt_cbuf(dst, fresh);
   const size_t outs[2] = {dst, x.digits2 ? size_t(copy_to) : dst};
   for (int i = 0; i < (x.digits2 ? 2 : 1); ++i) {
diff --git a/prmers_amd/csrc/engine.hpp b/prmers_amd/csrc/engine.hpp
--- a/prmers_amd/csrc/engine.hpp
+++ b/prmers_amd/csrc/engine.hpp
@@ -92,6 +92,9 @@
 
   Plan pl_;
   DevPlan dp_{};
+  DevPlan dp_sq_{};
+  int rows_mode_ = -1;
+  const DevPlan& back_plan() const { return (rows_mode_ == 0 || rows_mode_ == 4) ? dp_sq_ : dp_; }
   CanonGeom cg_{};
   int device_ = 0;
   bool verbose_ = false;
diff --git a/prmers_amd/csrc/gfdft.hpp b/prmers_amd/csrc/gfdft.hpp
--- a/prmers_amd/csrc/gfdft.hpp
+++ b/prmers_amd/csrc/gfdft.hpp
@@ -33,4 +33,10 @@
   x[3] = (LAZY >= 1) ? add_lazy(f0, f1) : add(f0, f1); x[7] = sub(f0, f1);
 }
 
+GF_HD void sqr3(uint64_t a, uint64_t b, uint64_t tau, uint64_t& ra, uint64_t& rb) {
+  const uint64_t t = mul(b, tau);
+  ra = mul(add_lazy(t, a), sub(a, t));
+  rb = mul(b, a);
 }
+
+}
diff --git a/prmers_amd/csrc/kernels.hip b/prmers_amd/csrc/kernels.hip
--- a/prmers_amd/csrc/kernels.hip
+++ b/prmers_amd/csrc/kernels.hip
@@ -2,7 +2,7 @@
 #include <stdint.h>
 #include <stdlib.h>
 
-#include "gf.hpp"
+#include "gfdft.hpp"
 #include "kernels.hpp"
 
 namespace mi355 {
@@ -16,6 +16,10 @@
 
 __device__ __forceinline__ uint64_t tw_lookup(const DevPlan& pl, uint64_t e) {
   const uint64_t lo = pl.TWlo[e & ((1u << pl.twh) - 1)], hi = pl.TWhi[e >> pl.twh];
+  return gf::mul(lo, hi);
+}
+__device__ __forceinline__ uint64_t tau_lookup(const DevPlan& pl, uint64_t e) {
+  const uint64_t lo = pl.TAUlo[e & ((1u << pl.twh) - 1)], hi = pl.TAUhi[e >> pl.twh];
   return gf::mul(lo, hi);
 }
 
@@ -282,7 +286,7 @@
   uint64_t pre_lo = 0, pre_hi = 0;
   if (one && tid < M2 && mode != 2) {
     const uint64_t ex = rho_exponent(pl, k1, __brev(tid) >> (32 - pl.logM2));
-    pre_lo = pl.TWlo[ex & ((1u << pl.twh) - 1)]; pre_hi = pl.TWhi[ex >> pl.twh];
+    pre_lo = (mode == 0 ? pl.TAUlo : pl.TWlo)[ex & ((1u << pl.twh) - 1)]; pre_hi = (mode == 0 ? pl.TAUhi : pl.TWhi)[ex >> pl.twh];
   }
   lds_pow2_dft<false>(X, M2, pl.logM2, 1, 1, 0, pl.UT2, M2, 1, pl.I4, tid, nthr);
   if (mode == 2) {
@@ -296,12 +300,11 @@
   const P2* Y = reinterpret_cast<const P2*>(Yimg) + size_t(row) * M2;
   for (uint32_t e = tid; e < M2; e += nthr) {
     const uint32_t k2 = __brev(e) >> (32 - pl.logM2);
-    const uint64_t rho = one ? gf::mul(pre_lo, pre_hi) : tw_lookup(pl, rho_exponent(pl, k1, k2));
+    const uint64_t rho = one ? gf::mul(pre_lo, pre_hi) : mode == 0 ? tau_lookup(pl, rho_exponent(pl, k1, k2)) : tw_lookup(pl, rho_exponent(pl, k1, k2));
     const P2 u = X[e];
     P2 r;
     if (mode == 0) {
-      r.a = gf::add(gf::sqr(u.a), gf::mul(gf::sqr(u.b), rho));
-      r.b = gf::mul(u.b, gf::dbl(u.a));
+      gf::sqr3(u.a, u.b, rho, r.a, r.b);
     } else {
       P2 y = Y[e];
       if (mode == 3) {
diff --git a/prmers_amd/csrc/kernels.hpp b/prmers_amd/csrc/kernels.hpp
--- a/prmers_amd/csrc/kernels.hpp
+++ b/prmers_amd/csrc/kernels.hpp
@@ -10,6 +10,7 @@
   const uint64_t *TA, *TAi, *TB, *TBi;
   const uint64_t *TAh, *TAi2;
   const uint64_t *TWlo, *TWhi, *UT1, *UT2;
+  const uint64_t *TAUlo, *TAUhi;
   const uint64_t *S2r, *S2ri, *S1r, *S1ri;
   uint64_t I4, I4inv;
   uint64_t W5c[4];
diff --git a/prmers_amd/csrc/kernels_v2.hip b/prmers_amd/csrc/kernels_v2.hip
--- a/prmers_amd/csrc/kernels_v2.hip
+++ b/prmers_amd/csrc/kernels_v2.hip
@@ -54,7 +54,8 @@
   const uint32_t blk = row / pl.L1, qq = row - blk * pl.L1;
   const uint32_t k1row = col_label(pl, blk, pl.logL1 ? (__brev(qq) >> (32 - pl.logL1)) : 0u);
   const uint64_t erho = rho_exponent(pl, k1row, HH * kb + h);
-  const uint64_t rho_lo = pl.TWlo[erho & ((1u << pl.twh) - 1)], rho_hi = pl.TWhi[erho >> pl.twh];
+  constexpr bool SQ = (mode == 0 || mode == 4);
+  const uint64_t rho_lo = (SQ ? pl.TAUlo : pl.TWlo)[erho & ((1u << pl.twh) - 1)], rho_hi = (SQ ? pl.TAUhi : pl.TWhi)[erho >> pl.twh];
 
   if (H == 1) {
 #pragma unroll
@@ -115,17 +116,17 @@
   {
     const uint64_t rho0 = gf::mul(rho_lo, rho_hi);
     const P2* Y = reinterpret_cast<const P2*>(Yimg) + size_t(tile) * (4096 * HH) + h * 4096;
-#pragma unroll
-    for (int k4 = 0; k4 < 8; ++k4) {
+    uint64_t tau = rho0;
+#pragma unroll
+    for (int j4 = 0; j4 < 8; ++j4) {
+      const int k4 = (5 * j4) & 7;
       const unsigned sh = 24u * (k4 & 3);
       const bool neg = (k4 == 1) || (k4 == 3) || (k4 == 4) || (k4 == 6);
       const P2 u = x[k4];
       P2 r;
-      if (mode == 0 || mode == 4) {
-        const uint64_t q = gf::mul_pow2(gf::mul(gf::sqr(u.b), rho0), sh);
-        const uint64_t s0 = gf::sqr(u.a);
-        r.a = neg ? gf::sub(s0, q) : gf::add(s0, q);
-        r.b = gf::dbl(gf::mul(u.b, u.a));
+      if (SQ) {
+        if (j4) tau = gf::mul_pow2(tau, 12);
+        r = p2_sqr3(u, tau);
       } else {
         P2 y = Y[512 * k4 + t];
         if (mode == 3) {
@@ -267,7 +268,8 @@
   const uint32_t blk = row / pl.L1, qq = row - blk * pl.L1;
   const uint32_t k1row = col_label(pl, blk, pl.logL1 ? (__brev(qq) >> (32 - pl.logL1)) : 0u);
   const uint64_t erho = rho_exponent(pl, k1row, kb);
-  const uint64_t rho_lo = pl.TWlo[erho & ((1u << pl.twh) - 1)], rho_hi = pl.TWhi[erho >> pl.twh];
+  constexpr bool SQ = (mode == 0 || mode == 4);
+  const uint64_t rho_lo = (SQ ? pl.TAUlo : pl.TWlo)[erho & ((1u << pl.twh) - 1)], rho_hi = (SQ ? pl.TAUhi : pl.TWhi)[erho >> pl.twh];
 
 #pragma unroll
   for (int d = 0; d < 4; ++d) { const P2 v = in[512 * d + t]; x[d] = v.a; x[4 + d] = v.b; }
@@ -317,11 +319,11 @@
       const bool neg = (k4 == 1) || (k4 == 3) || (k4 == 4) || (k4 == 6);
       const uint64_t w = x[k4];
       uint64_t keep, send;
-      if (mode == 0 || mode == 4) {
+      if (SQ) {
+        const unsigned e16 = (156u * unsigned(k4)) % 192u, ts = e16 >= 96u ? e16 - 96u : e16;
         const uint64_t o = swap32(w, partner);
-        keep = gf::sqr(w);
-        send = gf::mul(pln ? keep : w, pln ? rho0 : o);
-        if (pln) send = gf::mul_pow2(send, sh);
+        keep = w;
+        send = gf::mul(w, pln ? gf::mul_pow2(rho0, ts) : o);
       } else {
         uint64_t y = Y[512 * k4 + t], yo = Y[512 * k4 + (t ^ 32u)];
         if (mode == 3) {
@@ -333,7 +335,7 @@
         if (pln) { const uint64_t q = gf::mul_pow2(gf::mul(keep, rho0), sh); keep = send; send = q; }
       }
       const uint64_t recv = swap32(send, partner);
-      if (mode == 0 || mode == 4) x[k4] = pln ? gf::dbl(recv) : (neg ? gf::sub(keep, recv) : gf::add(keep, recv));
+      if (SQ) x[k4] = pln ? recv : gf::mul(gf::add_lazy(recv, keep), gf::sub(keep, recv));
       else x[k4] = pln ? gf::add(keep, recv) : (neg ? gf::sub(keep, recv) : gf::add(keep, recv));
     }
   }
diff --git a/prmers_amd/csrc/kernels_v2_common.hpp b/prmers_amd/csrc/kernels_v2_common.hpp
--- a/prmers_amd/csrc/kernels_v2_common.hpp
+++ b/prmers_amd/csrc/kernels_v2_common.hpp
@@ -18,6 +18,7 @@
 __device__ __forceinline__ P2 w_load(const P2* p) { return *p; }
 
 __device__ __forceinline__ P2 p2_mul(P2 x, uint64_t w) { return {gf::mul(x.a, w), gf::mul(x.b, w)}; }
+__device__ __forceinline__ P2 p2_sqr3(P2 u, uint64_t tau) { P2 r; gf::sqr3(u.a, u.b, tau, r.a, r.b); return r; }
 
 template <bool INV, int LAZY = 0>
 __device__ __forceinline__ void dft8p(P2 (&x)[8]) {
diff --git a/prmers_amd/csrc/kernels_v3.hip b/prmers_amd/csrc/kernels_v3.hip
--- a/prmers_amd/csrc/kernels_v3.hip
+++ b/prmers_amd/csrc/kernels_v3.hip
@@ -116,13 +116,13 @@
 #pragma unroll
   for (int k5 = 0; k5 < 4; ++k5) {
     const P2 u = x[k5];
+    if (mode == 0) {
+      x[k5] = v2::p2_sqr3(u, gf::mul_pow2(rho0, 24u * unsigned(k5)));
+      continue;
+    }
     P2 r;
     uint64_t q, s0;
-    if (mode == 0) {
-      q = gf::mul(gf::sqr(u.b), rho0);
-      s0 = gf::sqr(u.a);
-      r.b = gf::dbl(gf::mul(u.b, u.a));
-    } else {
+    {
       P2 y = reinterpret_cast<const P2*>(Y + base)[256 * k5 + f.t];
       if (mode == 3) {
         const P2 z = reinterpret_cast<const P2*>(Y2 + base)[256 * k5 + f.t];
@@ -142,11 +142,13 @@
 #pragma unroll
   for (int k5 = 0; k5 < 4; ++k5) {
     const uint64_t u = x[k5], uo = swap_planes(u);
+    if (mode == 0) {
+      const uint64_t got = swap_planes(gf::mul(u, f.pln ? gf::mul_pow2(rho0, 24u * unsigned(k5)) : uo));
+      x[k5] = f.pln ? got : gf::mul(gf::add_lazy(got, u), gf::sub(u, got));
+      continue;
+    }
     uint64_t m1, cross;
-    if (mode == 0) {
-      m1 = gf::sqr(u);
-      cross = gf::dbl(gf::mul(u, uo));
-    } else {
+    {
       uint64_t y = (Y + base)[f.at(256 * k5 + f.t)];
       if (mode == 3) y = gf::add_lazy_any(y, (Y2 + base)[f.at(256 * k5 + f.t)]);
       const uint64_t yo = swap_planes(y);
@@ -180,7 +182,8 @@
   const uint32_t k1row = col_label(pl, blk, pl.logL1 ? (__brev(qq) >> (32 - pl.logL1)) : 0u);
   const uint64_t erho = rho_exponent(pl, k1row, kb);
   uint64_t rho_lo = 0, rho_hi = 0;
-  if (mode != 2) { rho_lo = pl.TWlo[erho & ((1u << pl.twh) - 1)]; rho_hi = pl.TWhi[erho >> pl.twh]; }
+  constexpr bool SQ = (mode == 0 || mode == 4);
+  if (mode != 2) { rho_lo = (SQ ? pl.TAUlo : pl.TWlo)[erho & ((1u << pl.twh) - 1)]; rho_hi = (SQ ? pl.TAUhi : pl.TWhi)[erho >> pl.twh]; }
 
   rows_forward(f, x, tw);
   if (mode == 4) {
diff --git a/prmers_amd/csrc/plan.hpp b/prmers_amd/csrc/plan.hpp
--- a/prmers_amd/csrc/plan.hpp
+++ b/prmers_amd/csrc/plan.hpp
@@ -48,6 +48,7 @@
   std::vector<uint32_t> SA, SB;
   std::vector<uint64_t> TA, TAi, TB, TBi;
   std::vector<uint64_t> TWlo, TWhi;
+  std::vector<uint64_t> TAUlo, TAUhi;
   std::vector<uint64_t> UT1, UT2;
   std::vector<uint64_t> S2r, S2ri, S1r, S1ri;
   std::vector<uint32_t> DI;
@@ -261,6 +262,14 @@
   pl.TWlo[0] = 1; for (size_t i = 1; i < lo_n; ++i) pl.TWlo[i] = gf::mul(pl.TWlo[i - 1], om);
   const uint64_t step = gf::mul(pl.TWlo[lo_n - 1], om);
   pl.TWhi[0] = 1; for (size_t i = 1; i < hi_n; ++i) pl.TWhi[i] = gf::mul(pl.TWhi[i - 1], step);
+  {
+    const uint64_t om2m = gf::root_of_unity(2 * m);
+    if (gf::mul(om2m, om2m) != om) throw std::runtime_error("internal: omega_2m^2 is expected to be omega_m");
+    pl.TAUlo.resize(lo_n); pl.TAUhi.resize(hi_n);
+    pl.TAUlo[0] = 1; for (size_t i = 1; i < lo_n; ++i) pl.TAUlo[i] = gf::mul(pl.TAUlo[i - 1], om2m);
+    const uint64_t step2 = gf::mul(pl.TAUlo[lo_n - 1], om2m);
+    pl.TAUhi[0] = uint64_t(1) << 48; for (size_t i = 1; i < hi_n; ++i) pl.TAUhi[i] = gf::mul(pl.TAUhi[i - 1], step2);
+  }
   const uint64_t om1 = gf::pow(om, pl.M2), om2 = gf::pow(om, pl.M1);
   pl.UT1.resize(pl.M1); pl.UT1[0] = 1; for (uint32_t i = 1; i < pl.M1; ++i) pl.UT1[i] = gf::mul(pl.UT1[i - 1], om1);
   pl.UT2.resize(pl.M2); pl.UT2[0] = 1; for (uint32_t i = 1; i < pl.M2; ++i) pl.UT2[i] = gf::mul(pl.UT2[i - 1], om2);
diff --git a/prmers_amd/csrc/selftest.hip b/prmers_amd/csrc/selftest.hip
--- a/prmers_amd/csrc/selftest.hip
+++ b/prmers_amd/csrc/selftest.hip
@@ -92,6 +92,7 @@
   std::vector<uint64_t> in, out, tuples, dft8_out;
   run_family<GfScalar>("gf scalars", in, out);
   run_family<GfLazySum>("gf lazy sum", in, out);
+  run_family<GfSquare3>("gf sqr3", in, out);
   run_family<GfDft8>("gf dft8", tuples, dft8_out);
   {
     in.clear(); GfDft4::fill(in);
diff --git a/prmers_amd/csrc/selftest_cases.hpp b/prmers_amd/csrc/selftest_cases.hpp
--- a/prmers_amd/csrc/selftest_cases.hpp
+++ b/prmers_amd/csrc/selftest_cases.hpp
@@ -145,6 +145,53 @@
       both_lazy += (x > P && y > P); sum_lazy += out[2 * i] > P;
     }
     if (!both_lazy || !sum_lazy) return msg("gf add_lazy_any: the operand list misses a lazy case (both operands above P: %zu, sum above P: %zu)", both_lazy, sum_lazy);
+    return "";
+  }
+};
+
+struct GfSquare3 {
+  static constexpr int IN = 3, OUT = 4;
+  static constexpr bool kHostEqualsDevice = false;
+  static void aux(std::vector<uint64_t>&) {}
+  static void fill(std::vector<uint64_t>& in) {
+    std::vector<uint64_t> e; GfScalar::edges(e);
+    const uint64_t taus[] = {0, 1, P - 1, uint64_t(1) << 48, 0xffffffffull, 0x123456789abcdef0ull % P, P, 0xffffffffffffffffull};
+    for (uint64_t x : e) for (uint64_t y : e) for (uint64_t t : taus) { in.push_back(x); in.push_back(y); in.push_back(t); }
+    Rng r(0x3f84d5b5b5470917ull);
+    for (int i = 0; i < 4096; ++i) { in.push_back(r.next()); in.push_back(r.next()); in.push_back((i & 3) == 3 ? r.next() : r.next() % P); }
+    for (int i = 0; i < 1024; ++i) { in.push_back(r.next() | 0xffffffff00000000ull); in.push_back(r.next() | 0xffffffff00000000ull); in.push_back(r.next() % P); }
+    for (int i = 0; i < 2048; ++i) {
+      const uint64_t b = r.next(), tau = r.next() % P, t = gf_mulmod(b, tau), d = 1 + r.next() % 0xfffffffeull;
+      in.push_back(P + d - t); in.push_back(b); in.push_back(tau);
+    }
+    for (int i = 0; i < 2048; ++i) {
+      uint64_t b = r.next(); if (b % P == 0) b = 1;
+      const uint64_t t = r.next() & 0x3fffffffull, d = 1 + (r.next() & 0x3fffffffull), tau = gf::mul(gf::inv(b % P), t);
+      in.push_back(t + P + d); in.push_back(b); in.push_back(tau);
+    }
+  }
+  static GF_HDM void eval(const uint64_t* in, uint64_t* o, const uint64_t*) {
+    gf::sqr3(in[0], in[1], in[2], o[0], o[1]);
+    const uint64_t t = gf::mul(in[1], in[2]);
+    o[2] = gf::add_lazy(t, in[0]);
+    o[3] = gf::sub(in[0], t);
+  }
+  static std::string check(const uint64_t* in, const uint64_t* out, size_t n) {
+    size_t lazy[4] = {};
+    for (size_t i = 0; i < n; ++i) {
+      const uint64_t a = in[3 * i], b = in[3 * i + 1], tau = in[3 * i + 2];
+      const uint64_t* o = out + 4 * i;
+      const uint64_t t = gf_mulmod(b, tau), rho = (P - gf_mulmod(tau, tau)) % P;
+      const uint64_t want_a = uint64_t((u128(gf_mulmod(a, a)) + gf_mulmod(rho, gf_mulmod(b, b))) % P), want_b = gf_mulmod(a, b);
+      if (o[0] != want_a || o[1] != want_b)
+        return msg("gf sqr3: a=%016llx b=%016llx tau=%016llx got (%016llx, %016llx) want (%016llx, %016llx)", MI355_X(a), MI355_X(b), MI355_X(tau), MI355_X(o[0]),
+                   MI355_X(o[1]), MI355_X(want_a), MI355_X(want_b));
+      if (o[2] % P != uint64_t((u128(t) + a % P) % P) || o[3] % P != uint64_t((u128(a % P) + P - t) % P))
+        return msg("gf sqr3, the sums: a=%016llx b=%016llx tau=%016llx got %016llx, %016llx", MI355_X(a), MI355_X(b), MI355_X(tau), MI355_X(o[2]), MI355_X(o[3]));
+      lazy[0] += a > P; lazy[1] += b > P; lazy[2] += o[2] > P; lazy[3] += o[3] > P;
+    }
+    for (int k = 0; k < 4; ++k)
+      if (!lazy[k]) return msg("gf sqr3: no case put a value above P into lazy slot %d (a, b, t + a, a - t)", k);
     return "";
   }
 };
```

Result: faster. 6721 iter/s (median of 4 runs) (+6.6%).
